# ccnmaastricht/ODE-Column

Hardware: NVIDIA B200
Metric: population_steps_per_sec_fwd_adjoint (higher is better)
Workload: dtype f32

## Files before the change

ode-column_b200/csrc/stage_tc.cu:

```cuda
#include <cstdlib>
#include "stage_tc.cuh"

namespace odecol {
namespace tc {

struct StoreEpi {
    float* C; int M, N, ldc;
    ODECOL_DEVINL void prepare() {}
    ODECOL_DEVINL void rows(int, int i, int n0, int, int g, int TNq, const float (&tot)[kMaxQ]) const {
        if (i >= M) return;
#pragma unroll
        for (int j = 0; j < kMaxQ; ++j) {
            const int b = n0 + g * TNq + j;
            if (j < TNq && b < N) C[(size_t)b * ldc + i] = tot[j];
        }
    }
    ODECOL_DEVINL void tile_done(int, int, int, int, int) const {}
};

struct ContractLayout { int Mp, Np, Kp, TN; size_t off_Ahi, off_Alo, off_Bhi, off_Blo, total; };
static ContractLayout contract_layout(int M, int N, int K) {
    ContractLayout L;
    L.Mp = round_up(M, BM); L.Kp = round_up(K, BK);
    L.TN = pick_tile_n(L.Mp / BM, N);
    L.Np = round_up(N, L.TN);
    size_t o = 0;
    auto take = [&](size_t floats) { const size_t r = o; o += (floats * 4 + 1023) / 1024 * 1024; return r; };
    L.off_Ahi = take((size_t)L.Mp * L.Kp); L.off_Alo = take((size_t)L.Mp * L.Kp);
    L.off_Bhi = take((size_t)L.Np * L.Kp); L.off_Blo = take((size_t)L.Np * L.Kp);
    L.total = o;
    return L;
}


__global__ void k_tc_init(DevProblem p, TileGeom tg, const float* __restrict__ y, const float* __restrict__ t_ptr,
                          float* __restrict__ hi0, float* __restrict__ lo0, float* __restrict__ hi1, float* __restrict__ lo1,
                          float* __restrict__ V0T, float* __restrict__ A0T, float* __restrict__ F0T, int KPa) {
    const int b = blockIdx.x, N = p.N, Kaug = N + p.n_in + 1;
    const size_t ro = (size_t)b * KPa;
    const int nt = b / tg.TN, g = (b % tg.TN) / tg.TNq, jq = (b % tg.TN) % tg.TNq;
    const int q = jq >> 2, e4 = jq & 3;
    if (b >= p.B) {
        for (int k = threadIdx.x; k < KPa; k += blockDim.x) { hi0[ro + k] = 0.f; lo0[ro + k] = 0.f; hi1[ro + k] = 0.f; lo1[ro + k] = 0.f; }
        for (int i = threadIdx.x; i < tg.Np; i += blockDim.x) {
            const size_t o = tg.off(nt, g, q, i) + e4;
            V0T[o] = 0.f; A0T[o] = 0.f; F0T[o] = 0.f;
        }
        return;
    }
    const float* yb = y + (size_t)b * 3 * N;
    int idx = 1;
    const float tcl = knot_locate(p.knot_t, p.K, __ldg(t_ptr), idx);
    const float* ku = p.knot_u + (size_t)b * p.knot_stride_b;
    for (int k = threadIdx.x; k < KPa; k += blockDim.x) {
        float v = 0.f, one = 0.f;
        if (k < N) v = phi_fast(yb[k] - yb[N + k]);
        else if (k < N + p.n_in) v = knot_value(p.knot_t, ku, p.n_in, idx, tcl, k - N);
        else if (k == Kaug - 1) { v = 1.f; one = 1.f; }
        const float h = tf32_rna(v);
        hi0[ro + k] = h; lo0[ro + k] = tf32_rna(v - h);
        hi1[ro + k] = one; lo1[ro + k] = 0.f;
    }
    for (int i = threadIdx.x; i < tg.Np; i += blockDim.x) {
        const size_t o = tg.off(nt, g, q, i) + e4;
        const bool in = i < N;
        const float V = in ? yb[i] : 0.f, A = in ? yb[N + i] : 0.f, F = in ? yb[2 * N + i] : 0.f;
        V0T[o] = V; A0T[o] = A; F0T[o] = F;
    }
}

struct TcFwdLayout {
    int Np, Bp, KPa, TN, KP16;
    size_t off_Whi, off_Wlo, off_Rhi[2], off_Rlo[2], off_K[3], off_Y[2], off_done, off_inv, total;
    size_t off_W16[2], off_R16[2], off_wscale;
};

static TcFwdLayout tc_fwd_layout(const DevProblem& p) {
    TcFwdLayout L;
    L.Np = round_up(p.N, BM);
    L.KPa = round_up(p.N + p.n_in + 1, BK);
    L.TN = pick_tile_n(L.Np / BM, p.B);
    L.Bp = round_up(p.B, L.TN);
    size_t o = 0;
    auto take = [&](size_t floats) { const size_t r = o; o += (floats * 4 + 1023) / 1024 * 1024; return r; };
    L.off_Whi = take((size_t)L.Np * L.KPa); L.off_Wlo = take((size_t)L.Np * L.KPa);
    for (int i = 0; i < 2; ++i) { L.off_Rhi[i] = take((size_t)L.Bp * L.KPa); L.off_Rlo[i] = take((size_t)L.Bp * L.KPa); }
    const size_t plane = (size_t)L.Np * L.Bp;
    for (int i = 0; i < 3; ++i) L.off_K[i] = take(plane);
    for (int i = 0; i < 2; ++i) L.off_Y[i] = take(3 * plane);
    L.off_done = take((size_t)(L.Bp / L.TN) + 64);
    L.off_inv = take(3ull * p.N + 4);
    L.KP16 = round_up(p.N + p.n_in + 1, BK16);
    for (int i = 0; i < 2; ++i) L.off_W16[i] = take(((size_t)L.Np * L.KP16 + 1) / 2);
    for (int i = 0; i < 2; ++i) L.off_R16[i] = take((size_t)L.Bp * L.KP16);
    L.off_wscale = take(4);
    L.total = o;
    return L;
}

}

void tc_launch_init(const DevProblem& p, const tc::TileGeom& tg, const float* y0, const float* t_dev, float* hi0, float* lo0,
                    float* hi1, float* lo1, float* V0T, float* A0T, float* F0T, int KPa, int Bp, cudaStream_t s) {
    tc::k_tc_init<<<Bp, 128, 0, s>>>(p, tg, y0, t_dev, hi0, lo0, hi1, lo1, V0T, A0T, F0T, KPa);
}

int tc_rk4_fwd_persistent(const DevProblem& p, const float* t_dev, int T, const float* y0, float* y_out, int out_every,
                          float* Whi, float* Wlo, float* const Rhi[2], float* const Rlo[2], float* const KT[3],
                          float* const YT[2], unsigned int* done, int Np, int Bp, int KPa, int TN, const tc::CkptView* ck,
                          const tc::Mixed16* mx, cudaStream_t s);

namespace tc {
static Mixed16 mixed16_view(const TcFwdLayout& L, char* w) {
    Mixed16 m;
    for (int i = 0; i < 2; ++i) { m.W16[i] = w + L.off_W16[i]; m.R16[i] = reinterpret_cast<uint16_t*>(w + L.off_R16[i]); }
    m.wscale = reinterpret_cast<float*>(w + L.off_wscale);
    m.KP16 = L.KP16;
    return m;
}
}

static bool persistent_enabled() {
    const char* v = getenv("ODECOL_PERSISTENT");
    return v ? atoi(v) != 0 : true;
}

size_t tc_rk4_fwd_workspace_bytes(const DevProblem& p, int) { return tc::tc_fwd_layout(p).total; }

int tc_rk4_fwd(const DevProblem& p, const float* t_dev, int T, const float* y0, float* y_out, int out_every, void* ws,
               size_t ws_bytes, cudaStream_t s) {
    using namespace tc;
    const TcFwdLayout L = tc_fwd_layout(p);
    if (!ws || ws_bytes < L.total) return ODECOL_E_WORKSPACE;
    if (p.N % 4 != 0) return ODECOL_E_UNSUPPORTED;
    char* w = static_cast<char*>(ws);
    auto F = [&](size_t off) { return reinterpret_cast<float*>(w + off); };
    float *Whi = F(L.off_Whi), *Wlo = F(L.off_Wlo);
    float* Rhi[2] = {F(L.off_Rhi[0]), F(L.off_Rhi[1])};
    float* Rlo[2] = {F(L.off_Rlo[0]), F(L.off_Rlo[1])};
    float* KT[3] = {F(L.off_K[0]), F(L.off_K[1]), F(L.off_K[2])};
    float* YT[2] = {F(L.off_Y[0]), F(L.off_Y[1])};
    const int Kaug = p.N + p.n_in + 1;
    const size_t st = (size_t)p.B * 3 * p.N;
    const TileGeom tg{L.Bp / L.TN, L.Np, L.TN, L.TN / 4};
    if (persistent_enabled() && L.KPa / BK <= kChunkMin) {
        const Mixed16 mx = mixed16_view(L, w);
        return tc_rk4_fwd_persistent(p, t_dev, T, y0, y_out, out_every, Whi, Wlo, Rhi, Rlo, KT, YT,
                                     reinterpret_cast<unsigned int*>(w + L.off_done), L.Np, L.Bp, L.KPa, L.TN, nullptr, &mx, s);
    }

    k_split_pad<<<296, 256, 0, s>>>(p.W_aug, p.N, Kaug, p.ld_w, Whi, Wlo, L.Np, L.KPa);
    k_tc_init<<<L.Bp, 128, 0, s>>>(p, tg, y0, t_dev, Rhi[0], Rlo[0], Rhi[1], Rlo[1], YT[0], YT[0] + tg.plane(),
                                   YT[0] + 2 * tg.plane(), L.KPa);
    count_launch(2);
    if (cudaMemcpyAsync(y_out, y0, sizeof(float) * st, cudaMemcpyDeviceToDevice, s) != cudaSuccess) return ODECOL_E_CUDA;
    CUtensorMap mWhi, mWlo, mRhi[2], mRlo[2];
    bool ok = make_map(&mWhi, Whi, L.Np, L.KPa, L.KPa, BM) && make_map(&mWlo, Wlo, L.Np, L.KPa, L.KPa, BM);
    for (int i = 0; i < 2; ++i)
        ok = ok && make_map(&mRhi[i], Rhi[i], L.Bp, L.KPa, L.KPa, L.TN) && make_map(&mRlo[i], Rlo[i], L.Bp, L.KPa, L.KPa, L.TN);
    if (!ok) return ODECOL_E_CUDA;
    const TileShape ts{L.Np / BM, L.Bp / L.TN, L.TN, L.KPa / BK, 0};
    int cur = 0;
    auto launch = [&](auto& e) { return launch_contract(mWhi, mWlo, mRhi[cur], mRlo[cur], ts, e, s); };
    for (int n = 0; n < T - 1; ++n) {
        const int j = n + 1;
        const bool emit = (j % out_every == 0) || (j == T - 1);
        const size_t r = (j % out_every == 0) ? (size_t)(j / out_every) : (size_t)((T - 2) / out_every + 1);
        auto fill = [&](auto& e) {
            e.p = p; e.tg = tg; e.t = t_dev; e.n = n; e.KPa = L.KPa;
            const size_t pl = tg.plane();
            e.V0T = YT[n & 1]; e.A0T = YT[n & 1] + pl; e.F0T = YT[n & 1] + 2 * pl;
            e.V1T = YT[(n + 1) & 1]; e.A1T = YT[(n + 1) & 1] + pl; e.F1T = YT[(n + 1) & 1] + 2 * pl;
            e.traj_row = emit ? y_out + r * st : nullptr; e.ysel_row = nullptr; e.inv = nullptr; e.G = 0;
            e.K1T = KT[0]; e.K2T = KT[1]; e.K3T = KT[2];
            e.Rhi_nxt = Rhi[cur ^ 1]; e.Rlo_nxt = Rlo[cur ^ 1]; e.DRT_nxt = nullptr;
            e.inv_tm = 1.0f / p.c.tau_m; e.inv_ta = 1.0f / p.c.tau_a; e.inv_ts = 1.0f / p.c.tau_s;
            e.t0 = e.t1 = e.dt = 0.f;
        };
        for (int S = 1; S <= 4; ++S) {
            int rc;
            if (S == 1) { FwdEpiT<1> e; fill(e); rc = launch(e); }
            else if (S == 2) { FwdEpiT<2> e; fill(e); rc = launch(e); }
            else if (S == 3) { FwdEpiT<3> e; fill(e); rc = launch(e); }
            else { FwdEpiT<4> e; fill(e); rc = launch(e); }
            if (rc != ODECOL_OK) return rc;
            cur ^= 1;
        }
    }
    return cudaGetLastError() == cudaSuccess ? ODECOL_OK : ODECOL_E_CUDA;
}


size_t tc_rk4_ckpt_bytes(const DevProblem& p, int T) {
    const tc::TcFwdLayout L = tc::tc_fwd_layout(p);
    if (L.KPa / tc::BK > tc::kChunkMin) return 0;
    const size_t plane = 4ull * L.Np * L.Bp;
    return plane * (2ull * T + 3ull * (T - 1));
}

int tc_rk4_fwd_ckpt(const DevProblem& p, const float* t_dev, int T, const float* y0, const int* sel, int G, float* y_sel,
                    void* ckpt, size_t ckpt_bytes, void* ws, size_t ws_bytes, cudaStream_t s) {
    using namespace tc;
    const TcFwdLayout L = tc_fwd_layout(p);
    if (!ws || ws_bytes < L.total) return ODECOL_E_WORKSPACE;
    if (L.KPa / BK > kChunkMin) return ODECOL_E_UNSUPPORTED;
    if (!ckpt || ckpt_bytes < tc_rk4_ckpt_bytes(p, T)) return ODECOL_E_WORKSPACE;
    if (p.N % 4 != 0) return ODECOL_E_UNSUPPORTED;
    char* w = static_cast<char*>(ws);
    auto F = [&](size_t off) { return reinterpret_cast<float*>(w + off); };
    float* Rhi[2] = {F(L.off_Rhi[0]), F(L.off_Rhi[1])};
    float* Rlo[2] = {F(L.off_Rlo[0]), F(L.off_Rlo[1])};
    float* KT[3] = {F(L.off_K[0]), F(L.off_K[1]), F(L.off_K[2])};
    float* YT[2] = {F(L.off_Y[0]), F(L.off_Y[1])};
    int* inv = reinterpret_cast<int*>(w + L.off_inv);
    const size_t plane = (size_t)L.Np * L.Bp;
    k_tc_build_inv<<<1, 256, 0, s>>>(sel, G, 3 * p.N, inv);
    k_tc_gather_sel<<<296, 256, 0, s>>>(y0, sel, G, p.B, 3 * p.N, y_sel);
    count_launch(2);
    CkptView ck;
    ck.VA = static_cast<float*>(ckpt); ck.K = ck.VA + 2 * plane * (size_t)T; ck.y_sel = y_sel; ck.inv = inv; ck.G = G;
    const Mixed16 mx = mixed16_view(L, w);
    return tc_rk4_fwd_persistent(p, t_dev, T, y0, nullptr, 1, F(L.off_Whi), F(L.off_Wlo), Rhi, Rlo, KT, YT,
                                 reinterpret_cast<unsigned int*>(w + L.off_done), L.Np, L.Bp, L.KPa, L.TN, &ck, &mx, s);
}

size_t tc_contract_workspace_bytes(int M, int N, int K) { return tc::contract_layout(M, N, K).total; }

int tc_contract(const float* A, const float* B, float* C, int M, int N, int K, void* ws, size_t ws_bytes, cudaStream_t s) {
    using namespace tc;
    const ContractLayout L = contract_layout(M, N, K);
    if (!ws || ws_bytes < L.total) return ODECOL_E_WORKSPACE;
    char* w = static_cast<char*>(ws);
    float* Ahi = reinterpret_cast<float*>(w + L.off_Ahi); float* Alo = reinterpret_cast<float*>(w + L.off_Alo);
    float* Bhi = reinterpret_cast<float*>(w + L.off_Bhi); float* Blo = reinterpret_cast<float*>(w + L.off_Blo);
    k_split_pad<<<296, 256, 0, s>>>(A, M, K, K, Ahi, Alo, L.Mp, L.Kp);
    k_split_pad<<<296, 256, 0, s>>>(B, N, K, K, Bhi, Blo, L.Np, L.Kp);
    count_launch(2);
    CUtensorMap ma_hi, ma_lo, mb_hi, mb_lo;
    if (!make_map(&ma_hi, Ahi, L.Mp, L.Kp, L.Kp, BM) || !make_map(&ma_lo, Alo, L.Mp, L.Kp, L.Kp, BM) ||
        !make_map(&mb_hi, Bhi, L.Np, L.Kp, L.Kp, L.TN) || !make_map(&mb_lo, Blo, L.Np, L.Kp, L.Kp, L.TN))
        return ODECOL_E_CUDA;
    const TileShape ts{L.Mp / BM, L.Np / L.TN, L.TN, L.Kp / BK, 0};
    StoreEpi epi{C, M, N, M};
    return launch_contract(ma_hi, ma_lo, mb_hi, mb_lo, ts, epi, s);
}

}
```

ode-column_b200/csrc/stage_tc.cuh:

```cuda
#pragma once
#include <cuda.h>
#include <cuda_fp16.h>
#include "odecol_common.cuh"

namespace odecol {

constexpr float kOneThirdL = 0.3333333333333333f;
constexpr float kTwoThirdsL = 0.6666666666666666f;

static inline int round_up(int x, int m) { return (x + m - 1) / m * m; }

ODECOL_DEVINL float4 ld4(const float* p) { return *reinterpret_cast<const float4*>(p); }
ODECOL_DEVINL void st4(float* p, float4 v) { *reinterpret_cast<float4*>(p) = v; }
ODECOL_DEVINL float4 ld4s(const float* p) { return __ldcg(reinterpret_cast<const float4*>(p)); }
ODECOL_DEVINL void st4s(float* p, float4 v) { __stcg(reinterpret_cast<float4*>(p), v); }

namespace tc {

constexpr int BM = 128;
constexpr int BK = 32;
#ifndef ODECOL_TC_STAGES
#define ODECOL_TC_STAGES 3
#endif
constexpr int STAGES = ODECOL_TC_STAGES;
constexpr int kEpiWarps = 16;
constexpr int kMainAcc = 3;
#ifndef ODECOL_EPI_REGS
#define ODECOL_EPI_REGS 0
#endif
constexpr int kEpiRegs = ODECOL_EPI_REGS;
constexpr int kThreads = 32 * ((kEpiRegs ? 4 : 2) + kEpiWarps);
#ifdef ODECOL_ROLES_HIGH
constexpr int kEpiWarp0 = 0, kTmaWarp = kEpiWarps, kMmaWarp = kEpiWarps + 1;
#else
constexpr int kTmaWarp = 0, kMmaWarp = 1, kEpiWarp0 = kEpiRegs ? 4 : 2;
#endif
template <int N> ODECOL_DEVINL void setmaxnreg_inc() { asm volatile("setmaxnreg.inc.sync.aligned.u32 %0;" ::"n"(N)); }
template <int N> ODECOL_DEVINL void setmaxnreg_dec() { asm volatile("setmaxnreg.dec.sync.aligned.u32 %0;" ::"n"(N)); }
constexpr uint32_t kSpinLimit = 1u << 24;
constexpr int kChunkKB = 16;
constexpr int kChunkMin = 24;

ODECOL_DEVINL uint32_t smem_u32(const void* p) { return (uint32_t)__cvta_generic_to_shared(p); }

ODECOL_DEVINL void mbar_init(uint32_t bar, uint32_t count) {
    asm volatile("mbarrier.init.shared::cta.b64 [%0], %1;" ::"r"(bar), "r"(count) : "memory");
}
ODECOL_DEVINL void mbar_expect_tx(uint32_t bar, uint32_t bytes) {
    asm volatile("mbarrier.arrive.expect_tx.shared::cta.b64 _, [%0], %1;" ::"r"(bar), "r"(bytes) : "memory");
}
ODECOL_DEVINL void mbar_arrive(uint32_t bar) {
    asm volatile("mbarrier.arrive.shared::cta.b64 _, [%0];" ::"r"(bar) : "memory");
}
ODECOL_DEVINL void mbar_wait(uint32_t bar, uint32_t parity) {
    uint32_t done = 0, spins = 0;
    while (true) {
        asm volatile("{\n\t.reg .pred p;\n\tmbarrier.try_wait.parity.shared::cta.b64 p, [%1], %2;\n\tselp.u32 %0, 1, 0, p;\n\t}"
                     : "=r"(done) : "r"(bar), "r"(parity) : "memory");
        if (done) break;
        if (++spins > kSpinLimit) __trap();
    }
}
ODECOL_DEVINL void tma_load_2d(uint32_t dst, const CUtensorMap* map, uint32_t bar, int c0, int c1) {
    asm volatile("cp.async.bulk.tensor.2d.shared::cluster.global.mbarrier::complete_tx::bytes [%0], [%1, {%3, %4}], [%2];"
                 ::"r"(dst), "l"(reinterpret_cast<uint64_t>(map)), "r"(bar), "r"(c0), "r"(c1) : "memory");
}
ODECOL_DEVINL void umma_tf32(uint32_t d_tmem, uint64_t adesc, uint64_t bdesc, uint32_t idesc, uint32_t accumulate) {
    asm volatile("{\n\t.reg .pred p;\n\tsetp.ne.b32 p, %4, 0;\n\ttcgen05.mma.cta_group::1.kind::tf32 [%0], %1, %2, %3, p;\n\t}"
                 ::"r"(d_tmem), "l"(adesc), "l"(bdesc), "r"(idesc), "r"(accumulate) : "memory");
}
ODECOL_DEVINL void umma_commit(uint32_t bar) {
    asm volatile("tcgen05.commit.cta_group::1.mbarrier::arrive::one.shared::cluster.b64 [%0];" ::"r"(bar) : "memory");
}
ODECOL_DEVINL void tc_fence_before() { asm volatile("tcgen05.fence::before_thread_sync;" ::: "memory"); }
ODECOL_DEVINL void tc_fence_after() { asm volatile("tcgen05.fence::after_thread_sync;" ::: "memory"); }
ODECOL_DEVINL void tmem_ld4_issue(uint32_t taddr, uint32_t (&u)[4]) {
    asm volatile("tcgen05.ld.sync.aligned.32x32b.x4.b32 {%0, %1, %2, %3}, [%4];"
                 : "=r"(u[0]), "=r"(u[1]), "=r"(u[2]), "=r"(u[3]) : "r"(taddr));
}
ODECOL_DEVINL void tmem_ld_wait() { asm volatile("tcgen05.wait::ld.sync.aligned;" ::: "memory"); }

ODECOL_DEVINL uint64_t make_smem_desc(uint32_t smem_addr) {
    uint64_t d = 0;
    d |= (uint64_t)((smem_addr & 0x3FFFFu) >> 4);
    d |= (uint64_t)1 << 16;
    d |= (uint64_t)(1024 >> 4) << 32;
    d |= (uint64_t)1 << 46;
    d |= (uint64_t)2 << 61;
    return d;
}
ODECOL_DEVINL uint32_t make_idesc(int tile_n) {
    return (1u << 4) | (2u << 7) | (2u << 10) | ((uint32_t)(tile_n >> 3) << 17) | ((uint32_t)(BM >> 4) << 24);
}

ODECOL_DEVINL float tf32_rna(float x) {
    return __uint_as_float((__float_as_uint(x) + 0x1000u) & 0xFFFFE000u);
}

ODECOL_DEVINL float ldg_if(const float* p, bool ok) {
    float v;
    asm volatile("{\n\t.reg .pred q;\n\tsetp.ne.b32 q, %2, 0;\n\tmov.f32 %0, 0f00000000;\n\t@q ld.global.nc.f32 %0, [%1];\n\t}"
                 : "=f"(v) : "l"(p), "r"((int)ok));
    return v;
}

constexpr int BK16 = 64;
constexpr float kF16Limit = 6.0e4f;
struct F16x2 { unsigned short h, l; };
ODECOL_DEVINL F16x2 f16_split2(float x) {
    const __half h = __float2half_rn(x);
    const __half l = __float2half_rn((x - __half2float(h)) * 2048.0f);
    return {__half_as_ushort(h), __half_as_ushort(l)};
}
ODECOL_DEVINL void st_global_u16_if(uint16_t* p, unsigned short v, bool ok) {
    asm volatile("{\n\t.reg .pred q;\n\tsetp.ne.b32 q, %2, 0;\n\t@q st.global.b16 [%0], %1;\n\t}" ::"l"(p), "h"(v), "r"((int)ok) : "memory");
}
ODECOL_DEVINL void umma_f16(uint32_t d_tmem, uint64_t adesc, uint64_t bdesc, uint32_t idesc, uint32_t accumulate) {
    asm volatile("{\n\t.reg .pred p;\n\tsetp.ne.b32 p, %4, 0;\n\ttcgen05.mma.cta_group::1.kind::f16 [%0], %1, %2, %3, p;\n\t}"
                 ::"r"(d_tmem), "l"(adesc), "l"(bdesc), "r"(idesc), "r"(accumulate) : "memory");
}
ODECOL_DEVINL uint32_t make_idesc16(int tile_n) {
    return (1u << 4) | ((uint32_t)(tile_n >> 3) << 17) | ((uint32_t)(BM >> 4) << 24);
}

struct Mixed16 {
    void* W16[2];
    uint16_t* R16[2];
    float* wscale;
    int KP16;
};

struct TileShape {
    int MT, NT, TN, KB;
    int b_row0;
};

ODECOL_DEVINL unsigned int ld_acquire_u32(const unsigned int* p) {
    unsigned int v;
    asm volatile("ld.acquire.gpu.global.u32 %0, [%1];" : "=r"(v) : "l"(p) : "memory");
    return v;
}

ODECOL_DEVINL void st_global(float* p, float v) { asm volatile("st.global.f32 [%0], %1;" ::"l"(p), "f"(v) : "memory"); }
ODECOL_DEVINL void st_global_if(float* p, float v, bool ok) {
    asm volatile("{\n\t.reg .pred q;\n\tsetp.ne.b32 q, %2, 0;\n\t@q st.global.f32 [%0], %1;\n\t}" ::"l"(p), "f"(v), "r"((int)ok) : "memory");
}
constexpr int kMaxQ = 32;

constexpr int kTileGroupM = 12;
ODECOL_DEVINL void tile_coords(int tile, int MT, int NT, int& m, int& nt) {
    const int per_group = kTileGroupM * NT;
    const int grp = tile / per_group, within = tile - grp * per_group;
    const int gm = min(kTileGroupM, MT - grp * kTileGroupM);
    nt = within / gm;
    m = grp * kTileGroupM + (within - nt * gm);
}

template <class Epi, bool CHUNKED, bool F16 = false>
__global__ void __launch_bounds__(kThreads, 1)
k_tc_contract(const __grid_constant__ CUtensorMap mA_hi, const __grid_constant__ CUtensorMap mA_lo,
              const __grid_constant__ CUtensorMap mB_hi, const __grid_constant__ CUtensorMap mB_lo, TileShape ts, Epi epi) {
    extern __shared__ uint8_t smem_raw[];
    __shared__ __align__(8) uint64_t bars[2 * STAGES + 4];
    __shared__ uint32_t tmem_base_slot;
    const int warp = threadIdx.x >> 5, lane = threadIdx.x & 31;
    const uint32_t ring = (smem_u32(smem_raw) + 1023u) & ~1023u;
    constexpr int KEL = F16 ? BK16 : BK;
    constexpr int CKB = F16 ? kChunkKB / 2 : kChunkKB;
    constexpr float XS = F16 ? 4.8828125e-4f : 1.0f;
    const uint32_t a_bytes = BM * 128, b_bytes = (uint32_t)ts.TN * 128;
    const uint32_t stage_bytes = 2 * a_bytes + 2 * b_bytes;
    const uint32_t full0 = smem_u32(&bars[0]), empty0 = smem_u32(&bars[STAGES]);
    const uint32_t tfull = smem_u32(&bars[2 * STAGES]), tempty = smem_u32(&bars[2 * STAGES + 1]);
    constexpr bool chunked = CHUNKED;
    const uint32_t cfull0 = tfull, cempty0 = smem_u32(&bars[2 * STAGES + 2]);

    const int tiles = ts.MT * ts.NT;
    const uint32_t acc_stride = (uint32_t)ts.TN;
    uint32_t ncols = 32;
    while (ncols < (kMainAcc + 1) * acc_stride) ncols <<= 1;

    if (threadIdx.x == 0) {
        for (int s = 0; s < STAGES; ++s) { mbar_init(full0 + 8 * s, 1); mbar_init(empty0 + 8 * s, 1); }
        mbar_init(tfull, 1);
        mbar_init(tempty, chunked ? 1 : kEpiWarps);
        mbar_init(cempty0, kEpiWarps);
        mbar_init(cempty0 + 8, kEpiWarps);
        asm volatile("fence.mbarrier_init.release.cluster;" ::: "memory");
    }
    if (warp == kMmaWarp) {
        asm volatile("tcgen05.alloc.cta_group::1.sync.aligned.shared::cta.b32 [%0], %1;" ::"r"(smem_u32(&tmem_base_slot)), "r"(ncols) : "memory");
        asm volatile("tcgen05.relinquish_alloc_permit.cta_group::1.sync.aligned;" ::: "memory");
    }
    tc_fence_before();
    __syncthreads();
    tc_fence_after();
    const uint32_t tmem_base = tmem_base_slot;

    if (warp == kTmaWarp) {
        if (lane == 0) {
            int stage = 0; uint32_t phase = 0;
            for (int tile = blockIdx.x; tile < tiles; tile += gridDim.x) {
                int mt_, nt_;
                tile_coords(tile, ts.MT, ts.NT, mt_, nt_);
                const int m0 = mt_ * BM, n0 = nt_ * ts.TN;
                for (int kb = 0; kb < ts.KB; ++kb) {
                    mbar_wait(empty0 + 8 * stage, phase ^ 1);
                    const uint32_t base = ring + stage * stage_bytes, fb = full0 + 8 * stage;
                    mbar_expect_tx(fb, stage_bytes);
                    tma_load_2d(base, &mA_hi, fb, kb * KEL, m0);
                    tma_load_2d(base + a_bytes, &mA_lo, fb, kb * KEL, m0);
                    tma_load_2d(base + 2 * a_bytes, &mB_hi, fb, kb * KEL, n0 + ts.b_row0);
                    tma_load_2d(base + 2 * a_bytes + b_bytes, &mB_lo, fb, kb * KEL, n0 + ts.b_row0);
                    if (++stage == STAGES) { stage = 0; phase ^= 1; }
                }
            }
        }
    } else if (warp == kMmaWarp) {
        if (lane == 0) {
            const uint32_t idesc = F16 ? make_idesc16(ts.TN) : make_idesc(ts.TN);
            const uint32_t d_small = tmem_base + kMainAcc * acc_stride;
            int stage = 0; uint32_t phase = 0, tphase = 0;
            int c = 0;
            for (int tile = blockIdx.x; chunked && tile < tiles; tile += gridDim.x) {
                int jj = 0;
                uint32_t d_main = tmem_base, d_cross = tmem_base + acc_stride;
                for (int kb = 0; kb < ts.KB; ++kb) {
                    if (kb % CKB == 0) {
                        const int set = c & 1;
                        mbar_wait(cempty0 + 8 * set, (uint32_t)((c >> 1) & 1) ^ 1u);
                        tc_fence_after();
                        d_main = tmem_base + (uint32_t)set * 2 * acc_stride;
                        d_cross = d_main + acc_stride;
                        jj = 0;
                    }
                    mbar_wait(full0 + 8 * stage, phase);
                    tc_fence_after();
                    const uint32_t base = ring + stage * stage_bytes;
                    const uint64_t a_hi = make_smem_desc(base), a_lo = make_smem_desc(base + a_bytes);
                    const uint64_t b_hi = make_smem_desc(base + 2 * a_bytes), b_lo = make_smem_desc(base + 2 * a_bytes + b_bytes);
#pragma unroll
                    for (int k = 0; k < 4; ++k, ++jj) {
                        const uint64_t adv = (uint64_t)(k * 32 >> 4);
                        if (F16) {
                            umma_f16(d_cross, a_lo + adv, b_hi + adv, idesc, jj != 0);
                            umma_f16(d_cross, a_hi + adv, b_lo + adv, idesc, 1);
                            umma_f16(d_main, a_hi + adv, b_hi + adv, idesc, jj != 0);
                        } else {
                            umma_tf32(d_cross, a_lo + adv, b_hi + adv, idesc, jj != 0);
                            umma_tf32(d_cross, a_hi + adv, b_lo + adv, idesc, 1);
                            umma_tf32(d_main, a_hi + adv, b_hi + adv, idesc, jj != 0);
                        }
                    }
                    umma_commit(empty0 + 8 * stage);
                    if (++stage == STAGES) { stage = 0; phase ^= 1; }
                    if (kb % CKB == CKB - 1 || kb == ts.KB - 1) { umma_commit(cfull0 + 8 * (c & 1)); ++c; }
                }
            }
            for (int tile = blockIdx.x; !chunked && tile < tiles; tile += gridDim.x) {
                mbar_wait(tempty, tphase ^ 1);
                tc_fence_after();
                int j = 0;
                for (int kb = 0; kb < ts.KB; ++kb) {
                    mbar_wait(full0 + 8 * stage, phase);
                    tc_fence_after();
                    const uint32_t base = ring + stage * stage_bytes;
                    const uint64_t a_hi = make_smem_desc(base), a_lo = make_smem_desc(base + a_bytes);
                    const uint64_t b_hi = make_smem_desc(base + 2 * a_bytes), b_lo = make_smem_desc(base + 2 * a_bytes + b_bytes);
#pragma unroll
                    for (int k = 0; k < 4; ++k, ++j) {
                        const uint64_t adv = (uint64_t)(k * 32 >> 4);
                        const uint32_t d_main = tmem_base + (uint32_t)(j % kMainAcc) * acc_stride;
                        if (F16) {
                            umma_f16(d_small, a_lo + adv, b_hi + adv, idesc, j != 0);
                            umma_f16(d_small, a_hi + adv, b_lo + adv, idesc, 1);
                            umma_f16(d_main, a_hi + adv, b_hi + adv, idesc, j >= kMainAcc);
                        } else {
                            umma_tf32(d_small, a_lo + adv, b_hi + adv, idesc, j != 0);
                            umma_tf32(d_small, a_hi + adv, b_lo + adv, idesc, 1);
                            umma_tf32(d_main, a_hi + adv, b_hi + adv, idesc, j >= kMainAcc);
                        }
                    }
                    umma_commit(empty0 + 8 * stage);
                    if (++stage == STAGES) { stage = 0; phase ^= 1; }
                }
                umma_commit(tfull);
                tphase ^= 1;
            }
        }
    } else if (warp >= kEpiWarp0) {
        const int ew = warp - kEpiWarp0;
        const int quarter = warp & 3;
        const int g = ew >> 2;
        const int etid = ew * 32 + lane;
        const int TNq = ts.TN >> 2;
        epi.prepare();
        uint32_t tphase = 0;
        int cchunk = 0;
        for (int tile = blockIdx.x; tile < tiles; tile += gridDim.x) {
            int m_tile, nt;
            tile_coords(tile, ts.MT, ts.NT, m_tile, nt);
            const int n0 = nt * ts.TN;
            const int row = m_tile * BM + quarter * 32 + lane;
            float tot[kMaxQ];
            if (chunked) {
                const uint32_t lb = tmem_base + ((uint32_t)(quarter * 32) << 16) + (uint32_t)(g * TNq);
#pragma unroll
                for (int q = 0; q < kMaxQ; ++q) tot[q] = 0.f;
                const int nchunks = (ts.KB + CKB - 1) / CKB;
                for (int cc = 0; cc < nchunks; ++cc, ++cchunk) {
                    const int set = cchunk & 1;
                    mbar_wait(cfull0 + 8 * set, (uint32_t)((cchunk >> 1) & 1));
                    tc_fence_after();
#pragma unroll
                    for (int q0 = 0; q0 < kMaxQ / 4; q0 += 4) {
                        uint32_t um[4][4], ux[4][4];
#pragma unroll
                        for (int d = 0; d < 4; ++d) {
                            if (4 * (q0 + d) < TNq) {
                                tmem_ld4_issue(lb + (uint32_t)set * 2 * acc_stride + 4 * (q0 + d), um[d]);
                                tmem_ld4_issue(lb + (uint32_t)set * 2 * acc_stride + acc_stride + 4 * (q0 + d), ux[d]);
                            }
                        }
                        tmem_ld_wait();
#pragma unroll
                        for (int d = 0; d < 4; ++d) {
                            if (4 * (q0 + d) < TNq) {
#pragma unroll
                                for (int e = 0; e < 4; ++e) tot[4 * (q0 + d) + e] += __uint_as_float(ux[d][e]) * XS + __uint_as_float(um[d][e]);
                            }
                        }
                    }
                    tc_fence_before();
                    __syncwarp();
                    if (lane == 0) mbar_arrive(cempty0 + 8 * set);
                }
                epi.rows(m_tile, row, n0, nt, g, TNq, tot);
                epi.tile_done(m_tile, n0, ts.TN, etid, kEpiWarps * 32);
                continue;
            }
            mbar_wait(tfull, tphase);
            tc_fence_after();
            const uint32_t lane_base = tmem_base + ((uint32_t)(quarter * 32) << 16) + (uint32_t)(g * TNq);
#pragma unroll
            for (int q = 0; q < kMaxQ / 4; ++q) {
                if (4 * q < TNq) {
                    uint32_t u[kMainAcc + 1][4];
#pragma unroll
                    for (int a = 0; a <= kMainAcc; ++a) tmem_ld4_issue(lane_base + a * acc_stride + 4 * q, u[a]);
                    tmem_ld_wait();
#pragma unroll
                    for (int e = 0; e < 4; ++e) {
                        float sum = __uint_as_float(u[kMainAcc][e]) * XS;
#pragma unroll
                        for (int a = 0; a < kMainAcc; ++a) sum += __uint_as_float(u[a][e]);
                        tot[4 * q + e] = sum;
                    }
                }
            }
            tc_fence_before();
            __syncwarp();
            if (lane == 0) mbar_arrive(tempty);
            tphase ^= 1;
            epi.rows(m_tile, row, n0, nt, g, TNq, tot);
            epi.tile_done(m_tile, n0, ts.TN, etid, kEpiWarps * 32);
        }
    }
    tc_fence_before();
    __syncthreads();
    if (warp == kMmaWarp) {
        asm volatile("tcgen05.dealloc.cta_group::1.sync.aligned.b32 %0, %1;" ::"r"(tmem_base), "r"(ncols) : "memory");
    }
}

typedef CUresult (*EncodeTiledFn)(CUtensorMap*, CUtensorMapDataType, cuuint32_t, void*, const cuuint64_t*, const cuuint64_t*,
                                  const cuuint32_t*, const cuuint32_t*, CUtensorMapInterleave, CUtensorMapSwizzle,
                                  CUtensorMapL2promotion, CUtensorMapFloatOOBfill);

inline EncodeTiledFn encode_fn() {
    static EncodeTiledFn fn = nullptr;
    if (!fn) {
        void* p = nullptr;
        cudaDriverEntryPointQueryResult q;
        if (cudaGetDriverEntryPoint("cuTensorMapEncodeTiled", &p, cudaEnableDefault, &q) == cudaSuccess && q == cudaDriverEntryPointSuccess)
            fn = reinterpret_cast<EncodeTiledFn>(p);
    }
    return fn;
}

inline bool make_map(CUtensorMap* map, const float* base, uint64_t rows, uint64_t cols, uint64_t ld, uint32_t box_rows,
                     CUtensorMapSwizzle swz = CU_TENSOR_MAP_SWIZZLE_128B) {
    EncodeTiledFn fn = encode_fn();
    if (!fn) return false;
    const cuuint64_t dims[2] = {cols, rows};
    const cuuint64_t strides[1] = {ld * sizeof(float)};
    const cuuint32_t box[2] = {BK, box_rows};
    const cuuint32_t estr[2] = {1, 1};
    return fn(map, CU_TENSOR_MAP_DATA_TYPE_FLOAT32, 2, const_cast<float*>(base), dims, strides, box, estr,
              CU_TENSOR_MAP_INTERLEAVE_NONE, swz, CU_TENSOR_MAP_L2_PROMOTION_L2_256B,
              CU_TENSOR_MAP_FLOAT_OOB_FILL_NONE) == CUDA_SUCCESS;
}

inline bool make_map16(CUtensorMap* map, const void* base, uint64_t rows, uint64_t cols, uint64_t ld, uint32_t box_rows, bool bf16) {
    EncodeTiledFn fn = encode_fn();
    if (!fn) return false;
    const cuuint64_t dims[2] = {cols, rows};
    const cuuint64_t strides[1] = {ld * 2};
    const cuuint32_t box[2] = {BK16, box_rows};
    const cuuint32_t estr[2] = {1, 1};
    return fn(map, bf16 ? CU_TENSOR_MAP_DATA_TYPE_BFLOAT16 : CU_TENSOR_MAP_DATA_TYPE_FLOAT16, 2, const_cast<void*>(base), dims,
              strides, box, estr, CU_TENSOR_MAP_INTERLEAVE_NONE, CU_TENSOR_MAP_SWIZZLE_128B, CU_TENSOR_MAP_L2_PROMOTION_L2_256B,
              CU_TENSOR_MAP_FLOAT_OOB_FILL_NONE) == CUDA_SUCCESS;
}

inline int num_sms() {
    static int n = 0;
    if (!n) {
        int dev = 0;
        cudaGetDevice(&dev);
        cudaDeviceGetAttribute(&n, cudaDevAttrMultiProcessorCount, dev);
        if (n <= 0) n = 148;
    }
    return n;
}

inline int pick_tile_n(int MT, int B) {
    const int sms = num_sms();
    int best = 16;
    double best_cost = 1e30;
    for (int tn = 16; tn <= 128; tn += 16) {
        const int nt = (B + tn - 1) / tn;
        const long tiles = (long)MT * nt;
        const long waves = (tiles + sms - 1) / sms;
        const double cost = (double)waves * (tn + 24.0);
        if (cost < best_cost - 1e-9) { best_cost = cost; best = tn; }
    }
    return best;
}

template <class Epi>
static int launch_contract(const CUtensorMap& a_hi, const CUtensorMap& a_lo, const CUtensorMap& b_hi, const CUtensorMap& b_lo,
                           const TileShape& ts, const Epi& epi, cudaStream_t s) {
    const size_t smem = (size_t)STAGES * (2 * BM * BK * 4 + 2 * (size_t)ts.TN * BK * 4) + 1024;
    static bool configured = false;
    if (!configured) {
        if (cudaFuncSetAttribute(k_tc_contract<Epi, false>, cudaFuncAttributeMaxDynamicSharedMemorySize, 200 * 1024) != cudaSuccess ||
            cudaFuncSetAttribute(k_tc_contract<Epi, true>, cudaFuncAttributeMaxDynamicSharedMemorySize, 200 * 1024) != cudaSuccess)
            return ODECOL_E_CUDA;
        configured = true;
    }
    const int tiles = ts.MT * ts.NT;
    const int grid = tiles < num_sms() ? tiles : num_sms();
    if (ts.KB > kChunkMin) k_tc_contract<Epi, true><<<grid, kThreads, smem, s>>>(a_hi, a_lo, b_hi, b_lo, ts, epi);
    else k_tc_contract<Epi, false><<<grid, kThreads, smem, s>>>(a_hi, a_lo, b_hi, b_lo, ts, epi);
    count_launch();
    return cudaGetLastError() == cudaSuccess ? ODECOL_OK : ODECOL_E_CUDA;
}

template <class Epi>
static int launch_contract16(const CUtensorMap& a_hi, const CUtensorMap& a_lo, const CUtensorMap& b_hi, const CUtensorMap& b_lo,
                             const TileShape& ts, const Epi& epi, cudaStream_t s) {
    const size_t smem = (size_t)STAGES * (2 * BM * 128 + 2 * (size_t)ts.TN * 128) + 1024;
    static bool configured = false;
    if (!configured) {
        if (cudaFuncSetAttribute(k_tc_contract<Epi, false, true>, cudaFuncAttributeMaxDynamicSharedMemorySize, 200 * 1024) != cudaSuccess ||
            cudaFuncSetAttribute(k_tc_contract<Epi, true, true>, cudaFuncAttributeMaxDynamicSharedMemorySize, 200 * 1024) != cudaSuccess)
            return ODECOL_E_CUDA;
        configured = true;
    }
    const int tiles = ts.MT * ts.NT;
    const int grid = tiles < num_sms() ? tiles : num_sms();
    if (ts.KB > kChunkMin / 2) k_tc_contract<Epi, true, true><<<grid, kThreads, smem, s>>>(a_hi, a_lo, b_hi, b_lo, ts, epi);
    else k_tc_contract<Epi, false, true><<<grid, kThreads, smem, s>>>(a_hi, a_lo, b_hi, b_lo, ts, epi);
    count_launch();
    return cudaGetLastError() == cudaSuccess ? ODECOL_OK : ODECOL_E_CUDA;
}

static __global__ void k_split_pad(const float* __restrict__ src, int rows, int cols, int ld, float* __restrict__ hi,
                            float* __restrict__ lo, int rows_p, int cols_p) {
    const size_t total = (size_t)rows_p * cols_p;
    for (size_t e = blockIdx.x * (size_t)blockDim.x + threadIdx.x; e < total; e += (size_t)gridDim.x * blockDim.x) {
        const int r = (int)(e / cols_p), c = (int)(e % cols_p);
        const float x = (r < rows && c < cols) ? src[(size_t)r * ld + c] : 0.0f;
        const float h = tf32_rna(x);
        hi[e] = h;
        lo[e] = tf32_rna(x - h);
    }
}

static __global__ void k_absmax(const float* __restrict__ src, int rows, int cols, int ld, unsigned int* __restrict__ out) {
    unsigned int m = 0;
    const size_t total = (size_t)rows * cols;
    for (size_t e = blockIdx.x * (size_t)blockDim.x + threadIdx.x; e < total; e += (size_t)gridDim.x * blockDim.x) {
        const float x = fabsf(src[(e / cols) * ld + (e % cols)]);
        if (x == x && x < 3.0e38f) m = max(m, __float_as_uint(x));
    }
#pragma unroll
    for (int o = 16; o > 0; o >>= 1) m = max(m, __shfl_xor_sync(0xffffffffu, m, o));
    if ((threadIdx.x & 31) == 0 && m) atomicMax(out, m);
}
static __global__ void k_split16_w(const float* __restrict__ src, int rows, int cols, int ld, __half* __restrict__ hi,
                                   __half* __restrict__ lo, int rows_p, int cols_p, const unsigned int* __restrict__ amax,
                                   float* __restrict__ wscale) {
    const float m = __uint_as_float(*amax);
    int ex = 0;
    if (m > 0.f) frexpf(m, &ex);
    const int sh = m > 0.f ? max(-100, min(100, 14 - ex)) : 0;
    const float sc = ldexpf(1.0f, sh);
    if (blockIdx.x == 0 && threadIdx.x == 0) wscale[0] = ldexpf(1.0f, -sh);
    unsigned int* ovf = reinterpret_cast<unsigned int*>(wscale + 2);
    const size_t total = (size_t)rows_p * cols_p;
    for (size_t e = blockIdx.x * (size_t)blockDim.x + threadIdx.x; e < total; e += (size_t)gridDim.x * blockDim.x) {
        const int r = (int)(e / cols_p), c = (int)(e % cols_p);
        const float x = (r < rows && c < cols) ? src[(size_t)r * ld + c] * sc : 0.0f;
        if (!(fabsf(x) <= kF16Limit)) *ovf = 1u;
        const F16x2 t = f16_split2(x);
        hi[e] = __ushort_as_half(t.h);
        lo[e] = __ushort_as_half(t.l);
    }
}
static __global__ void k_r16_from32(const float* __restrict__ hi, const float* __restrict__ lo, int Bp, int KPa,
                                    uint16_t* __restrict__ R16, int KP16, unsigned int* __restrict__ ovf) {
    const size_t total = (size_t)Bp * KP16, plane = total;
    for (size_t e = blockIdx.x * (size_t)blockDim.x + threadIdx.x; e < total; e += (size_t)gridDim.x * blockDim.x) {
        const int b = (int)(e / KP16), k = (int)(e % KP16);
        const float x = k < KPa ? hi[(size_t)b * KPa + k] + lo[(size_t)b * KPa + k] : 0.0f;
        if (!(fabsf(x) <= kF16Limit)) *ovf = 1u;
        const F16x2 t = f16_split2(x);
        R16[e] = t.h; R16[plane + e] = t.l;
    }
}

static __global__ void k_tc_build_inv(const int* __restrict__ sel, int G, int n3, int* __restrict__ inv) {
    for (int e = threadIdx.x; e < n3; e += blockDim.x) inv[e] = sel ? -1 : e;
    if (threadIdx.x == 0) inv[n3] = sel ? 0 : 1;
    __syncthreads();
    if (sel) for (int g = threadIdx.x; g < G; g += blockDim.x) {
        inv[sel[g]] = g;
        if (sel[g] >= 2 * (n3 / 3)) inv[n3] = 1;
    }
}

static __global__ void k_tc_gather_sel(const float* __restrict__ y, const int* __restrict__ sel, int G, int B, int n3,
                                       float* __restrict__ out) {
    const size_t total = (size_t)B * G;
    for (size_t e = blockIdx.x * (size_t)blockDim.x + threadIdx.x; e < total; e += (size_t)gridDim.x * blockDim.x) {
        const int b = (int)(e / G), g = (int)(e % G);
        out[e] = y[(size_t)b * n3 + (sel ? sel[g] : g)];
    }
}

struct CkptView {
    float* VA; float* K;
    float* y_sel;
    const int* inv;
    int G;
};


struct TileGeom {
    int NT, Np, TN, TNq;
    __host__ __device__ __forceinline__ size_t plane() const { return (size_t)NT * 4 * Np * TNq; }
    ODECOL_DEVINL size_t off(int nt, int g, int q, int i) const {
        return ((((size_t)nt * 4 + g) * (TNq >> 2) + q) * Np + i) * 4;
    }
};

ODECOL_DEVINL void stimulus_columns(const DevProblem& p, int KPa, int idx, float tcl, int n0, int tile_n, int part, int parts,
                                    int tid, int nthr, float* __restrict__ Rhi, float* __restrict__ Rlo) {
    const int n_in = p.n_in, N = p.N;
    const float x0 = __ldg(p.knot_t + idx - 1), x1 = __ldg(p.knot_t + idx);
    const float dx = __fsub_rn(x1, x0), dtc = __fsub_rn(tcl, x0);
    const bool vec = ((n_in | N | KPa | (int)p.knot_stride_b) & 3) == 0 &&
                     ((reinterpret_cast<uintptr_t>(p.knot_u) | reinterpret_cast<uintptr_t>(Rhi) | reinterpret_cast<uintptr_t>(Rlo)) & 15) == 0;
    if (vec) {
        const int nq = n_in >> 2, total = tile_n * nq, share = (total + parts - 1) / parts;
        const int e_end = min(total, (part + 1) * share);
        int e = part * share + tid;
        if (e >= e_end) return;
        int bl = e / nq, c = e - bl * nq;
        const int dbl = nthr / nq, dc = nthr - dbl * nq;
        for (; e < e_end; e += nthr) {
            const int b = n0 + bl;
            if (b < p.B) {
                const float* ku = p.knot_u + (size_t)b * p.knot_stride_b + 4 * c;
                const float4 y0 = __ldg(reinterpret_cast<const float4*>(ku + (size_t)(idx - 1) * n_in));
                const float4 y1 = __ldg(reinterpret_cast<const float4*>(ku + (size_t)idx * n_in));
                float4 h, l;
#pragma unroll
                for (int k = 0; k < 4; ++k) {
                    const float slope = __fdiv_rn(__fsub_rn((&y1.x)[k], (&y0.x)[k]), dx);
                    const float v = __fadd_rn((&y0.x)[k], __fmul_rn(slope, dtc));
                    (&h.x)[k] = tf32_rna(v);
                    (&l.x)[k] = tf32_rna(v - (&h.x)[k]);
                }
                const size_t at = (size_t)b * KPa + N + 4 * c;
                *reinterpret_cast<float4*>(Rhi + at) = h;
                *reinterpret_cast<float4*>(Rlo + at) = l;
            }
            bl += dbl; c += dc;
            if (c >= nq) { c -= nq; ++bl; }
        }
        return;
    }
    const int total = tile_n * n_in, share = (total + parts - 1) / parts;
    const int e_end = min(total, (part + 1) * share);
    for (int e = part * share + tid; e < e_end; e += nthr) {
        const int b = n0 + e / n_in, ch = e % n_in;
        if (b < p.B) {
            const float v = knot_value(p.knot_t, p.knot_u + (size_t)b * p.knot_stride_b, n_in, idx, tcl, ch);
            const float h = tf32_rna(v);
            Rhi[(size_t)b * KPa + N + ch] = h;
            Rlo[(size_t)b * KPa + N + ch] = tf32_rna(v - h);
        }
    }
}

ODECOL_DEVINL void stimulus_columns16(const DevProblem& p, int KP16, size_t plane, int idx, float tcl, int n0, int tile_n, int part,
                                      int parts, int tid, int nthr, uint16_t* __restrict__ R16, unsigned int* __restrict__ ovf) {
    const int n_in = p.n_in, N = p.N;
    const float x0 = __ldg(p.knot_t + idx - 1), x1 = __ldg(p.knot_t + idx);
    const float dx = __fsub_rn(x1, x0), dtc = __fsub_rn(tcl, x0);
    const bool vec = ((n_in | N | KP16 | (int)p.knot_stride_b) & 3) == 0 && (plane & 3) == 0 &&
                     (reinterpret_cast<uintptr_t>(p.knot_u) & 15) == 0 && (reinterpret_cast<uintptr_t>(R16) & 7) == 0;
    if (vec) {
        const int nq = n_in >> 2, total = tile_n * nq, share = (total + parts - 1) / parts;
        const int e_end = min(total, (part + 1) * share);
        int e = part * share + tid;
        if (e >= e_end) return;
        int bl = e / nq, c = e - bl * nq;
        const int dbl = nthr / nq, dc = nthr - dbl * nq;
        for (; e < e_end; e += nthr) {
            const int b = n0 + bl;
            if (b < p.B) {
                const float* ku = p.knot_u + (size_t)b * p.knot_stride_b + 4 * c;
                const float4 y0 = __ldg(reinterpret_cast<const float4*>(ku + (size_t)(idx - 1) * n_in));
                const float4 y1 = __ldg(reinterpret_cast<const float4*>(ku + (size_t)idx * n_in));
                F16x2 t[4];
                bool big = false;
#pragma unroll
                for (int k = 0; k < 4; ++k) {
                    const float slope = __fdiv_rn(__fsub_rn((&y1.x)[k], (&y0.x)[k]), dx);
                    const float v = __fadd_rn((&y0.x)[k], __fmul_rn(slope, dtc));
                    big |= !(fabsf(v) <= kF16Limit);
                    t[k] = f16_split2(v);
                }
                if (big) *ovf = 1u;
                uint16_t* at = R16 + (size_t)b * KP16 + N + 4 * c;
                *reinterpret_cast<uint2*>(at) = make_uint2((uint32_t)t[0].h | ((uint32_t)t[1].h << 16), (uint32_t)t[2].h | ((uint32_t)t[3].h << 16));
                *reinterpret_cast<uint2*>(at + plane) = make_uint2((uint32_t)t[0].l | ((uint32_t)t[1].l << 16), (uint32_t)t[2].l | ((uint32_t)t[3].l << 16));
            }
            bl += dbl; c += dc;
            if (c >= nq) { c -= nq; ++bl; }
        }
        return;
    }
    const int total = tile_n * n_in, share = (total + parts - 1) / parts;
    const int e_end = min(total, (part + 1) * share);
    for (int e = part * share + tid; e < e_end; e += nthr) {
        const int b = n0 + e / n_in, ch = e % n_in;
        if (b < p.B) {
            const float v = knot_value(p.knot_t, p.knot_u + (size_t)b * p.knot_stride_b, n_in, idx, tcl, ch);
            if (!(fabsf(v) <= kF16Limit)) *ovf = 1u;
            const F16x2 t = f16_split2(v);
            uint16_t* at = R16 + (size_t)b * KP16 + N + ch;
            at[0] = t.h; at[plane] = t.l;
        }
    }
}

template <int S, bool F16 = false>
struct FwdEpiT {
    DevProblem p;
    TileGeom tg;
    const float* t;
    int n, KPa;
    uint16_t* R16_nxt; size_t r16_plane; int KP16;
    const float* wscale;
    unsigned int* ovf;
    float ws;
    const float* V0T; const float* A0T; const float* F0T;
    float* V1T; float* A1T; float* F1T;
    float* traj_row;
    float* ysel_row;
    const int* inv;
    int G;
    float* K1T; float* K2T; float* K3T;
    float* Rhi_nxt; float* Rlo_nxt;
    float* DRT_nxt;
    float inv_tm, inv_ta, inv_ts;
    float t0, t1, dt;
    int needF;

    ODECOL_DEVINL void prepare() {
        t0 = __ldg(t + n); t1 = __ldg(t + n + 1);
        dt = __fsub_rn(t1, t0);
        needF = (S == 4 && ysel_row && inv && !traj_row) ? __ldg(inv + 3 * p.N) : 1;
        ws = F16 ? __ldg(wscale) : 1.0f;
    }

    struct Group { float4 V0, A0, k1V, k2V, k3V, F0; };
    ODECOL_DEVINL void load_group(Group& L, size_t oq) const {
        L.V0 = ld4s(V0T + oq); L.A0 = ld4s(A0T + oq);
        if (S >= 2) L.k1V = ld4s(K1T + oq);
        if (S >= 3) L.k2V = ld4s(K2T + oq);
        if (S >= 4) { L.k3V = ld4s(K3T + oq); if (needF) L.F0 = ld4s(F0T + oq); }
    }

    ODECOL_DEVINL void rows(int, int i, int n0, int nt, int g, int TNq, const float (&tot)[kMaxQ]) const {
        if (i >= p.N) return;
        const int N = p.N, B = p.B;
        const float kap = __ldg(p.kappa + i);
        const float third = kOneThirdL;
        const int nq = TNq >> 2;
        const size_t qstride = (size_t)tg.Np * 4;
        const size_t o0 = tg.off(nt, g, 0, i);
        int gV = -1, gA = -1, gF = -1;
        if (S == 4 && ysel_row) { gV = __ldg(inv + i); gA = __ldg(inv + N + i); gF = __ldg(inv + 2 * N + i); }
        Group nxt;
        load_group(nxt, o0);
#pragma unroll 1
        for (int q = 0; q < nq; ++q) {
            const size_t oq = o0 + q * qstride;
            const Group L = nxt;
            if (q + 1 < nq) load_group(nxt, oq + qstride);
            const float4 &V0 = L.V0, &A0 = L.A0, &F0 = L.F0;
            const float4 &k1V = L.k1V, &k2V = L.k2V, &k3V = L.k3V;
            const int q4 = 4 * q;
            float oKV[4], oNV[4], oNA[4], oNF[4], oR[4], oD[4];
#pragma unroll
            for (int e = 0; e < 4; ++e) {
                const float v0 = (&V0.x)[e], a0 = (&A0.x)[e];
                float k1A = 0.f, k2A = 0.f, k3A = 0.f, A = a0, V = v0;
                float r2 = 0.f, r3 = 0.f;
                const float r1 = phi_fast(v0 - a0);
                float r = r1;
                if (S >= 2) {
                    k1A = (kap * r1 - a0) * inv_ta;
                    const float v2 = v0 + dt * (&k1V.x)[e] * third, a2 = a0 + dt * k1A * third;
                    r2 = phi_fast(v2 - a2);
                    if (S == 2) { V = v2; A = a2; r = r2; }
                    if (S >= 3) {
                        k2A = (kap * r2 - a2) * inv_ta;
                        const float v3 = v0 + dt * ((&k2V.x)[e] - (&k1V.x)[e] * third), a3 = a0 + dt * (k2A - k1A * third);
                        r3 = phi_fast(v3 - a3);
                        if (S == 3) { V = v3; A = a3; r = r3; }
                        if (S >= 4) {
                            k3A = (kap * r3 - a3) * inv_ta;
                            V = v0 + dt * ((&k1V.x)[e] - (&k2V.x)[e] + (&k3V.x)[e]); A = a0 + dt * (k1A - k2A + k3A);
                            r = phi_fast(V - A);
                        }
                    }
                }
                const float total = (F16 ? tot[q4 + e] * ws : tot[q4 + e]) * p.c.tau_s;
                const float dV = (total * p.c.R - V) * inv_tm;
                const float dA = (kap * r - A) * inv_ta;
                oKV[e] = dV;
                float nV, nA, nF = 0.f;
                if (S == 1) { nV = v0 + dt * dV * third; nA = a0 + dt * dA * third; }
                if (S == 2) { nV = v0 + dt * (dV - (&k1V.x)[e] * third); nA = a0 + dt * (dA - k1A * third); }
                if (S == 3) { nV = v0 + dt * ((&k1V.x)[e] - (&k2V.x)[e] + dV); nA = a0 + dt * (k1A - k2A + dA); }
                if (S == 4) {
                    nV = v0 + ((&k1V.x)[e] + 3.f * ((&k2V.x)[e] + (&k3V.x)[e]) + dV) * dt * 0.125f;
                    nA = a0 + (k1A + 3.f * (k2A + k3A) + dA) * dt * 0.125f;
                    if (needF) {
                    const float f0 = (&F0.x)[e];
                    const float k1F = (r1 - f0) * inv_ts;
                    const float f2 = f0 + dt * k1F * third;
                    const float k2F = (r2 - f2) * inv_ts;
                    const float f3 = f0 + dt * (k2F - k1F * third);
                    const float k3F = (r3 - f3) * inv_ts;
                    const float f4 = f0 + dt * (k1F - k2F + k3F);
                    const float k4F = (r - f4) * inv_ts;
                    nF = f0 + (k1F + 3.f * (k2F + k3F) + k4F) * dt * 0.125f;
                    }
                }
                oNV[e] = nV; oNA[e] = nA; oNF[e] = nF;
                if (DRT_nxt) phi_dphi_fast(nV - nA, oR[e], oD[e]);
                else oR[e] = phi_fast(nV - nA);
            }
            if (DRT_nxt) st4s(DRT_nxt + oq, make_float4(oD[0], oD[1], oD[2], oD[3]));
            const float4 kV4 = make_float4(oKV[0], oKV[1], oKV[2], oKV[3]);
            if (S == 1) st4s(K1T + oq, kV4);
            if (S == 2) st4s(K2T + oq, kV4);
            if (S == 3) st4s(K3T + oq, kV4);
            if (S == 4) {
                st4s(V1T + oq, make_float4(oNV[0], oNV[1], oNV[2], oNV[3]));
                st4s(A1T + oq, make_float4(oNA[0], oNA[1], oNA[2], oNA[3]));
                if (needF) st4s(F1T + oq, make_float4(oNF[0], oNF[1], oNF[2], oNF[3]));
            }
            const int b0 = n0 + g * TNq + q4;
            float* rh = Rhi_nxt + (size_t)b0 * KPa + i;
            const ptrdiff_t lo_off = Rlo_nxt - Rhi_nxt;
            float* yr = (S == 4 && traj_row) ? traj_row + (size_t)b0 * 3 * N + i : nullptr;
            uint16_t* r16 = F16 ? R16_nxt + (size_t)b0 * KP16 + i : nullptr;
#pragma unroll
            for (int e = 0; e < 4; ++e) {
                const bool ok = b0 + e < B;
                if (F16) {
                    const F16x2 t2 = f16_split2(oR[e]);
                    uint16_t* ph = r16 + (size_t)e * KP16;
                    st_global_u16_if(ph, t2.h, ok);
                    st_global_u16_if(ph + r16_plane, t2.l, ok);
                    if (ok && !(fabsf(oR[e]) <= kF16Limit)) *ovf = 1u;
                } else {
                    const float h = tf32_rna(oR[e]);
                    float* ph = rh + (size_t)e * KPa;
                    st_global_if(ph, h, ok);
                    st_global_if(ph + lo_off, tf32_rna(oR[e] - h), ok);
                }
                if (S == 4 && yr && ok) {
                    float* y = yr + (size_t)e * 3 * N;
                    st_global(y, oNV[e]); st_global(y + N, oNA[e]); st_global(y + 2 * N, oNF[e]);
                }
                if (S == 4 && ysel_row) {
                    float* y = ysel_row + (size_t)(b0 + e) * G;
                    st_global_if(y + gV, oNV[e], ok && gV >= 0);
                    st_global_if(y + gA, oNA[e], ok && gA >= 0);
                    st_global_if(y + gF, oNF[e], ok && gF >= 0);
                }
            }
        }
    }

    ODECOL_DEVINL void tile_done(int m_tile, int n0, int tile_n, int etid, int nthr) const {
        if (p.n_in == 0) return;
        const float tn = S == 1 ? __fadd_rn(t0, __fmul_rn(dt, kOneThirdL)) : S == 2 ? __fadd_rn(t0, __fmul_rn(dt, kTwoThirdsL)) : t1;
        int idx = 1;
        const float tcl = knot_locate(p.knot_t, p.K, tn, idx);
        const int MT = tg.Np / BM;
        if (F16) stimulus_columns16(p, KP16, r16_plane, idx, tcl, n0, tile_n, m_tile, MT, etid, nthr, R16_nxt, ovf);
        else stimulus_columns(p, KPa, idx, tcl, n0, tile_n, m_tile, MT, etid, nthr, Rhi_nxt, Rlo_nxt);
    }
};


}
}
```

ode-column_b200/csrc/stage_tc_bwd.cu:

```cuda
#include "stage_tc.cuh"

namespace odecol {
namespace tc {

template <int S>
struct BwdEpiT {
    DevProblem p;
    TileGeom tg;
    const float* t;
    int n, NPk, G;
    float* acurT;
    float* lamT;
    float* b4T;
    float* b3T;
    const float* DRT;
    float* AVhi_nxt; float* AVlo_nxt;
    const float* grad_y;
    const int* inv;
    float gamma, inv_tm, inv_ta, inv_ts;
    float dt, h8p;
    const float* gy_step;
    int needF;

    ODECOL_DEVINL void prepare() {
        dt = __fsub_rn(__ldg(t + n + 1), __ldg(t + n));
        h8p = n > 0 ? __fsub_rn(__ldg(t + n), __ldg(t + n - 1)) * 0.125f : 0.f;
        needF = __ldg(inv + 3 * p.N);
        gy_step = grad_y + (size_t)n * p.B * G;
    }

    struct Group { float4 aV, aA, dr, lV, lA, lF, p4V, p4A, p3V, p3A, gv, ga, gf; };
    ODECOL_DEVINL void load_group(Group& L, size_t oq, size_t pl, int b0, int gV, int gA, int gF) const {
        L.dr = ld4s(DRT + oq);
        L.lV = ld4s(lamT + oq); L.lA = ld4s(lamT + pl + oq);
        L.lF = needF ? ld4s(lamT + 2 * pl + oq) : make_float4(0.f, 0.f, 0.f, 0.f);
        if (S == 1) { L.aV = ld4s(acurT + oq); L.aA = ld4s(acurT + pl + oq); }
        if (S <= 3) { L.p4V = ld4s(b4T + oq); L.p4A = ld4s(b4T + pl + oq); }
        if (S == 2) { L.p3V = ld4s(b3T + oq); L.p3A = ld4s(b3T + pl + oq); }
        if (S == 1) {
            const float* gy = gy_step + (size_t)b0 * G;
#pragma unroll
            for (int e = 0; e < 4; ++e) {
                const bool ok = b0 + e < p.B;
                (&L.gv.x)[e] = ldg_if(gy + gV, ok && gV >= 0);
                (&L.ga.x)[e] = ldg_if(gy + gA, ok && gA >= 0);
                (&L.gf.x)[e] = ldg_if(gy + gF, ok && gF >= 0);
                gy += G;
            }
        }
    }
    ODECOL_DEVINL void rows(int, int j, int n0, int nt, int g, int TNq, const float (&graw)[kMaxQ]) const {
        if (j >= p.N) return;
        const int N = p.N, B = p.B;
        const float kap = __ldg(p.kappa + j);
        const size_t pl = tg.plane();
        const float h8 = dt * 0.125f, h38 = 3.0f * h8, h3 = dt * kOneThirdL;
        int gV = -1, gA = -1, gF = -1;
        if (S == 1) { gV = inv[j]; gA = inv[N + j]; gF = inv[2 * N + j]; }
        const int nq = TNq >> 2;
        const size_t qstride = (size_t)tg.Np * 4;
        const size_t o0 = tg.off(nt, g, 0, j);
        const int bg = n0 + g * TNq;
        Group nxt;
        load_group(nxt, o0, pl, bg, gV, gA, gF);
#pragma unroll 1
        for (int q = 0; q < nq; ++q) {
            const size_t oq = o0 + q * qstride;
            const Group L = nxt;
            if (q + 1 < nq) load_group(nxt, oq + qstride, pl, bg + 4 * (q + 1), gV, gA, gF);
            float nV[4], nA[4], sV[4], sA[4], sF[4];
#pragma unroll
            for (int e = 0; e < 4; ++e) {
                const float d = (&L.dr.x)[e];
                const float lv = (&L.lV.x)[e], la = (&L.lA.x)[e], lf = (&L.lF.x)[e];
                float av, aa;
                if (S == 4) { av = h8 * lv; aa = h8 * la; }
                if (S == 3) { av = h38 * lv + dt * (&L.p4V.x)[e]; aa = h38 * la + dt * (&L.p4A.x)[e]; }
                if (S == 2) {
                    av = h38 * lv - dt * (&L.p4V.x)[e] + dt * (&L.p3V.x)[e];
                    aa = h38 * la - dt * (&L.p4A.x)[e] + dt * (&L.p3A.x)[e];
                }
                if (S == 1) { av = (&L.aV.x)[e]; aa = (&L.aA.x)[e]; }
                const float bF4 = -(h8 * lf) * inv_ts;
                float af = h8 * lf, bF3 = 0.f, bF2 = 0.f;
                if (S <= 3) { af = h38 * lf + dt * bF4; bF3 = -af * inv_ts; }
                if (S <= 2) { af = h38 * lf - dt * bF4 + dt * bF3; bF2 = -af * inv_ts; }
                if (S == 1) { af = h8 * lf + dt * bF4 - h3 * bF3 + h3 * bF2; }
                const float gg = graw[4 * q + e] + kap * aa * inv_ta + af * inv_ts;
                const float bV = -av * inv_tm + d * gg;
                const float bA = -aa * inv_ta - d * gg;
                if (S == 4) {
                    sV[e] = bV; sA[e] = bA;
                    nV[e] = h38 * lv + dt * bV; nA[e] = h38 * la + dt * bA;
                }
                if (S == 3) {
                    sV[e] = bV; sA[e] = bA;
                    nV[e] = h38 * lv - dt * (&L.p4V.x)[e] + dt * bV;
                    nA[e] = h38 * la - dt * (&L.p4A.x)[e] + dt * bA;
                }
                if (S == 2) {
                    nV[e] = h8 * lv + dt * (&L.p4V.x)[e] - h3 * (&L.p3V.x)[e] + h3 * bV;
                    nA[e] = h8 * la + dt * (&L.p4A.x)[e] - h3 * (&L.p3A.x)[e] + h3 * bA;
                    sV[e] = (&L.p4V.x)[e] + (&L.p3V.x)[e] + bV; sA[e] = (&L.p4A.x)[e] + (&L.p3A.x)[e] + bA;
                }
                if (S == 1) {
                    const float bF1 = -af * inv_ts;
                    const float LV = lv + (&L.p4V.x)[e] + bV + (&L.gv.x)[e];
                    const float LA = la + (&L.p4A.x)[e] + bA + (&L.ga.x)[e];
                    const float LF = lf + (bF4 + bF3 + bF2) + bF1 + (&L.gf.x)[e];
                    sV[e] = LV; sA[e] = LA; sF[e] = LF;
                    nV[e] = h8p * LV; nA[e] = h8p * LA;
                }
            }
            float* sdst = S == 4 ? b4T : S == 3 ? b3T : S == 2 ? b4T : lamT;
            st4s(sdst + oq, make_float4(sV[0], sV[1], sV[2], sV[3]));
            st4s(sdst + pl + oq, make_float4(sA[0], sA[1], sA[2], sA[3]));
            if (S == 1 && needF) st4s(lamT + 2 * pl + oq, make_float4(sF[0], sF[1], sF[2], sF[3]));
            if (S == 2) {
                st4s(acurT + oq, make_float4(nV[0], nV[1], nV[2], nV[3]));
                st4s(acurT + pl + oq, make_float4(nA[0], nA[1], nA[2], nA[3]));
            }
            const int b0 = bg + 4 * q;
            float* ah = AVhi_nxt + (size_t)b0 * NPk + j;
            const ptrdiff_t lo_off = AVlo_nxt - AVhi_nxt;
#pragma unroll
            for (int e = 0; e < 4; ++e) {
                const float v = gamma * nV[e];
                const float h = tf32_rna(v);
                float* ph = ah + (size_t)e * NPk;
                st_global_if(ph, h, b0 + e < B);
                st_global_if(ph + lo_off, tf32_rna(v - h), b0 + e < B);
            }
        }
    }
    ODECOL_DEVINL void tile_done(int, int, int, int, int) const {}
};

constexpr int DW_BK = 32;
constexpr int DW_T = 128;
struct DwShape { int MT, NT, Z, rows_per_split, total_rows, N, Kaug, ld_w; float* grad_W; uint32_t lbo, sbo, major_bits, kadv;
                 float* partial; };
ODECOL_DEVINL uint64_t make_smem_desc_mn(uint32_t smem_addr, uint32_t lbo, uint32_t sbo) {
    uint64_t d = 0;
    d |= (uint64_t)((smem_addr & 0x3FFFFu) >> 4);
    d |= (uint64_t)(lbo >> 4) << 16;
    d |= (uint64_t)(sbo >> 4) << 32;
    d |= (uint64_t)1 << 46;
    d |= (uint64_t)1 << 61;
    return d;
}

struct BwdChainArgs {
    DevProblem p;
    TileGeom tg;
    TileShape ts;
    const float* t;
    int n, NPk, G, Bp;
    float* acurT; float* lamT; float* b4T; float* b3T;
    const float* DRT[4];
    float* AVhi; float* AVlo;
    int set;
    const float* grad_y; const int* inv;
    float gamma, inv_tm, inv_ta, inv_ts;
    unsigned int* done; unsigned int done_base;
    DwShape ds;
};

template <int S>
ODECOL_DEVINL void chain_epilogue(const BwdChainArgs& a, int m_tile, int row, int n0, int nt, int g, int TNq,
                                  const float (&tot)[kMaxQ]) {
    BwdEpiT<S> e;
    e.p = a.p; e.tg = a.tg; e.t = a.t; e.n = a.n; e.NPk = a.NPk; e.G = a.G;
    e.acurT = a.acurT; e.lamT = a.lamT; e.b4T = a.b4T; e.b3T = a.b3T; e.DRT = a.DRT[S - 1];
    const size_t astride = (size_t)a.Bp * a.NPk;
    const size_t nxt = S == 1 ? (size_t)((a.set ^ 1) * 4 + 3) : (size_t)(a.set * 4 + S - 2);
    e.AVhi_nxt = a.AVhi + nxt * astride; e.AVlo_nxt = a.AVlo + nxt * astride;
    e.grad_y = a.grad_y; e.inv = a.inv; e.gamma = a.gamma;
    e.inv_tm = a.inv_tm; e.inv_ta = a.inv_ta; e.inv_ts = a.inv_ts;
    e.prepare();
    e.rows(m_tile, row, n0, nt, g, TNq, tot);
}

template <bool FUSE_DW>
__global__ void __launch_bounds__(kThreads, 1)
k_tc_bwd_chain(const __grid_constant__ CUtensorMap mW_hi, const __grid_constant__ CUtensorMap mW_lo,
               const __grid_constant__ CUtensorMap mA_hi, const __grid_constant__ CUtensorMap mA_lo,
               const __grid_constant__ CUtensorMap dA_hi, const __grid_constant__ CUtensorMap dA_lo,
               const __grid_constant__ CUtensorMap dB_hi, const __grid_constant__ CUtensorMap dB_lo, BwdChainArgs a) {
    extern __shared__ uint8_t smem_raw[];
    __shared__ __align__(8) uint64_t bars[2 * STAGES + 2];
    __shared__ uint32_t tmem_base_slot;
    const TileShape ts = a.ts;
    const int warp = threadIdx.x >> 5, lane = threadIdx.x & 31;
    const uint32_t ring = (smem_u32(smem_raw) + 1023u) & ~1023u;
    const uint32_t a_bytes = BM * BK * 4, b_bytes = (uint32_t)ts.TN * BK * 4;
    const uint32_t stage_bytes = 2 * a_bytes + 2 * b_bytes;
    const uint32_t full0 = smem_u32(&bars[0]), empty0 = smem_u32(&bars[STAGES]);
    const uint32_t tfull = smem_u32(&bars[2 * STAGES]), tempty = smem_u32(&bars[2 * STAGES + 1]);
    const int tiles = ts.MT * ts.NT;
    const uint32_t acc_stride = (uint32_t)ts.TN;
    uint32_t ncols = 32;
    while (ncols < (kMainAcc + 1) * acc_stride) ncols <<= 1;
    if (FUSE_DW) ncols = 512;
    const DwShape& ds = a.ds;
    const int dw_tiles = ds.MT * ds.NT, dw_items = FUSE_DW ? dw_tiles * ds.Z : 0;
    constexpr uint32_t dw_box = DW_BK * 128, dw_op = 4 * dw_box, dw_stage = 4 * dw_op;
    const uint32_t stride = FUSE_DW ? (stage_bytes > dw_stage ? stage_bytes : dw_stage) : stage_bytes;

    if (threadIdx.x == 0) {
        for (int s = 0; s < STAGES; ++s) { mbar_init(full0 + 8 * s, 1); mbar_init(empty0 + 8 * s, 1); }
        mbar_init(tfull, 1);
        mbar_init(tempty, kEpiWarps);
        asm volatile("fence.mbarrier_init.release.cluster;" ::: "memory");
    }
    if (warp == kMmaWarp) {
        asm volatile("tcgen05.alloc.cta_group::1.sync.aligned.shared::cta.b32 [%0], %1;" ::"r"(smem_u32(&tmem_base_slot)), "r"(ncols) : "memory");
        asm volatile("tcgen05.relinquish_alloc_permit.cta_group::1.sync.aligned;" ::: "memory");
    }
    tc_fence_before();
    __syncthreads();
    tc_fence_after();
    const uint32_t tmem_base = tmem_base_slot;
    if (kEpiRegs && warp < kEpiWarp0) setmaxnreg_dec<32>();

    if (warp == kTmaWarp) {
        if (lane == 0) {
            int stage = 0; uint32_t phase = 0;
            for (int q = 0; q < 4; ++q) {
                const int row0 = (a.set * 4 + 3 - q) * a.Bp;
                for (int tile = blockIdx.x; tile < tiles; tile += gridDim.x) {
                    const int nt = tile / ts.MT, m0 = (tile % ts.MT) * BM, n0 = nt * ts.TN;
                    const unsigned int need = a.done_base + (unsigned int)ts.MT * (unsigned int)q;
                    uint32_t spins = 0;
                    while ((int)(ld_acquire_u32(a.done + nt) - need) < 0) {
                        __nanosleep(64);
                        if (++spins > (1u << 26)) __trap();
                    }
                    asm volatile("fence.proxy.async;" ::: "memory");
                    for (int kb = 0; kb < ts.KB; ++kb) {
                        mbar_wait(empty0 + 8 * stage, phase ^ 1);
                        const uint32_t base = ring + stage * stride, fb = full0 + 8 * stage;
                        mbar_expect_tx(fb, stage_bytes);
                        tma_load_2d(base, &mW_hi, fb, kb * BK, m0);
                        tma_load_2d(base + a_bytes, &mW_lo, fb, kb * BK, m0);
                        tma_load_2d(base + 2 * a_bytes, &mA_hi, fb, kb * BK, n0 + row0);
                        tma_load_2d(base + 2 * a_bytes + b_bytes, &mA_lo, fb, kb * BK, n0 + row0);
                        if (++stage == STAGES) { stage = 0; phase ^= 1; }
                    }
                }
            }
            for (int item = blockIdx.x; item < dw_items; item += gridDim.x) {
                const int tile = item % dw_tiles, z = ds.Z - 1 - item / dw_tiles;
                const int i0 = (tile % ds.MT) * DW_T, k0 = (tile / ds.MT) * DW_T;
                const int r0 = z * ds.rows_per_split;
                int r1 = r0 + ds.rows_per_split;
                if (r1 > ds.total_rows) r1 = ds.total_rows;
                const int KBd = (r1 - r0) / DW_BK;
                for (int slot = r0 / a.Bp; slot <= (r1 - 1) / a.Bp && slot < 3 && KBd > 0; ++slot) {
                    const int lo = (r0 > slot * a.Bp ? r0 - slot * a.Bp : 0) / ts.TN;
                    const int hi = ((r1 < (slot + 1) * a.Bp ? r1 - slot * a.Bp : a.Bp) - 1) / ts.TN;
                    const unsigned int need = a.done_base + (unsigned int)ts.MT * (unsigned int)(3 - slot);
                    for (int nt = lo; nt <= hi; ++nt) {
                        uint32_t spins = 0;
                        while ((int)(ld_acquire_u32(a.done + nt) - need) < 0) {
                            __nanosleep(64);
                            if (++spins > (1u << 26)) __trap();
                        }
                    }
                }
                asm volatile("fence.proxy.async;" ::: "memory");
                for (int kb = 0; kb < KBd; ++kb) {
                    const int row = r0 + kb * DW_BK;
                    mbar_wait(empty0 + 8 * stage, phase ^ 1);
                    const uint32_t base = ring + stage * stride, fb = full0 + 8 * stage;
                    mbar_expect_tx(fb, dw_stage);
#pragma unroll
                    for (int m = 0; m < 4; ++m) {
                        tma_load_2d(base + m * dw_box, &dA_hi, fb, i0 + 32 * m, row);
                        tma_load_2d(base + dw_op + m * dw_box, &dA_lo, fb, i0 + 32 * m, row);
                        tma_load_2d(base + 2 * dw_op + m * dw_box, &dB_hi, fb, k0 + 32 * m, row);
                        tma_load_2d(base + 3 * dw_op + m * dw_box, &dB_lo, fb, k0 + 32 * m, row);
                    }
                    if (++stage == STAGES) { stage = 0; phase ^= 1; }
                }
            }
        }
    } else if (warp == kMmaWarp) {
        if (lane == 0) {
            const uint32_t idesc = make_idesc(ts.TN);
            const uint32_t d_small = tmem_base + kMainAcc * acc_stride;
            int stage = 0; uint32_t phase = 0, tphase = 0;
            for (int q = 0; q < 4; ++q) {
                for (int tile = blockIdx.x; tile < tiles; tile += gridDim.x) {
                    mbar_wait(tempty, tphase ^ 1);
                    tc_fence_after();
                    int j = 0;
                    for (int kb = 0; kb < ts.KB; ++kb) {
                        mbar_wait(full0 + 8 * stage, phase);
                        tc_fence_after();
                        const uint32_t base = ring + stage * stride;
                        const uint64_t a_hi = make_smem_desc(base), a_lo = make_smem_desc(base + a_bytes);
                        const uint64_t b_hi = make_smem_desc(base + 2 * a_bytes), b_lo = make_smem_desc(base + 2 * a_bytes + b_bytes);
#pragma unroll
                        for (int k = 0; k < BK / 8; ++k, ++j) {
                            const uint64_t adv = (uint64_t)(k * 32 >> 4);
                            umma_tf32(d_small, a_lo + adv, b_hi + adv, idesc, j != 0);
                            umma_tf32(d_small, a_hi + adv, b_lo + adv, idesc, 1);
                            umma_tf32(tmem_base + (uint32_t)(j % kMainAcc) * acc_stride, a_hi + adv, b_hi + adv, idesc, j >= kMainAcc);
                        }
                        umma_commit(empty0 + 8 * stage);
                        if (++stage == STAGES) { stage = 0; phase ^= 1; }
                    }
                    umma_commit(tfull);
                    tphase ^= 1;
                }
            }
            const uint32_t idesc_dw = (1u << 4) | (2u << 7) | (2u << 10) | ds.major_bits |
                                      ((uint32_t)(DW_T >> 3) << 17) | ((uint32_t)(BM >> 4) << 24);
            const uint32_t d_small_dw = tmem_base + kMainAcc * DW_T;
            for (int item = blockIdx.x; item < dw_items; item += gridDim.x) {
                const int z = ds.Z - 1 - item / dw_tiles;
                const int r0 = z * ds.rows_per_split;
                int r1 = r0 + ds.rows_per_split;
                if (r1 > ds.total_rows) r1 = ds.total_rows;
                const int KBd = (r1 - r0) / DW_BK;
                mbar_wait(tempty, tphase ^ 1);
                tc_fence_after();
                int j = 0;
                for (int kb = 0; kb < KBd; ++kb) {
                    mbar_wait(full0 + 8 * stage, phase);
                    tc_fence_after();
                    const uint32_t base = ring + stage * stride;
                    const uint64_t a_hi = make_smem_desc_mn(base, ds.lbo, ds.sbo), a_lo = make_smem_desc_mn(base + dw_op, ds.lbo, ds.sbo);
                    const uint64_t b_hi = make_smem_desc_mn(base + 2 * dw_op, ds.lbo, ds.sbo), b_lo = make_smem_desc_mn(base + 3 * dw_op, ds.lbo, ds.sbo);
#pragma unroll
                    for (int k = 0; k < DW_BK / 8; ++k, ++j) {
                        const uint64_t adv = (uint64_t)((k * ds.kadv) >> 4);
                        umma_tf32(d_small_dw, a_lo + adv, b_hi + adv, idesc_dw, j != 0);
                        umma_tf32(d_small_dw, a_hi + adv, b_lo + adv, idesc_dw, 1);
                        umma_tf32(tmem_base + (uint32_t)(j % kMainAcc) * DW_T, a_hi + adv, b_hi + adv, idesc_dw, j >= kMainAcc);
                    }
                    umma_commit(empty0 + 8 * stage);
                    if (++stage == STAGES) { stage = 0; phase ^= 1; }
                }
                umma_commit(tfull);
                tphase ^= 1;
            }
        }
    } else if (warp >= kEpiWarp0) {
        if (kEpiRegs) setmaxnreg_inc<(kEpiRegs ? kEpiRegs : 96)>();
        const int ew = warp - kEpiWarp0;
        const int quarter = warp & 3;
        const int g = ew >> 2;
        const int etid = ew * 32 + lane;
        const int TNq = ts.TN >> 2;
        uint32_t tphase = 0;
        for (int q = 0; q < 4; ++q) {
            for (int tile = blockIdx.x; tile < tiles; tile += gridDim.x) {
                const int m_tile = tile % ts.MT, nt = tile / ts.MT, n0 = nt * ts.TN;
                const int row = m_tile * BM + quarter * 32 + lane;
                float tot[kMaxQ];
                mbar_wait(tfull, tphase);
                tc_fence_after();
                const uint32_t lane_base = tmem_base + ((uint32_t)(quarter * 32) << 16) + (uint32_t)(g * TNq);
#pragma unroll
                for (int qq = 0; qq < kMaxQ / 4; ++qq) {
                    if (4 * qq < TNq) {
                        uint32_t u[kMainAcc + 1][4];
#pragma unroll
                        for (int c = 0; c <= kMainAcc; ++c) tmem_ld4_issue(lane_base + c * acc_stride + 4 * qq, u[c]);
                        tmem_ld_wait();
#pragma unroll
                        for (int e = 0; e < 4; ++e) {
                            float sum = __uint_as_float(u[kMainAcc][e]);
#pragma unroll
                            for (int c = 0; c < kMainAcc; ++c) sum += __uint_as_float(u[c][e]);
                            tot[4 * qq + e] = sum;
                        }
                    }
                }
                tc_fence_before();
                __syncwarp();
                if (lane == 0) mbar_arrive(tempty);
                tphase ^= 1;
                switch (q) {
                    case 0: chain_epilogue<4>(a, m_tile, row, n0, nt, g, TNq, tot); break;
                    case 1: chain_epilogue<3>(a, m_tile, row, n0, nt, g, TNq, tot); break;
                    case 2: chain_epilogue<2>(a, m_tile, row, n0, nt, g, TNq, tot); break;
                    default: chain_epilogue<1>(a, m_tile, row, n0, nt, g, TNq, tot); break;
                }
                __threadfence();
                asm volatile("bar.sync 1, %0;" ::"r"(kEpiWarps * 32) : "memory");
                if (etid == 0) atomicAdd(a.done + nt, 1u);
            }
        }
        for (int item = blockIdx.x; item < dw_items; item += gridDim.x) {
            const int tile = item % dw_tiles, z = ds.Z - 1 - item / dw_tiles;
            const int i0 = (tile % ds.MT) * DW_T, k0 = (tile / ds.MT) * DW_T;
            const int r0 = z * ds.rows_per_split;
            int r1 = r0 + ds.rows_per_split;
            if (r1 > ds.total_rows) r1 = ds.total_rows;
            const bool any = (r1 - r0) / DW_BK > 0;
            const int i = i0 + quarter * 32 + lane;
            mbar_wait(tfull, tphase);
            tc_fence_after();
            const uint32_t lane_base = tmem_base + ((uint32_t)(quarter * 32) << 16) + (uint32_t)(g * 32);
#pragma unroll
            for (int qq = 0; qq < 8; ++qq) {
                uint32_t u[kMainAcc + 1][4];
#pragma unroll
                for (int c = 0; c <= kMainAcc; ++c) tmem_ld4_issue(lane_base + c * DW_T + 4 * qq, u[c]);
                tmem_ld_wait();
#pragma unroll
                for (int e = 0; e < 4; ++e) {
                    float sum = __uint_as_float(u[kMainAcc][e]);
#pragma unroll
                    for (int c = 0; c < kMainAcc; ++c) sum += __uint_as_float(u[c][e]);
                    const int k = k0 + g * 32 + 4 * qq + e;
                    if (any && i < ds.N && k < ds.Kaug) atomicAdd(ds.grad_W + (size_t)i * ds.ld_w + k, sum);
                }
            }
            tc_fence_before();
            __syncwarp();
            if (lane == 0) mbar_arrive(tempty);
            tphase ^= 1;
        }
    }
    tc_fence_before();
    __syncthreads();
    if (warp == kMmaWarp) {
        asm volatile("tcgen05.dealloc.cta_group::1.sync.aligned.b32 %0, %1;" ::"r"(tmem_base), "r"(ncols) : "memory");
    }
}

__global__ void k_tc_step_begin(DevProblem p, TileGeom tg, const float* __restrict__ y, const float* __restrict__ t_ptr,
                                float* __restrict__ hi0, float* __restrict__ lo0, float* __restrict__ Y0T,
                                float* __restrict__ DRT, int KPa) {
    const int b4 = blockIdx.x * 4, N = p.N;
    const int nt = b4 / tg.TN, g = (b4 % tg.TN) / tg.TNq, q = ((b4 % tg.TN) % tg.TNq) >> 2;
    const size_t pl = tg.plane();
    for (int i = threadIdx.x; i < tg.Np; i += blockDim.x) {
        float V[4], A[4], F[4], R[4], D[4];
#pragma unroll
        for (int e = 0; e < 4; ++e) {
            const int b = b4 + e;
            const bool in = i < N && b < p.B;
            const float* yb = y + (size_t)b * 3 * N;
            V[e] = in ? yb[i] : 0.f; A[e] = in ? yb[N + i] : 0.f; F[e] = in ? yb[2 * N + i] : 0.f;
            R[e] = 0.f; D[e] = 0.f;
            if (in) {
                phi_dphi_fast(V[e] - A[e], R[e], D[e]);
                const float h = tf32_rna(R[e]);
                hi0[(size_t)b * KPa + i] = h;
                lo0[(size_t)b * KPa + i] = tf32_rna(R[e] - h);
            }
        }
        const size_t o = tg.off(nt, g, q, i);
        st4(Y0T + o, make_float4(V[0], V[1], V[2], V[3]));
        st4(Y0T + pl + o, make_float4(A[0], A[1], A[2], A[3]));
        st4(Y0T + 2 * pl + o, make_float4(F[0], F[1], F[2], F[3]));
        if (DRT) st4(DRT + o, make_float4(D[0], D[1], D[2], D[3]));
    }
    int idx = 1;
    const float tcl = knot_locate(p.knot_t, p.K, __ldg(t_ptr), idx);
    for (int e = threadIdx.x; e < 4 * (p.n_in + 1); e += blockDim.x) {
        const int b = b4 + e / (p.n_in + 1), ch = e % (p.n_in + 1);
        if (b >= p.B) continue;
        float v = 1.0f;
        if (ch < p.n_in) v = knot_value(p.knot_t, p.knot_u + (size_t)b * p.knot_stride_b, p.n_in, idx, tcl, ch);
        const float h = tf32_rna(v);
        hi0[(size_t)b * KPa + N + ch] = h;
        lo0[(size_t)b * KPa + N + ch] = tf32_rna(v - h);
    }
}

struct ReplayJob {
    DevProblem p; TileGeom tg;
    const float* VA; const float* KV; const float* t;
    int n, KPa, slices;
    float* Rhi; float* Rlo; size_t rstride;
    float* D[4];
};

ODECOL_DEVINL void replay_unit(const ReplayJob& j, int blk, int slice, int tid) {
    const DevProblem& p = j.p;
    const TileGeom& tg = j.tg;
    const int b4 = blk * 4, N = p.N;
    const float t0 = __ldg(j.t + j.n), t1 = __ldg(j.t + j.n + 1), dt = __fsub_rn(t1, t0);
    const float third = kOneThirdL, inv_ta = 1.0f / p.c.tau_a;
    const int i = slice * 128 + tid;
    if (i < N) {
        const size_t o = tg.off(b4 / tg.TN, (b4 % tg.TN) / tg.TNq, ((b4 % tg.TN) % tg.TNq) >> 2, i), pl = tg.plane();
        const float4 V0 = ld4s(j.VA + o), A0 = ld4s(j.VA + pl + o);
        const float4 k1V = ld4s(j.KV + o), k2V = ld4s(j.KV + pl + o), k3V = ld4s(j.KV + 2 * pl + o);
        const float kap = __ldg(p.kappa + i);
        float R[4][4], D[4][4];
#pragma unroll
        for (int e = 0; e < 4; ++e) {
            const float v0 = (&V0.x)[e], a0 = (&A0.x)[e];
            phi_dphi_fast(v0 - a0, R[0][e], D[0][e]);
            const float k1A = (kap * R[0][e] - a0) * inv_ta;
            float nV = v0 + dt * (&k1V.x)[e] * third, nA = a0 + dt * k1A * third;
            phi_dphi_fast(nV - nA, R[1][e], D[1][e]);
            const float k2A = (kap * R[1][e] - nA) * inv_ta;
            nV = v0 + dt * ((&k2V.x)[e] - (&k1V.x)[e] * third); nA = a0 + dt * (k2A - k1A * third);
            phi_dphi_fast(nV - nA, R[2][e], D[2][e]);
            const float k3A = (kap * R[2][e] - nA) * inv_ta;
            nV = v0 + dt * ((&k1V.x)[e] - (&k2V.x)[e] + (&k3V.x)[e]); nA = a0 + dt * (k1A - k2A + k3A);
            phi_dphi_fast(nV - nA, R[3][e], D[3][e]);
        }
#pragma unroll
        for (int s = 0; s < 4; ++s) st4s(j.D[s] + o, make_float4(D[s][0], D[s][1], D[s][2], D[s][3]));
        float* rh = j.Rhi + (size_t)b4 * j.KPa + i;
        const ptrdiff_t lo_off = j.Rlo - j.Rhi;
#pragma unroll
        for (int s = 0; s < 4; ++s)
#pragma unroll
            for (int e = 0; e < 4; ++e) {
                const float h = tf32_rna(R[s][e]);
                float* ph = rh + s * j.rstride + (size_t)e * j.KPa;
                st_global_if(ph, h, b4 + e < p.B);
                st_global_if(ph + lo_off, tf32_rna(R[s][e] - h), b4 + e < p.B);
            }
    }
    if (slice != 0) return;
    if (p.n_in == 0) return;
    const int s = tid >> 5;
    const float ts = s == 0 ? t0 : s == 1 ? __fadd_rn(t0, __fmul_rn(dt, kOneThirdL)) : s == 2 ? __fadd_rn(t0, __fmul_rn(dt, kTwoThirdsL)) : t1;
    int idx = 1;
    const float tcl = knot_locate(p.knot_t, p.K, ts, idx);
    stimulus_columns(p, j.KPa, idx, tcl, b4, 4, 0, 1, tid & 31, 32, j.Rhi + s * j.rstride, j.Rlo + s * j.rstride);
}

__global__ void __launch_bounds__(128, 8) k_tc_replay(ReplayJob j) {
    for (int slice = 0; slice < j.slices; ++slice) replay_unit(j, blockIdx.x, slice, threadIdx.x);
}

__global__ void k_tc_bwd_begin(DevProblem p, TileGeom tg, const float* __restrict__ grad_y, const int* __restrict__ inv,
                               int G, const float* __restrict__ t, int T, float gamma, float* __restrict__ lamT,
                               float* __restrict__ acurT, float* __restrict__ AVhi, float* __restrict__ AVlo, int NPk) {
    const int b4 = blockIdx.x * 4, N = p.N;
    const int nt = b4 / tg.TN, g = (b4 % tg.TN) / tg.TNq, q = ((b4 % tg.TN) % tg.TNq) >> 2;
    const size_t pl = tg.plane();
    const float h8 = __fsub_rn(__ldg(t + T - 1), __ldg(t + T - 2)) * 0.125f;
    for (int i = threadIdx.x; i < tg.Np; i += blockDim.x) {
        float L[3][4];
#pragma unroll
        for (int c = 0; c < 3; ++c)
#pragma unroll
            for (int e = 0; e < 4; ++e) {
                const int b = b4 + e;
                float v = 0.f;
                if (i < N && b < p.B) {
                    const int gi = inv[c * N + i];
                    if (gi >= 0) v = grad_y[((size_t)(T - 1) * p.B + b) * G + gi];
                }
                L[c][e] = v;
            }
        const size_t o = tg.off(nt, g, q, i);
#pragma unroll
        for (int c = 0; c < 3; ++c) {
            st4(lamT + c * pl + o, make_float4(L[c][0], L[c][1], L[c][2], L[c][3]));
        }
#pragma unroll
        for (int e = 0; e < 4; ++e) {
            const int b = b4 + e;
            if (i < N && b < p.B) {
                const float v = gamma * h8 * L[0][e];
                const float h = tf32_rna(v);
                AVhi[(size_t)b * NPk + i] = h;
                AVlo[(size_t)b * NPk + i] = tf32_rna(v - h);
            }
        }
    }
}

__global__ void k_tc_untile(DevProblem p, TileGeom tg, const float* __restrict__ srcT, float* __restrict__ dst) {
    const int b4 = blockIdx.x * 4, N = p.N;
    const int nt = b4 / tg.TN, g = (b4 % tg.TN) / tg.TNq, q = ((b4 % tg.TN) % tg.TNq) >> 2;
    const size_t pl = tg.plane();
    for (int i = threadIdx.x; i < N; i += blockDim.x) {
        const size_t o = tg.off(nt, g, q, i);
        for (int c = 0; c < 3; ++c) {
            const float4 v = ld4(srcT + c * pl + o);
#pragma unroll
            for (int e = 0; e < 4; ++e)
                if (b4 + e < p.B) dst[(size_t)(b4 + e) * 3 * N + c * N + i] = (&v.x)[e];
        }
    }
}

__global__ void k_tc_set_one(float* __restrict__ Rhi, int Bp, int B, int KPa, int col, int nslots) {
    const int e = blockIdx.x * blockDim.x + threadIdx.x;
    if (e >= nslots * B) return;
    const int s = e / B, b = e % B;
    Rhi[((size_t)s * Bp + b) * KPa + col] = 1.0f;
}



#ifndef ODECOL_DW_CHUNK
#define ODECOL_DW_CHUNK 8
#endif
constexpr int DW_CHUNK = ODECOL_DW_CHUNK;

__global__ void __launch_bounds__(kThreads, 1)
k_tc_dw(const __grid_constant__ CUtensorMap mA_hi, const __grid_constant__ CUtensorMap mA_lo,
        const __grid_constant__ CUtensorMap mB_hi, const __grid_constant__ CUtensorMap mB_lo, DwShape ds) {
    extern __shared__ uint8_t smem_raw[];
    __shared__ __align__(8) uint64_t bars[2 * STAGES + 4];
    __shared__ uint32_t tmem_base_slot;
    const int warp = threadIdx.x >> 5, lane = threadIdx.x & 31;
    const uint32_t ring = (smem_u32(smem_raw) + 1023u) & ~1023u;
    constexpr uint32_t box_bytes = DW_BK * 128;
    constexpr uint32_t op_bytes = 4 * box_bytes;
    constexpr uint32_t stage_bytes = 4 * op_bytes;
    const uint32_t full0 = smem_u32(&bars[0]), empty0 = smem_u32(&bars[STAGES]);
    const uint32_t tfull0 = smem_u32(&bars[2 * STAGES]), tempty0 = smem_u32(&bars[2 * STAGES + 2]);
    constexpr uint32_t ncols = 512;
    const int tile = blockIdx.x % (ds.MT * ds.NT), z = blockIdx.x / (ds.MT * ds.NT);
    const int i0 = (tile % ds.MT) * DW_T, k0 = (tile / ds.MT) * DW_T;
    const int r0 = z * ds.rows_per_split;
    int r1 = r0 + ds.rows_per_split;
    if (r1 > ds.total_rows) r1 = ds.total_rows;
    const int KB = (r1 - r0) / DW_BK;
    const int nchunks = (KB + DW_CHUNK - 1) / DW_CHUNK;

    if (threadIdx.x == 0) {
        for (int s = 0; s < STAGES; ++s) { mbar_init(full0 + 8 * s, 1); mbar_init(empty0 + 8 * s, 1); }
        for (int s = 0; s < 2; ++s) { mbar_init(tfull0 + 8 * s, 1); mbar_init(tempty0 + 8 * s, kEpiWarps); }
        asm volatile("fence.mbarrier_init.release.cluster;" ::: "memory");
    }
    if (warp == kMmaWarp) {
        asm volatile("tcgen05.alloc.cta_group::1.sync.aligned.shared::cta.b32 [%0], %1;" ::"r"(smem_u32(&tmem_base_slot)), "r"(ncols) : "memory");
        asm volatile("tcgen05.relinquish_alloc_permit.cta_group::1.sync.aligned;" ::: "memory");
    }
    tc_fence_before();
    __syncthreads();
    tc_fence_after();
    const uint32_t tmem_base = tmem_base_slot;

    if (warp == kTmaWarp) {
        if (lane == 0) {
            int stage = 0; uint32_t phase = 0;
            for (int kb = 0; kb < KB; ++kb) {
                mbar_wait(empty0 + 8 * stage, phase ^ 1);
                const uint32_t base = ring + stage * stage_bytes, fb = full0 + 8 * stage;
                mbar_expect_tx(fb, stage_bytes);
                const int row = r0 + kb * DW_BK;
#pragma unroll
                for (int m = 0; m < 4; ++m) {
                    tma_load_2d(base + m * box_bytes, &mA_hi, fb, i0 + 32 * m, row);
                    tma_load_2d(base + op_bytes + m * box_bytes, &mA_lo, fb, i0 + 32 * m, row);
                    tma_load_2d(base + 2 * op_bytes + m * box_bytes, &mB_hi, fb, k0 + 32 * m, row);
                    tma_load_2d(base + 3 * op_bytes + m * box_bytes, &mB_lo, fb, k0 + 32 * m, row);
                }
                if (++stage == STAGES) { stage = 0; phase ^= 1; }
            }
        }
    } else if (warp == kMmaWarp) {
        if (lane == 0) {
            const uint32_t idesc = (1u << 4) | (2u << 7) | (2u << 10) | ds.major_bits |
                                   ((uint32_t)(DW_T >> 3) << 17) | ((uint32_t)(BM >> 4) << 24);
            int stage = 0; uint32_t phase = 0;
            int c = 0, jj = 0;
            uint32_t d_main = tmem_base, d_cross = tmem_base + DW_T;
            for (int kb = 0; kb < KB; ++kb) {
                if (kb % DW_CHUNK == 0) {
                    const int set = c & 1;
                    mbar_wait(tempty0 + 8 * set, (uint32_t)((c >> 1) & 1) ^ 1u);
                    tc_fence_after();
                    d_main = tmem_base + (uint32_t)set * 2 * DW_T;
                    d_cross = d_main + DW_T;
                    jj = 0;
                }
                mbar_wait(full0 + 8 * stage, phase);
                tc_fence_after();
                const uint32_t base = ring + stage * stage_bytes;
                const uint64_t a_hi = make_smem_desc_mn(base, ds.lbo, ds.sbo), a_lo = make_smem_desc_mn(base + op_bytes, ds.lbo, ds.sbo);
                const uint64_t b_hi = make_smem_desc_mn(base + 2 * op_bytes, ds.lbo, ds.sbo), b_lo = make_smem_desc_mn(base + 3 * op_bytes, ds.lbo, ds.sbo);
#pragma unroll
                for (int k = 0; k < DW_BK / 8; ++k, ++jj) {
                    const uint64_t adv = (uint64_t)((k * ds.kadv) >> 4);
                    umma_tf32(d_cross, a_lo + adv, b_hi + adv, idesc, jj != 0);
                    umma_tf32(d_cross, a_hi + adv, b_lo + adv, idesc, 1);
                    umma_tf32(d_main, a_hi + adv, b_hi + adv, idesc, jj != 0);
                }
                umma_commit(empty0 + 8 * stage);
                if (++stage == STAGES) { stage = 0; phase ^= 1; }
                if (kb % DW_CHUNK == DW_CHUNK - 1 || kb == KB - 1) { umma_commit(tfull0 + 8 * (c & 1)); ++c; }
            }
        }
    } else if (warp >= kEpiWarp0) {
        const int ew = warp - kEpiWarp0, quarter = warp & 3, g = ew >> 2;
        const int i = i0 + quarter * 32 + lane;
        float acc[32];
        float* dst = ds.partial ? ds.partial + (size_t)z * ds.N * ds.ld_w : nullptr;
#pragma unroll
        for (int q = 0; q < 32; ++q) {
            const int k = k0 + g * 32 + q;
            acc[q] = (dst && i < ds.N && k < ds.Kaug) ? __ldcg(dst + (size_t)i * ds.ld_w + k) : 0.f;
        }
        for (int c = 0; c < nchunks; ++c) {
            const int set = c & 1;
            mbar_wait(tfull0 + 8 * set, (uint32_t)((c >> 1) & 1));
            tc_fence_after();
            const uint32_t lane_base = tmem_base + ((uint32_t)(quarter * 32) << 16) + (uint32_t)(set * 2 * DW_T + g * 32);
#pragma unroll
            for (int q = 0; q < 8; ++q) {
                uint32_t um[4], ux[4];
                tmem_ld4_issue(lane_base + 4 * q, um);
                tmem_ld4_issue(lane_base + DW_T + 4 * q, ux);
                tmem_ld_wait();
#pragma unroll
                for (int e = 0; e < 4; ++e) acc[4 * q + e] += __uint_as_float(ux[e]) + __uint_as_float(um[e]);
            }
            tc_fence_before();
            __syncwarp();
            if (lane == 0) mbar_arrive(tempty0 + 8 * set);
        }
        if (dst) {
#pragma unroll
            for (int q = 0; q < 32; ++q) {
                const int k = k0 + g * 32 + q;
                if (i < ds.N && k < ds.Kaug) dst[(size_t)i * ds.ld_w + k] = acc[q];
            }
        } else {
#pragma unroll
            for (int q = 0; q < 32; ++q) {
                const int k = k0 + g * 32 + q;
                if (i < ds.N && k < ds.Kaug) atomicAdd(ds.grad_W + (size_t)i * ds.ld_w + k, acc[q]);
            }
        }
    }
    tc_fence_before();
    __syncthreads();
    if (warp == kMmaWarp) {
        asm volatile("tcgen05.dealloc.cta_group::1.sync.aligned.b32 %0, %1;" ::"r"(tmem_base), "r"(ncols) : "memory");
    }
}

__global__ void k_dw_reduce_partials(const float* __restrict__ partial, int Z, size_t n, float* __restrict__ grad_W) {
    for (size_t e = blockIdx.x * (size_t)blockDim.x + threadIdx.x; e < n; e += (size_t)gridDim.x * blockDim.x) {
        float s = 0.f;
        for (int z = 0; z < Z; ++z) s += partial[(size_t)z * n + e];
        grad_W[e] = s;
    }
}

static int launch_dw(const CUtensorMap& a_hi, const CUtensorMap& a_lo, const CUtensorMap& b_hi, const CUtensorMap& b_lo,
                     const DwShape& ds, cudaStream_t s) {
    static bool configured = false;
    if (!configured) {
        if (cudaFuncSetAttribute(k_tc_dw, cudaFuncAttributeMaxDynamicSharedMemorySize, 200 * 1024) != cudaSuccess)
            return ODECOL_E_CUDA;
        configured = true;
    }
    k_tc_dw<<<ds.MT * ds.NT * ds.Z, kThreads, (size_t)STAGES * 4 * 4 * DW_BK * 128 + 1024, s>>>(a_hi, a_lo, b_hi, b_lo, ds);
    count_launch();
    return cudaGetLastError() == cudaSuccess ? ODECOL_OK : ODECOL_E_CUDA;
}


__global__ void k_split_pad_T(const float* __restrict__ src, int n, int ld, float* __restrict__ hi, float* __restrict__ lo,
                              int rows_p, int cols_p) {
    const size_t total = (size_t)rows_p * cols_p;
    for (size_t e = blockIdx.x * (size_t)blockDim.x + threadIdx.x; e < total; e += (size_t)gridDim.x * blockDim.x) {
        const int r = (int)(e / cols_p), c = (int)(e % cols_p);
        const float x = (r < n && c < n) ? src[(size_t)c * ld + r] : 0.0f;
        const float h = tf32_rna(x);
        hi[e] = h;
        lo[e] = tf32_rna(x - h);
    }
}

struct TcBwdLayout {
    int Np, Bp, KPa, NPk, TN;
    size_t off_Whi, off_Wlo, off_WThi, off_WTlo, off_Rhi, off_Rlo, off_AVhi, off_AVlo;
    size_t off_K[3], off_Y, off_DRT[4], off_lam, off_b4, off_b3, off_acur, off_inv, off_done, off_dwpart, total;
    int dwZ;
};

static TcBwdLayout tc_bwd_layout(const DevProblem& p) {
    TcBwdLayout L;
    L.Np = round_up(p.N, BM);
    L.NPk = L.Np;
    L.KPa = round_up(p.N + p.n_in + 1, BK);
    L.TN = pick_tile_n(L.Np / BM, p.B);
    L.Bp = round_up(p.B, L.TN);
    size_t o = 0;
    auto take = [&](size_t bytes) { const size_t r = o; o += (bytes + 1023) / 1024 * 1024; return r; };
    L.off_Whi = take(4ull * L.Np * L.KPa); L.off_Wlo = take(4ull * L.Np * L.KPa);
    L.off_WThi = take(4ull * L.Np * L.NPk); L.off_WTlo = take(4ull * L.Np * L.NPk);
    L.off_Rhi = take(16ull * L.Bp * L.KPa); L.off_Rlo = take(16ull * L.Bp * L.KPa);
    L.off_AVhi = take(32ull * L.Bp * L.NPk); L.off_AVlo = take(32ull * L.Bp * L.NPk);
    const size_t plane = 4ull * L.Np * L.Bp;
    for (int i = 0; i < 3; ++i) L.off_K[i] = take(plane);
    L.off_Y = take(3 * plane);
    for (int i = 0; i < 4; ++i) L.off_DRT[i] = take(plane);
    L.off_lam = take(3 * plane); L.off_b4 = take(2 * plane); L.off_b3 = take(2 * plane); L.off_acur = take(2 * plane);
    L.off_inv = take(sizeof(int) * (3ull * p.N + 4));
    L.off_done = take(sizeof(unsigned int) * (size_t)(L.Bp / L.TN) + 256);
    {
        const int tiles = (L.Np / DW_T) * ((L.KPa + DW_T - 1) / DW_T);
        int z = num_sms() / tiles;
        if (z < 1) z = 1;
        L.dwZ = z;
        L.off_dwpart = take(4ull * (size_t)z * p.N * p.ld_w);
    }
    L.total = o;
    return L;
}

}

size_t tc_contract_tn_workspace_bytes(int M, int N, int K) {
    const size_t Mp = round_up(M, 128), Np = round_up(N, 32), Kp = round_up(K, 64);
    return 4 * (2 * Kp * Mp + 2 * Kp * Np) + 4096;
}

int tc_contract_tn(const float* A, const float* B, float* C, int M, int N, int K, void* ws, size_t ws_bytes, cudaStream_t s) {
    using namespace tc;
    const int Mp = round_up(M, 128), Np = round_up(N, 32), Kp = round_up(K, 64);
    if (!ws || ws_bytes < tc_contract_tn_workspace_bytes(M, N, K)) return ODECOL_E_WORKSPACE;
    float* Ahi = static_cast<float*>(ws);
    float* Alo = Ahi + (size_t)Kp * Mp;
    float* Bhi = Alo + (size_t)Kp * Mp;
    float* Blo = Bhi + (size_t)Kp * Np;
    k_split_pad<<<296, 256, 0, s>>>(A, K, M, M, Ahi, Alo, Kp, Mp);
    k_split_pad<<<296, 256, 0, s>>>(B, K, N, N, Bhi, Blo, Kp, Np);
    CUtensorMap a_hi, a_lo, b_hi, b_lo;
    const CUtensorMapSwizzle sw = CU_TENSOR_MAP_SWIZZLE_128B_ATOM_32B;
    if (!make_map(&a_hi, Ahi, Kp, Mp, Mp, DW_BK, sw) || !make_map(&a_lo, Alo, Kp, Mp, Mp, DW_BK, sw) ||
        !make_map(&b_hi, Bhi, Kp, Np, Np, DW_BK, sw) || !make_map(&b_lo, Blo, Kp, Np, Np, DW_BK, sw))
        return ODECOL_E_CUDA;
    DwShape ds;
    ds.MT = Mp / DW_T; ds.NT = (Np + DW_T - 1) / DW_T; ds.total_rows = Kp;
    int z = 2;
    int rows = (Kp / DW_BK + z - 1) / z * DW_BK;
    ds.rows_per_split = rows; ds.Z = (Kp + rows - 1) / rows;
    ds.N = M; ds.Kaug = N; ds.ld_w = N; ds.grad_W = C; ds.partial = nullptr;
    ds.lbo = DW_BK * 128; ds.sbo = 512; ds.major_bits = (1u << 15) | (1u << 16); ds.kadv = 1024;
    if (cudaMemsetAsync(C, 0, sizeof(float) * (size_t)M * N, s) != cudaSuccess) return ODECOL_E_CUDA;
    count_launch(2);
    return launch_dw(a_hi, a_lo, b_hi, b_lo, ds, s);
}

int tc_dw_accumulate(const float* Ahi, const float* Alo, const float* Bhi, const float* Blo, int rows, int Np, int KPa, int N,
                     int Kaug, int ld_w, float* grad_W, cudaStream_t s) {
    using namespace tc;
    if (rows % DW_BK) return ODECOL_E_SHAPE;
    CUtensorMap a_hi, a_lo, b_hi, b_lo;
    const CUtensorMapSwizzle sw = CU_TENSOR_MAP_SWIZZLE_128B_ATOM_32B;
    if (!make_map(&a_hi, Ahi, rows, Np, Np, DW_BK, sw) || !make_map(&a_lo, Alo, rows, Np, Np, DW_BK, sw) ||
        !make_map(&b_hi, Bhi, rows, KPa, KPa, DW_BK, sw) || !make_map(&b_lo, Blo, rows, KPa, KPa, DW_BK, sw))
        return ODECOL_E_CUDA;
    DwShape ds;
    ds.MT = Np / DW_T; ds.NT = (KPa + DW_T - 1) / DW_T; ds.total_rows = rows;
    int z = num_sms() / (ds.MT * ds.NT);
    if (z < 1) z = 1;
    int rps = (rows / DW_BK + z - 1) / z * DW_BK;
    if (rps < DW_BK) rps = DW_BK;
    ds.rows_per_split = rps; ds.Z = (rows + rps - 1) / rps;
    ds.N = N; ds.Kaug = Kaug; ds.ld_w = ld_w; ds.grad_W = grad_W; ds.partial = nullptr;
    ds.lbo = DW_BK * 128; ds.sbo = 512; ds.major_bits = (1u << 15) | (1u << 16); ds.kadv = 1024;
    return launch_dw(a_hi, a_lo, b_hi, b_lo, ds, s);
}

size_t tc_rk4_bwd_workspace_bytes(const DevProblem& p, int) { return tc::tc_bwd_layout(p).total; }

static int tc_rk4_bwd_impl(const DevProblem& p, const float* t_dev, int T, const float* y_traj, const float* ckVA,
                           const float* ckK, const float* grad_y, const int* sel, int G, float* grad_y0, float* grad_W,
                           void* ws, size_t ws_bytes, cudaStream_t s) {
    using namespace tc;
    const TcBwdLayout L = tc_bwd_layout(p);
    if (!ws || ws_bytes < L.total) return ODECOL_E_WORKSPACE;
    if (p.N % 4 != 0) return ODECOL_E_UNSUPPORTED;
    char* w = static_cast<char*>(ws);
    auto F = [&](size_t off) { return reinterpret_cast<float*>(w + off); };
    float *Whi = F(L.off_Whi), *Wlo = F(L.off_Wlo), *WThi = F(L.off_WThi), *WTlo = F(L.off_WTlo);
    float *Rhi = F(L.off_Rhi), *Rlo = F(L.off_Rlo), *AVhi = F(L.off_AVhi), *AVlo = F(L.off_AVlo);
    float* KT[3] = {F(L.off_K[0]), F(L.off_K[1]), F(L.off_K[2])};
    float* YT = F(L.off_Y);
    float* DRT[4];
    for (int k = 0; k < 4; ++k) DRT[k] = F(L.off_DRT[k]);
    float *lamT = F(L.off_lam), *b4T = F(L.off_b4), *b3T = F(L.off_b3), *acurT = F(L.off_acur);
    int* inv = reinterpret_cast<int*>(w + L.off_inv);
    const int Kaug = p.N + p.n_in + 1;
    const size_t st = (size_t)p.B * 3 * p.N;
    const float gamma = p.c.tau_s * p.c.R / p.c.tau_m;
    const TileGeom tg{L.Bp / L.TN, L.Np, L.TN, L.TN / 4};
    const size_t rstride = (size_t)L.Bp * L.KPa, astride = (size_t)L.Bp * L.NPk;

    if (cudaMemsetAsync(w + L.off_Rhi, 0, L.off_K[0] - L.off_Rhi, s) != cudaSuccess) return ODECOL_E_CUDA;
    k_split_pad<<<296, 256, 0, s>>>(p.W_aug, p.N, Kaug, p.ld_w, Whi, Wlo, L.Np, L.KPa);
    k_split_pad_T<<<296, 256, 0, s>>>(p.W_aug, p.N, p.ld_w, WThi, WTlo, L.Np, L.NPk);
    k_tc_set_one<<<(4 * p.B + 255) / 256, 256, 0, s>>>(Rhi, L.Bp, p.B, L.KPa, Kaug - 1, 4);
    k_tc_build_inv<<<1, 256, 0, s>>>(sel, G, 3 * p.N, inv);
    const size_t first = (size_t)(((T - 2) & 1) * 4 + 3);
    k_tc_bwd_begin<<<L.Bp / 4, 128, 0, s>>>(p, tg, grad_y, inv, G, t_dev, T, gamma, lamT, acurT, AVhi + first * astride,
                                           AVlo + first * astride, L.NPk);
    unsigned int* done = reinterpret_cast<unsigned int*>(w + L.off_done);
    if (cudaMemsetAsync(done, 0, sizeof(unsigned int) * (size_t)(L.Bp / L.TN), s) != cudaSuccess) return ODECOL_E_CUDA;
    count_launch(5);

    CUtensorMap mWhi, mWlo, mWThi, mWTlo, mRhi, mRlo, mAVhi, mAVlo, dAhi[2], dAlo[2], dBhi, dBlo;
    bool ok = make_map(&mWhi, Whi, L.Np, L.KPa, L.KPa, BM) && make_map(&mWlo, Wlo, L.Np, L.KPa, L.KPa, BM) &&
              make_map(&mWThi, WThi, L.Np, L.NPk, L.NPk, BM) && make_map(&mWTlo, WTlo, L.Np, L.NPk, L.NPk, BM) &&
              make_map(&mRhi, Rhi, 4ull * L.Bp, L.KPa, L.KPa, L.TN) && make_map(&mRlo, Rlo, 4ull * L.Bp, L.KPa, L.KPa, L.TN) &&
              make_map(&mAVhi, AVhi, 8ull * L.Bp, L.NPk, L.NPk, L.TN) && make_map(&mAVlo, AVlo, 8ull * L.Bp, L.NPk, L.NPk, L.TN) &&
              make_map(&dAhi[0], AVhi, 4ull * L.Bp, L.NPk, L.NPk, DW_BK, CU_TENSOR_MAP_SWIZZLE_128B_ATOM_32B) &&
              make_map(&dAlo[0], AVlo, 4ull * L.Bp, L.NPk, L.NPk, DW_BK, CU_TENSOR_MAP_SWIZZLE_128B_ATOM_32B) &&
              make_map(&dAhi[1], AVhi + 4 * astride, 4ull * L.Bp, L.NPk, L.NPk, DW_BK, CU_TENSOR_MAP_SWIZZLE_128B_ATOM_32B) &&
              make_map(&dAlo[1], AVlo + 4 * astride, 4ull * L.Bp, L.NPk, L.NPk, DW_BK, CU_TENSOR_MAP_SWIZZLE_128B_ATOM_32B) &&
              make_map(&dBhi, Rhi, 4ull * L.Bp, L.KPa, L.KPa, DW_BK, CU_TENSOR_MAP_SWIZZLE_128B_ATOM_32B) &&
              make_map(&dBlo, Rlo, 4ull * L.Bp, L.KPa, L.KPa, DW_BK, CU_TENSOR_MAP_SWIZZLE_128B_ATOM_32B);
    if (!ok) return ODECOL_E_CUDA;

    DwShape ds;
    ds.MT = L.Np / DW_T; ds.NT = (L.KPa + DW_T - 1) / DW_T;
    ds.total_rows = 4 * L.Bp;
    int z = num_sms() / (ds.MT * ds.NT);
    if (z < 1) z = 1;
    int rows = (ds.total_rows / DW_BK + z - 1) / z * DW_BK;
    if (rows < DW_BK) rows = DW_BK;
    ds.rows_per_split = rows; ds.Z = (ds.total_rows + rows - 1) / rows;
    ds.N = p.N; ds.Kaug = Kaug; ds.ld_w = p.ld_w; ds.grad_W = grad_W;
    ds.lbo = DW_BK * 128; ds.sbo = 512; ds.major_bits = (1u << 15) | (1u << 16); ds.kadv = 1024;
    ds.partial = nullptr;

    const int MT = L.Np / BM, NT = L.Bp / L.TN;
    const char* pe = getenv("ODECOL_PERSISTENT");
    bool use_chain = (pe ? atoi(pe) != 0 : true) && L.NPk / BK <= kChunkMin && L.KPa / BK <= kChunkMin;
    const char* fe = getenv("ODECOL_FUSE_DW");
    const bool dw_fixed_order = (p.flags & ODECOL_FLAG_DETERMINISTIC) != 0;
    const bool fuse_dw = use_chain && !dw_fixed_order && (fe ? atoi(fe) != 0 : true);
    float* dw_partial = nullptr;
    if (dw_fixed_order && ds.Z <= L.dwZ) {
        dw_partial = reinterpret_cast<float*>(w + L.off_dwpart);
        if (cudaMemsetAsync(dw_partial, 0, sizeof(float) * (size_t)ds.Z * p.N * p.ld_w, s) != cudaSuccess) return ODECOL_E_CUDA;
        ds.partial = dw_partial;
    }
    const size_t chain_stage = 2 * BM * BK * 4 + 2 * (size_t)L.TN * BK * 4, dw_stage_b = 4 * 4 * DW_BK * 128;
    const size_t chain_smem = (size_t)STAGES * (fuse_dw && dw_stage_b > chain_stage ? dw_stage_b : chain_stage) + 1024;
    int chain_grid = MT * NT < num_sms() ? MT * NT : num_sms();
    if (use_chain) {
        int max_blocks = 0;
        if (cudaFuncSetAttribute(k_tc_bwd_chain<false>, cudaFuncAttributeMaxDynamicSharedMemorySize, 200 * 1024) != cudaSuccess ||
            cudaFuncSetAttribute(k_tc_bwd_chain<true>, cudaFuncAttributeMaxDynamicSharedMemorySize, 200 * 1024) != cudaSuccess ||
            cudaOccupancyMaxActiveBlocksPerMultiprocessor(&max_blocks, k_tc_bwd_chain<true>, kThreads, chain_smem) != cudaSuccess || max_blocks < 1)
            use_chain = false;
    }
    const size_t ckpl = (size_t)L.Np * L.Bp;
    auto replay = [&](int n) {
        ReplayJob j;
        j.p = p; j.tg = tg;
        j.VA = ckVA + 2 * ckpl * (size_t)n; j.KV = ckK + 3 * ckpl * (size_t)n; j.t = t_dev;
        j.n = n; j.KPa = L.KPa; j.slices = L.Np / 128;
        j.Rhi = Rhi; j.Rlo = Rlo; j.rstride = rstride;
        for (int k = 0; k < 4; ++k) j.D[k] = DRT[k];
        k_tc_replay<<<L.Bp / 4, 128, 0, s>>>(j);
        count_launch();
    };
    for (int n = T - 2; n >= 0; --n) {
        int rc = ODECOL_OK;
        if (ckVA) {
            replay(n);
        } else {
        const float* yn = y_traj + (size_t)n * st;
        k_tc_step_begin<<<L.Bp / 4, 128, 0, s>>>(p, tg, yn, t_dev + n, Rhi, Rlo, YT, DRT[0], L.KPa);
        count_launch();
        auto fill_f = [&](auto& e, int S) {
            e.p = p; e.tg = tg; e.t = t_dev; e.n = n; e.KPa = L.KPa;
            e.V0T = YT; e.A0T = YT + tg.plane(); e.F0T = nullptr;
            e.V1T = e.A1T = e.F1T = nullptr; e.traj_row = nullptr; e.ysel_row = nullptr; e.inv = nullptr; e.G = 0;
            e.K1T = KT[0]; e.K2T = KT[1]; e.K3T = KT[2];
            e.Rhi_nxt = Rhi + S * rstride; e.Rlo_nxt = Rlo + S * rstride; e.DRT_nxt = DRT[S];
            e.inv_tm = 1.0f / p.c.tau_m; e.inv_ta = 1.0f / p.c.tau_a; e.inv_ts = 1.0f / p.c.tau_s;
            e.t0 = e.t1 = e.dt = 0.f;
        };
        { FwdEpiT<1> e; fill_f(e, 1); rc = launch_contract(mWhi, mWlo, mRhi, mRlo, TileShape{MT, NT, L.TN, L.KPa / BK, 0 * L.Bp}, e, s); if (rc) return rc; }
        { FwdEpiT<2> e; fill_f(e, 2); rc = launch_contract(mWhi, mWlo, mRhi, mRlo, TileShape{MT, NT, L.TN, L.KPa / BK, 1 * L.Bp}, e, s); if (rc) return rc; }
        { FwdEpiT<3> e; fill_f(e, 3); rc = launch_contract(mWhi, mWlo, mRhi, mRlo, TileShape{MT, NT, L.TN, L.KPa / BK, 2 * L.Bp}, e, s); if (rc) return rc; }
        }
        const int set = n & 1;
        if (use_chain) {
            BwdChainArgs a;
            a.p = p; a.tg = tg; a.ts = TileShape{MT, NT, L.TN, L.NPk / BK, 0}; a.t = t_dev; a.n = n; a.NPk = L.NPk; a.G = G;
            a.Bp = L.Bp; a.acurT = acurT; a.lamT = lamT; a.b4T = b4T; a.b3T = b3T;
            for (int k = 0; k < 4; ++k) a.DRT[k] = DRT[k];
            a.AVhi = AVhi; a.AVlo = AVlo; a.set = set; a.grad_y = grad_y; a.inv = inv; a.gamma = gamma;
            a.inv_tm = 1.0f / p.c.tau_m; a.inv_ta = 1.0f / p.c.tau_a; a.inv_ts = 1.0f / p.c.tau_s;
            a.done = done; a.done_base = (unsigned int)MT * 4u * (unsigned int)(T - 2 - n);
            a.ds = ds;
            void* args[] = {&mWThi, &mWTlo, &mAVhi, &mAVlo, &dAhi[set], &dAlo[set], &dBhi, &dBlo, &a};
            const void* chain_fn = fuse_dw ? (const void*)k_tc_bwd_chain<true> : (const void*)k_tc_bwd_chain<false>;
            if (cudaLaunchCooperativeKernel(chain_fn, dim3(chain_grid), dim3(kThreads), args, chain_smem, s) != cudaSuccess)
                return ODECOL_E_CUDA;
            count_launch();
        } else {
            auto fill_b = [&](auto& e, int S) {
                e.p = p; e.tg = tg; e.t = t_dev; e.n = n; e.NPk = L.NPk; e.G = G;
                e.acurT = acurT; e.lamT = lamT; e.b4T = b4T; e.b3T = b3T; e.DRT = DRT[S - 1];
                const size_t nxt = S == 1 ? (size_t)((set ^ 1) * 4 + 3) : (size_t)(set * 4 + S - 2);
                e.AVhi_nxt = AVhi + nxt * astride; e.AVlo_nxt = AVlo + nxt * astride;
                e.grad_y = grad_y; e.inv = inv; e.gamma = gamma;
                e.inv_tm = 1.0f / p.c.tau_m; e.inv_ta = 1.0f / p.c.tau_a; e.inv_ts = 1.0f / p.c.tau_s;
                e.dt = e.h8p = 0.f;
            };
            const int r0 = set * 4 * L.Bp;
            { BwdEpiT<4> e; fill_b(e, 4); rc = launch_contract(mWThi, mWTlo, mAVhi, mAVlo, TileShape{MT, NT, L.TN, L.NPk / BK, r0 + 3 * L.Bp}, e, s); if (rc) return rc; }
            { BwdEpiT<3> e; fill_b(e, 3); rc = launch_contract(mWThi, mWTlo, mAVhi, mAVlo, TileShape{MT, NT, L.TN, L.NPk / BK, r0 + 2 * L.Bp}, e, s); if (rc) return rc; }
            { BwdEpiT<2> e; fill_b(e, 2); rc = launch_contract(mWThi, mWTlo, mAVhi, mAVlo, TileShape{MT, NT, L.TN, L.NPk / BK, r0 + 1 * L.Bp}, e, s); if (rc) return rc; }
            { BwdEpiT<1> e; fill_b(e, 1); rc = launch_contract(mWThi, mWTlo, mAVhi, mAVlo, TileShape{MT, NT, L.TN, L.NPk / BK, r0 + 0 * L.Bp}, e, s); if (rc) return rc; }
        }
        if (!(use_chain && fuse_dw)) {
            const int rcd = launch_dw(dAhi[set], dAlo[set], dBhi, dBlo, ds, s);
            if (rcd) return rcd;
        }
    }
    if (dw_partial) {
        k_dw_reduce_partials<<<296, 256, 0, s>>>(dw_partial, ds.Z, (size_t)p.N * p.ld_w, grad_W);
        count_launch();
    }
    if (grad_y0) {
        k_tc_untile<<<L.Bp / 4, 128, 0, s>>>(p, tg, lamT, grad_y0);
        count_launch();
    }
    return cudaGetLastError() == cudaSuccess ? ODECOL_OK : ODECOL_E_CUDA;
}

int tc_rk4_bwd(const DevProblem& p, const float* t_dev, int T, const float* y_traj, const float* grad_y, const int* sel,
               int G, float* grad_y0, float* grad_W, void* ws, size_t ws_bytes, cudaStream_t s) {
    return tc_rk4_bwd_impl(p, t_dev, T, y_traj, nullptr, nullptr, grad_y, sel, G, grad_y0, grad_W, ws, ws_bytes, s);
}

int tc_rk4_bwd_ckpt(const DevProblem& p, const float* t_dev, int T, const void* ckpt, size_t ckpt_bytes, const float* grad_y,
                    const int* sel, int G, float* grad_y0, float* grad_W, void* ws, size_t ws_bytes, cudaStream_t s) {
    const tc::TcBwdLayout L = tc::tc_bwd_layout(p);
    const size_t plane = (size_t)L.Np * L.Bp;
    if (!ckpt || ckpt_bytes < 4 * plane * (2ull * T + 3ull * (T - 1))) return ODECOL_E_WORKSPACE;
    const float* VA = static_cast<const float*>(ckpt);
    return tc_rk4_bwd_impl(p, t_dev, T, nullptr, VA, VA + 2 * plane * (size_t)T, grad_y, sel, G, grad_y0, grad_W, ws, ws_bytes, s);
}

}
```

ode-column_b200/csrc/stage_tc_persist.cu:

```cuda
#include "stage_tc.cuh"

namespace odecol {
namespace tc {

struct PersistArgs {
    DevProblem p;
    TileGeom tg;
    TileShape ts;
    const float* t;
    int T, out_every, KPa;
    float* y_out;
    float* YT[2];
    float* KT[3];
    float* Rhi[2]; float* Rlo[2];
    uint16_t* R16[2]; size_t r16_plane; int KP16; const float* wscale;
    unsigned int* ovf;
    const unsigned int* run_if;
    unsigned int* done;
    CkptView ck;
    float inv_tm, inv_ta, inv_ts;
};

template <int S, bool F16>
ODECOL_DEVINL FwdEpiT<S, F16> persist_epi(const PersistArgs& a, int n, int q) {
    FwdEpiT<S, F16> e;
    e.p = a.p; e.tg = a.tg; e.t = a.t; e.n = n; e.KPa = a.KPa;
    const size_t pl = a.tg.plane();
    const int j = n + 1;
    e.F0T = a.YT[n & 1] + 2 * pl; e.F1T = a.YT[j & 1] + 2 * pl;
    if (a.ck.VA) {
        e.V0T = a.ck.VA + 2 * pl * (size_t)n; e.A0T = e.V0T + pl;
        e.V1T = a.ck.VA + 2 * pl * (size_t)j; e.A1T = e.V1T + pl;
        e.K1T = a.ck.K + 3 * pl * (size_t)n; e.K2T = e.K1T + pl; e.K3T = e.K2T + pl;
        e.traj_row = nullptr;
        e.ysel_row = a.ck.y_sel + (size_t)j * a.p.B * a.ck.G; e.inv = a.ck.inv; e.G = a.ck.G;
    } else {
        e.V0T = a.YT[n & 1]; e.A0T = e.V0T + pl; e.V1T = a.YT[j & 1]; e.A1T = e.V1T + pl;
        e.K1T = a.KT[0]; e.K2T = a.KT[1]; e.K3T = a.KT[2];
        const bool emit = (j % a.out_every == 0) || (j == a.T - 1);
        const size_t r = (j % a.out_every == 0) ? (size_t)(j / a.out_every) : (size_t)((a.T - 2) / a.out_every + 1);
        e.traj_row = emit ? a.y_out + r * ((size_t)a.p.B * 3 * a.p.N) : nullptr;
        e.ysel_row = nullptr; e.inv = nullptr; e.G = 0;
    }
    e.Rhi_nxt = a.Rhi[(q + 1) & 1]; e.Rlo_nxt = a.Rlo[(q + 1) & 1];
    e.R16_nxt = a.R16[(q + 1) & 1]; e.r16_plane = a.r16_plane; e.KP16 = a.KP16; e.wscale = a.wscale; e.ovf = a.ovf;
    e.DRT_nxt = nullptr;
    e.inv_tm = a.inv_tm; e.inv_ta = a.inv_ta; e.inv_ts = a.inv_ts;
    return e;
}

template <int S, bool F16>
ODECOL_DEVINL void persist_epilogue(const PersistArgs& a, int n, int q, int m_tile, int row, int n0, int nt, int g, int TNq,
                                    const float (&tot)[kMaxQ], int etid) {
    FwdEpiT<S, F16> e = persist_epi<S, F16>(a, n, q);
    e.prepare();
    e.rows(m_tile, row, n0, nt, g, TNq, tot);
    e.tile_done(m_tile, n0, a.ts.TN, etid, kEpiWarps * 32);
}

template <bool F16>
__global__ void __launch_bounds__(kThreads, 1)
k_tc_rk4_fwd_persistent(const __grid_constant__ CUtensorMap mW_hi, const __grid_constant__ CUtensorMap mW_lo,
                        const __grid_constant__ CUtensorMap mR_hi0, const __grid_constant__ CUtensorMap mR_lo0,
                        const __grid_constant__ CUtensorMap mR_hi1, const __grid_constant__ CUtensorMap mR_lo1,
                        PersistArgs a) {
    extern __shared__ uint8_t smem_raw[];
    __shared__ __align__(8) uint64_t bars[2 * STAGES + 2];
    __shared__ uint32_t tmem_base_slot;
    if (!F16 && a.run_if && *a.run_if == 0u) return;
    const TileShape ts = a.ts;
    const int warp = threadIdx.x >> 5, lane = threadIdx.x & 31;
    const uint32_t ring = (smem_u32(smem_raw) + 1023u) & ~1023u;
    constexpr int RSTAGES = STAGES;
    constexpr int KEL = F16 ? BK16 : BK;
    const uint32_t a_bytes = BM * 128, b_bytes = (uint32_t)ts.TN * 128;
    const uint32_t stage_bytes = 2 * a_bytes + 2 * b_bytes;
    const uint32_t full0 = smem_u32(&bars[0]), empty0 = smem_u32(&bars[STAGES]);
    const uint32_t tfull = smem_u32(&bars[2 * STAGES]), tempty = smem_u32(&bars[2 * STAGES + 1]);
    const int tiles = ts.MT * ts.NT;
    const uint32_t acc_stride = (uint32_t)ts.TN;
    uint32_t ncols = 32;
    while (ncols < (kMainAcc + 1) * acc_stride) ncols <<= 1;
    const int n_seq = 4 * (a.T - 1);

    if (threadIdx.x == 0) {
        for (int s = 0; s < RSTAGES; ++s) { mbar_init(full0 + 8 * s, 1); mbar_init(empty0 + 8 * s, 1); }
        mbar_init(tfull, 1);
        mbar_init(tempty, kEpiWarps);
        asm volatile("fence.mbarrier_init.release.cluster;" ::: "memory");
    }
    if (warp == kMmaWarp) {
        asm volatile("tcgen05.alloc.cta_group::1.sync.aligned.shared::cta.b32 [%0], %1;" ::"r"(smem_u32(&tmem_base_slot)), "r"(ncols) : "memory");
        asm volatile("tcgen05.relinquish_alloc_permit.cta_group::1.sync.aligned;" ::: "memory");
    }
    tc_fence_before();
    __syncthreads();
    tc_fence_after();
    const uint32_t tmem_base = tmem_base_slot;
    if (kEpiRegs && warp < kEpiWarp0) setmaxnreg_dec<32>();

    if (warp == kTmaWarp) {
        if (lane == 0) {
            int stage = 0; uint32_t phase = 0;
            for (int q = 0; q < n_seq; ++q) {
                const CUtensorMap* mb_hi = (q & 1) ? &mR_hi1 : &mR_hi0;
                const CUtensorMap* mb_lo = (q & 1) ? &mR_lo1 : &mR_lo0;
                for (int tile = blockIdx.x; tile < tiles; tile += gridDim.x) {
                    const int nt = tile / ts.MT, m0 = (tile % ts.MT) * BM, n0 = nt * ts.TN;
                    const unsigned int need = (unsigned int)ts.MT * (unsigned int)q;
                    uint32_t spins = 0;
                    while (ld_acquire_u32(a.done + nt) < need) {
                        __nanosleep(64);
                        if (++spins > (1u << 26)) __trap();
                    }
                    asm volatile("fence.proxy.async;" ::: "memory");
                    for (int kb = 0; kb < ts.KB; ++kb) {
                        mbar_wait(empty0 + 8 * stage, phase ^ 1);
                        const uint32_t base = ring + stage * stage_bytes, fb = full0 + 8 * stage;
                        mbar_expect_tx(fb, stage_bytes);
                        tma_load_2d(base, &mW_hi, fb, kb * KEL, m0);
                        tma_load_2d(base + a_bytes, &mW_lo, fb, kb * KEL, m0);
                        tma_load_2d(base + 2 * a_bytes, mb_hi, fb, kb * KEL, n0);
                        tma_load_2d(base + 2 * a_bytes + b_bytes, mb_lo, fb, kb * KEL, n0);
                        if (++stage == RSTAGES) { stage = 0; phase ^= 1; }
                    }
                }
            }
        }
    } else if (warp == kMmaWarp) {
        if (lane == 0) {
            const uint32_t idesc = F16 ? make_idesc16(ts.TN) : make_idesc(ts.TN);
            const uint32_t d_small = tmem_base + kMainAcc * acc_stride;
            int stage = 0; uint32_t phase = 0, tphase = 0;
            for (int q = 0; q < n_seq; ++q) {
                for (int tile = blockIdx.x; tile < tiles; tile += gridDim.x) {
                    mbar_wait(tempty, tphase ^ 1);
                    tc_fence_after();
                    int j = 0;
                    for (int kb = 0; kb < ts.KB; ++kb) {
                        mbar_wait(full0 + 8 * stage, phase);
                        tc_fence_after();
                        const uint32_t base = ring + stage * stage_bytes;
                        const uint64_t a_hi = make_smem_desc(base), a_lo = make_smem_desc(base + a_bytes);
                        const uint64_t b_hi = make_smem_desc(base + 2 * a_bytes), b_lo = make_smem_desc(base + 2 * a_bytes + b_bytes);
#pragma unroll
                        for (int k = 0; k < 4; ++k, ++j) {
                            const uint64_t adv = (uint64_t)(k * 32 >> 4);
                            const uint32_t d_main = tmem_base + (uint32_t)(j % kMainAcc) * acc_stride;
                            if (F16) {
                                umma_f16(d_small, a_lo + adv, b_hi + adv, idesc, j != 0);
                                umma_f16(d_small, a_hi + adv, b_lo + adv, idesc, 1);
                                umma_f16(d_main, a_hi + adv, b_hi + adv, idesc, j >= kMainAcc);
                            } else {
                                umma_tf32(d_small, a_lo + adv, b_hi + adv, idesc, j != 0);
                                umma_tf32(d_small, a_hi + adv, b_lo + adv, idesc, 1);
                                umma_tf32(d_main, a_hi + adv, b_hi + adv, idesc, j >= kMainAcc);
                            }
                        }
                        umma_commit(empty0 + 8 * stage);
                        if (++stage == RSTAGES) { stage = 0; phase ^= 1; }
                    }
                    umma_commit(tfull);
                    tphase ^= 1;
                }
            }
        }
    } else if (warp >= kEpiWarp0) {
        if (kEpiRegs) setmaxnreg_inc<(kEpiRegs ? kEpiRegs : 96)>();
        const int ew = warp - kEpiWarp0;
        const int quarter = warp & 3;
        const int g = ew >> 2;
        const int etid = ew * 32 + lane;
        const int TNq = ts.TN >> 2;
        uint32_t tphase = 0;
        for (int q = 0; q < n_seq; ++q) {
            const int n = q >> 2, s = (q & 3) + 1;
            for (int tile = blockIdx.x; tile < tiles; tile += gridDim.x) {
                const int m_tile = tile % ts.MT, nt = tile / ts.MT, n0 = nt * ts.TN;
                const int row = m_tile * BM + quarter * 32 + lane;
                float tot[kMaxQ];
                mbar_wait(tfull, tphase);
                tc_fence_after();
                const uint32_t lane_base = tmem_base + ((uint32_t)(quarter * 32) << 16) + (uint32_t)(g * TNq);
#pragma unroll
                for (int qq = 0; qq < kMaxQ / 4; ++qq) {
                    if (4 * qq < TNq) {
                        uint32_t u[kMainAcc + 1][4];
#pragma unroll
                        for (int c = 0; c <= kMainAcc; ++c) tmem_ld4_issue(lane_base + c * acc_stride + 4 * qq, u[c]);
                        tmem_ld_wait();
#pragma unroll
                        for (int e = 0; e < 4; ++e) {
                            float sum = __uint_as_float(u[kMainAcc][e]);
                            if (F16) sum *= 4.8828125e-4f;
#pragma unroll
                            for (int c = 0; c < kMainAcc; ++c) sum += __uint_as_float(u[c][e]);
                            tot[4 * qq + e] = sum;
                        }
                    }
                }
                tc_fence_before();
                __syncwarp();
                if (lane == 0) mbar_arrive(tempty);
                tphase ^= 1;
                switch (s) {
                    case 1: persist_epilogue<1, F16>(a, n, q, m_tile, row, n0, nt, g, TNq, tot, etid); break;
                    case 2: persist_epilogue<2, F16>(a, n, q, m_tile, row, n0, nt, g, TNq, tot, etid); break;
                    case 3: persist_epilogue<3, F16>(a, n, q, m_tile, row, n0, nt, g, TNq, tot, etid); break;
                    default: persist_epilogue<4, F16>(a, n, q, m_tile, row, n0, nt, g, TNq, tot, etid); break;
                }
                __threadfence();
                asm volatile("bar.sync 1, %0;" ::"r"(kEpiWarps * 32) : "memory");
                if (etid == 0) atomicAdd(a.done + nt, 1u);
            }
        }
    }
    tc_fence_before();
    __syncthreads();
    if (warp == kMmaWarp) {
        asm volatile("tcgen05.dealloc.cta_group::1.sync.aligned.b32 %0, %1;" ::"r"(tmem_base), "r"(ncols) : "memory");
    }
}

}

int tc_rk4_fwd_persistent(const DevProblem& p, const float* t_dev, int T, const float* y0, float* y_out, int out_every,
                          float* Whi, float* Wlo, float* const Rhi[2], float* const Rlo[2], float* const KT[3],
                          float* const YT[2], unsigned int* done, int Np, int Bp, int KPa, int TN, const tc::CkptView* ck,
                          const tc::Mixed16* mx, cudaStream_t s) {
    using namespace tc;
    const int Kaug = p.N + p.n_in + 1;
    const size_t st = (size_t)p.B * 3 * p.N;
    const TileGeom tg{Bp / TN, Np, TN, TN / 4};
    static const bool fwd16_env = [] { const char* e = getenv("ODECOL_FWD16"); return e ? atoi(e) != 0 : true; }();
    const bool f16 = mx && fwd16_env;
    const TileShape tsh{Np / BM, Bp / TN, TN, f16 ? mx->KP16 / BK16 : KPa / BK, 0};
    const int tiles = tsh.MT * tsh.NT;
    int grid = tiles < num_sms() ? tiles : num_sms();

    k_split_pad<<<296, 256, 0, s>>>(p.W_aug, p.N, Kaug, p.ld_w, Whi, Wlo, Np, KPa);
    extern void tc_launch_init(const DevProblem&, const TileGeom&, const float*, const float*, float*, float*, float*, float*,
                               float*, float*, float*, int, int, cudaStream_t);
    const size_t pl = tg.plane();
    float* V0 = ck ? ck->VA : YT[0];
    tc_launch_init(p, tg, y0, t_dev, Rhi[0], Rlo[0], Rhi[1], Rlo[1], V0, V0 + pl, YT[0] + 2 * pl, KPa, Bp, s);
    count_launch(2);
    unsigned int* ovf = f16 ? reinterpret_cast<unsigned int*>(mx->wscale + 2) : nullptr;
    if (f16) {
        unsigned int* amax = reinterpret_cast<unsigned int*>(mx->wscale + 1);
        if (cudaMemsetAsync(amax, 0, 2 * sizeof(unsigned int), s) != cudaSuccess) return ODECOL_E_CUDA;
        k_absmax<<<148, 256, 0, s>>>(p.W_aug, p.N, Kaug, p.ld_w, amax);
        k_split16_w<<<296, 256, 0, s>>>(p.W_aug, p.N, Kaug, p.ld_w, static_cast<__half*>(mx->W16[0]), static_cast<__half*>(mx->W16[1]),
                                        Np, mx->KP16, amax, mx->wscale);
        for (int i = 0; i < 2; ++i) k_r16_from32<<<592, 256, 0, s>>>(Rhi[i], Rlo[i], Bp, KPa, mx->R16[i], mx->KP16, ovf);
        count_launch(4);
    }
    if (cudaMemsetAsync(done, 0, sizeof(unsigned int) * tsh.NT, s) != cudaSuccess) return ODECOL_E_CUDA;
    if (!ck && cudaMemcpyAsync(y_out, y0, sizeof(float) * st, cudaMemcpyDeviceToDevice, s) != cudaSuccess) return ODECOL_E_CUDA;
    CUtensorMap mWhi, mWlo, mR[2][2], m32[6];
    bool ok = make_map(&m32[0], Whi, Np, KPa, KPa, BM) && make_map(&m32[1], Wlo, Np, KPa, KPa, BM);
    for (int i = 0; i < 2; ++i)
        ok = ok && make_map(&m32[2 + 2 * i], Rhi[i], Bp, KPa, KPa, TN) && make_map(&m32[3 + 2 * i], Rlo[i], Bp, KPa, KPa, TN);
    if (f16) {
        const size_t plane = (size_t)Bp * mx->KP16;
        ok = ok && make_map16(&mWhi, mx->W16[0], Np, mx->KP16, mx->KP16, BM, false) && make_map16(&mWlo, mx->W16[1], Np, mx->KP16, mx->KP16, BM, false);
        for (int i = 0; i < 2; ++i)
            for (int c = 0; c < 2; ++c)
                ok = ok && make_map16(&mR[i][c], mx->R16[i] + c * plane, Bp, mx->KP16, mx->KP16, TN, false);
    }
    if (!ok) return ODECOL_E_CUDA;

    PersistArgs a;
    a.p = p; a.tg = tg; a.ts = tsh; a.t = t_dev; a.T = T; a.out_every = out_every; a.KPa = KPa; a.y_out = y_out;
    for (int i = 0; i < 2; ++i) { a.YT[i] = YT[i]; a.Rhi[i] = Rhi[i]; a.Rlo[i] = Rlo[i]; a.R16[i] = f16 ? mx->R16[i] : nullptr; }
    a.r16_plane = f16 ? (size_t)Bp * mx->KP16 : 0; a.KP16 = f16 ? mx->KP16 : 0; a.wscale = f16 ? mx->wscale : nullptr;
    a.ovf = ovf; a.run_if = nullptr;
    for (int i = 0; i < 3; ++i) a.KT[i] = KT[i];
    a.done = done;
    if (ck) a.ck = *ck; else a.ck = CkptView{nullptr, nullptr, nullptr, nullptr, 0};
    a.inv_tm = 1.0f / p.c.tau_m; a.inv_ta = 1.0f / p.c.tau_a; a.inv_ts = 1.0f / p.c.tau_s;
    const size_t smem = (size_t)STAGES * (2 * BM * BK * 4 + 2 * (size_t)TN * BK * 4) + 1024;
    for (int v = 0; v < 2; ++v) {
        const void* kern = v ? (const void*)k_tc_rk4_fwd_persistent<true> : (const void*)k_tc_rk4_fwd_persistent<false>;
        if (cudaFuncSetAttribute(kern, cudaFuncAttributeMaxDynamicSharedMemorySize, 200 * 1024) != cudaSuccess) return ODECOL_E_CUDA;
        int max_blocks = 0;
        if (cudaOccupancyMaxActiveBlocksPerMultiprocessor(&max_blocks, kern, kThreads, smem) != cudaSuccess || max_blocks < 1)
            return ODECOL_E_CUDA;
        if (grid > max_blocks * num_sms()) grid = max_blocks * num_sms();
    }
    if (f16) {
        void* args16[] = {&mWhi, &mWlo, &mR[0][0], &mR[0][1], &mR[1][0], &mR[1][1], &a};
        if (cudaLaunchCooperativeKernel((const void*)k_tc_rk4_fwd_persistent<true>, dim3(grid), dim3(kThreads), args16, smem, s) != cudaSuccess)
            return ODECOL_E_CUDA;
        count_launch();
        tc_launch_init(p, tg, y0, t_dev, Rhi[0], Rlo[0], Rhi[1], Rlo[1], V0, V0 + pl, YT[0] + 2 * pl, KPa, Bp, s);
        if (cudaMemsetAsync(done, 0, sizeof(unsigned int) * tsh.NT, s) != cudaSuccess) return ODECOL_E_CUDA;
        a.ts.KB = KPa / BK; a.run_if = ovf;
        count_launch();
    }
    void* args[] = {&m32[0], &m32[1], &m32[2], &m32[3], &m32[4], &m32[5], &a};
    if (cudaLaunchCooperativeKernel((const void*)k_tc_rk4_fwd_persistent<false>, dim3(grid), dim3(kThreads), args, smem, s) != cudaSuccess)
        return ODECOL_E_CUDA;
    count_launch();
    return cudaGetLastError() == cudaSuccess ? ODECOL_OK : ODECOL_E_CUDA;
}

}
```

Before: 7.732 billion.

## Use split-FP16 UMMA for the backward weight-gradient contraction with dynamic scaling

```diff
diff --git a/ode-column_b200/csrc/stage_tc.cu b/ode-column_b200/csrc/stage_tc.cu
--- a/ode-column_b200/csrc/stage_tc.cu
+++ b/ode-column_b200/csrc/stage_tc.cu
@@ -195,7 +195,7 @@
     const tc::TcFwdLayout L = tc::tc_fwd_layout(p);
     if (L.KPa / tc::BK > tc::kChunkMin) return 0;
     const size_t plane = 4ull * L.Np * L.Bp;
-    return plane * (2ull * T + 3ull * (T - 1));
+    return plane * (2ull * T + 3ull * (T - 1)) + 256;
 }
 
 int tc_rk4_fwd_ckpt(const DevProblem& p, const float* t_dev, int T, const float* y0, const int* sel, int G, float* y_sel,
@@ -219,6 +219,7 @@
     count_launch(2);
     CkptView ck;
     ck.VA = static_cast<float*>(ckpt); ck.K = ck.VA + 2 * plane * (size_t)T; ck.y_sel = y_sel; ck.inv = inv; ck.G = G;
+    ck.fmt = reinterpret_cast<unsigned int*>(ck.K + 3 * plane * (size_t)(T - 1));
     const Mixed16 mx = mixed16_view(L, w);
     return tc_rk4_fwd_persistent(p, t_dev, T, y0, nullptr, 1, F(L.off_Whi), F(L.off_Wlo), Rhi, Rlo, KT, YT,
                                  reinterpret_cast<unsigned int*>(w + L.off_done), L.Np, L.Bp, L.KPa, L.TN, &ck, &mx, s);
diff --git a/ode-column_b200/csrc/stage_tc.cuh b/ode-column_b200/csrc/stage_tc.cuh
--- a/ode-column_b200/csrc/stage_tc.cuh
+++ b/ode-column_b200/csrc/stage_tc.cuh
@@ -555,6 +555,7 @@
     float* y_sel;
     const int* inv;
     int G;
+    unsigned int* fmt;
 };
 
 
diff --git a/ode-column_b200/csrc/stage_tc_bwd.cu b/ode-column_b200/csrc/stage_tc_bwd.cu
--- a/ode-column_b200/csrc/stage_tc_bwd.cu
+++ b/ode-column_b200/csrc/stage_tc_bwd.cu
@@ -2,6 +2,35 @@
 
 namespace odecol {
 namespace tc {
+
+constexpr int DW_BK16 = 64;
+struct Dw16 {
+    const unsigned int* fmt;
+    unsigned int* amx;
+    float* scl;
+    unsigned int* rs_done;
+    uint16_t* A16; size_t a16_plane;
+};
+ODECOL_DEVINL int dw16_shift(unsigned int mbits) {
+    if (mbits == 0u || mbits >= 0x7f800000u) return 0;
+    int e = 0;
+    frexpf(__uint_as_float(mbits), &e);
+    return max(-126, min(126, 10 - e));
+}
+ODECOL_DEVINL bool dw16_window(unsigned int mbits, int sh) {
+    if (mbits == 0u) return true;
+    if (mbits >= 0x7f800000u) return false;
+    int e = 0;
+    frexpf(__uint_as_float(mbits), &e);
+    return e + sh >= 5 && e + sh <= 15;
+}
+ODECOL_DEVINL void dw16_resplit(const float* __restrict__ hi, const float* __restrict__ lo, uint16_t* __restrict__ h16,
+                                size_t plane16, size_t count, float sc, size_t e0, size_t step) {
+    for (size_t e = e0; e < count; e += step) {
+        const F16x2 t = f16_split2((__ldcg(hi + e) + __ldcg(lo + e)) * sc);
+        h16[e] = t.h; h16[plane16 + e] = t.l;
+    }
+}
 
 template <int S>
 struct BwdEpiT {
@@ -15,10 +44,14 @@
     float* b3T;
     const float* DRT;
     float* AVhi_nxt; float* AVlo_nxt;
+    uint16_t* A16_nxt;
+    size_t a16_plane;
+    const unsigned int* amx_pred; unsigned int* amx_rec;
     const float* grad_y;
     const int* inv;
     float gamma, inv_tm, inv_ta, inv_ts;
     float dt, h8p;
+    float a16s;
     const float* gy_step;
     int needF;
 
@@ -27,6 +60,7 @@
         h8p = n > 0 ? __fsub_rn(__ldg(t + n), __ldg(t + n - 1)) * 0.125f : 0.f;
         needF = __ldg(inv + 3 * p.N);
         gy_step = grad_y + (size_t)n * p.B * G;
+        a16s = A16_nxt ? ldexpf(1.0f, dw16_shift(__ldcg(amx_pred))) : 0.f;
     }
 
     struct Group { float4 aV, aA, dr, lV, lA, lF, p4V, p4A, p3V, p3A, gv, ga, gf; };
@@ -63,6 +97,7 @@
         const int bg = n0 + g * TNq;
         Group nxt;
         load_group(nxt, o0, pl, bg, gV, gA, gF);
+        unsigned int mx = 0u;
 #pragma unroll 1
         for (int q = 0; q < nq; ++q) {
             const size_t oq = o0 + q * qstride;
@@ -127,10 +162,23 @@
             for (int e = 0; e < 4; ++e) {
                 const float v = gamma * nV[e];
                 const float h = tf32_rna(v);
+                const bool ok = b0 + e < B;
                 float* ph = ah + (size_t)e * NPk;
-                st_global_if(ph, h, b0 + e < B);
-                st_global_if(ph + lo_off, tf32_rna(v - h), b0 + e < B);
-            }
+                st_global_if(ph, h, ok);
+                st_global_if(ph + lo_off, tf32_rna(v - h), ok);
+                if (A16_nxt) {
+                    const F16x2 t2 = f16_split2(v * a16s);
+                    uint16_t* p16 = A16_nxt + (size_t)(b0 + e) * NPk + j;
+                    st_global_u16_if(p16, t2.h, ok);
+                    st_global_u16_if(p16 + a16_plane, t2.l, ok);
+                    if (ok) mx = max(mx, __float_as_uint(fabsf(v)));
+                }
+            }
+        }
+        if (A16_nxt) {
+            const unsigned int act = __activemask();
+            const unsigned int m = __reduce_max_sync(act, mx);
+            if (m && (threadIdx.x & 31) == (unsigned)(__ffs(act) - 1)) atomicMax(amx_rec, m);
         }
     }
     ODECOL_DEVINL void tile_done(int, int, int, int, int) const {}
@@ -139,14 +187,17 @@
 constexpr int DW_BK = 32;
 constexpr int DW_T = 128;
 struct DwShape { int MT, NT, Z, rows_per_split, total_rows, N, Kaug, ld_w; float* grad_W; uint32_t lbo, sbo, major_bits, kadv;
-                 float* partial; };
-ODECOL_DEVINL uint64_t make_smem_desc_mn(uint32_t smem_addr, uint32_t lbo, uint32_t sbo) {
+                 float* partial;
+                 const unsigned int* fmt;
+                 const float* scl; };
+constexpr uint32_t DW16_BOX = DW_BK16 * 128, DW16_SBO = 1024, DW16_KADV = 2048;
+ODECOL_DEVINL uint64_t make_smem_desc_mn(uint32_t smem_addr, uint32_t lbo, uint32_t sbo, uint32_t swz = 1) {
     uint64_t d = 0;
     d |= (uint64_t)((smem_addr & 0x3FFFFu) >> 4);
     d |= (uint64_t)(lbo >> 4) << 16;
     d |= (uint64_t)(sbo >> 4) << 32;
     d |= (uint64_t)1 << 46;
-    d |= (uint64_t)1 << 61;
+    d |= (uint64_t)swz << 61;
     return d;
 }
 
@@ -164,7 +215,16 @@
     float gamma, inv_tm, inv_ta, inv_ts;
     unsigned int* done; unsigned int done_base;
     DwShape ds;
+    Dw16 d16;
 };
+
+template <class E>
+__host__ __device__ __forceinline__ void set_a16(E& e, const Dw16& d, int n, int S, size_t nxt, size_t astride) {
+    const int m = S == 1 ? n - 1 : n;
+    e.A16_nxt = d.A16 ? d.A16 + nxt * astride : nullptr;
+    e.a16_plane = d.a16_plane;
+    e.amx_pred = d.amx + m + 2; e.amx_rec = d.amx + m;
+}
 
 template <int S>
 ODECOL_DEVINL void chain_epilogue(const BwdChainArgs& a, int m_tile, int row, int n0, int nt, int g, int TNq,
@@ -175,10 +235,19 @@
     const size_t astride = (size_t)a.Bp * a.NPk;
     const size_t nxt = S == 1 ? (size_t)((a.set ^ 1) * 4 + 3) : (size_t)(a.set * 4 + S - 2);
     e.AVhi_nxt = a.AVhi + nxt * astride; e.AVlo_nxt = a.AVlo + nxt * astride;
+    set_a16(e, a.d16, a.n, S, nxt, astride);
     e.grad_y = a.grad_y; e.inv = a.inv; e.gamma = a.gamma;
     e.inv_tm = a.inv_tm; e.inv_ta = a.inv_ta; e.inv_ts = a.inv_ts;
     e.prepare();
     e.rows(m_tile, row, n0, nt, g, TNq, tot);
+}
+
+ODECOL_DEVINL void wait_count(const unsigned int* c, unsigned int need) {
+    uint32_t spins = 0;
+    while ((int)(ld_acquire_u32(c) - need) < 0) {
+        __nanosleep(64);
+        if (++spins > (1u << 26)) __trap();
+    }
 }
 
 template <bool FUSE_DW>
@@ -186,7 +255,9 @@
 k_tc_bwd_chain(const __grid_constant__ CUtensorMap mW_hi, const __grid_constant__ CUtensorMap mW_lo,
                const __grid_constant__ CUtensorMap mA_hi, const __grid_constant__ CUtensorMap mA_lo,
                const __grid_constant__ CUtensorMap dA_hi, const __grid_constant__ CUtensorMap dA_lo,
-               const __grid_constant__ CUtensorMap dB_hi, const __grid_constant__ CUtensorMap dB_lo, BwdChainArgs a) {
+               const __grid_constant__ CUtensorMap dB_hi, const __grid_constant__ CUtensorMap dB_lo,
+               const __grid_constant__ CUtensorMap dA16_hi, const __grid_constant__ CUtensorMap dA16_lo,
+               const __grid_constant__ CUtensorMap dB16_hi, const __grid_constant__ CUtensorMap dB16_lo, BwdChainArgs a) {
     extern __shared__ uint8_t smem_raw[];
     __shared__ __align__(8) uint64_t bars[2 * STAGES + 2];
     __shared__ uint32_t tmem_base_slot;
@@ -205,6 +276,8 @@
     const DwShape& ds = a.ds;
     const int dw_tiles = ds.MT * ds.NT, dw_items = FUSE_DW ? dw_tiles * ds.Z : 0;
     constexpr uint32_t dw_box = DW_BK * 128, dw_op = 4 * dw_box, dw_stage = 4 * dw_op;
+    const bool dw16 = FUSE_DW && ds.fmt && *ds.fmt == 0u;
+    const int dw_rows_kb = dw16 ? DW_BK16 : DW_BK;
     const uint32_t stride = FUSE_DW ? (stage_bytes > dw_stage ? stage_bytes : dw_stage) : stage_bytes;
 
     if (threadIdx.x == 0) {
@@ -249,13 +322,18 @@
                     }
                 }
             }
+            if (dw16 && dw_items) {
+                for (int nt = 0; nt < ts.NT; ++nt) wait_count(a.done + nt, a.done_base + (unsigned int)ts.MT * 3u);
+                const unsigned int m = ld_acquire_u32(a.d16.amx + a.n);
+                if (!dw16_window(m, dw16_shift(__ldcg(a.d16.amx + a.n + 2)))) wait_count(a.d16.rs_done + a.n, gridDim.x);
+            }
             for (int item = blockIdx.x; item < dw_items; item += gridDim.x) {
                 const int tile = item % dw_tiles, z = ds.Z - 1 - item / dw_tiles;
                 const int i0 = (tile % ds.MT) * DW_T, k0 = (tile / ds.MT) * DW_T;
                 const int r0 = z * ds.rows_per_split;
                 int r1 = r0 + ds.rows_per_split;
                 if (r1 > ds.total_rows) r1 = ds.total_rows;
-                const int KBd = (r1 - r0) / DW_BK;
+                const int KBd = (r1 - r0) / dw_rows_kb;
                 for (int slot = r0 / a.Bp; slot <= (r1 - 1) / a.Bp && slot < 3 && KBd > 0; ++slot) {
                     const int lo = (r0 > slot * a.Bp ? r0 - slot * a.Bp : 0) / ts.TN;
                     const int hi = ((r1 < (slot + 1) * a.Bp ? r1 - slot * a.Bp : a.Bp) - 1) / ts.TN;
@@ -270,16 +348,26 @@
                 }
                 asm volatile("fence.proxy.async;" ::: "memory");
                 for (int kb = 0; kb < KBd; ++kb) {
-                    const int row = r0 + kb * DW_BK;
+                    const int row = r0 + kb * dw_rows_kb;
                     mbar_wait(empty0 + 8 * stage, phase ^ 1);
                     const uint32_t base = ring + stage * stride, fb = full0 + 8 * stage;
                     mbar_expect_tx(fb, dw_stage);
-#pragma unroll
-                    for (int m = 0; m < 4; ++m) {
-                        tma_load_2d(base + m * dw_box, &dA_hi, fb, i0 + 32 * m, row);
-                        tma_load_2d(base + dw_op + m * dw_box, &dA_lo, fb, i0 + 32 * m, row);
-                        tma_load_2d(base + 2 * dw_op + m * dw_box, &dB_hi, fb, k0 + 32 * m, row);
-                        tma_load_2d(base + 3 * dw_op + m * dw_box, &dB_lo, fb, k0 + 32 * m, row);
+                    if (dw16) {
+#pragma unroll
+                        for (int m = 0; m < 2; ++m) {
+                            tma_load_2d(base + m * DW16_BOX, &dA16_hi, fb, i0 + 64 * m, row);
+                            tma_load_2d(base + dw_op + m * DW16_BOX, &dA16_lo, fb, i0 + 64 * m, row);
+                            tma_load_2d(base + 2 * dw_op + m * DW16_BOX, &dB16_hi, fb, k0 + 64 * m, row);
+                            tma_load_2d(base + 3 * dw_op + m * DW16_BOX, &dB16_lo, fb, k0 + 64 * m, row);
+                        }
+                    } else {
+#pragma unroll
+                        for (int m = 0; m < 4; ++m) {
+                            tma_load_2d(base + m * dw_box, &dA_hi, fb, i0 + 32 * m, row);
+                            tma_load_2d(base + dw_op + m * dw_box, &dA_lo, fb, i0 + 32 * m, row);
+                            tma_load_2d(base + 2 * dw_op + m * dw_box, &dB_hi, fb, k0 + 32 * m, row);
+                            tma_load_2d(base + 3 * dw_op + m * dw_box, &dB_lo, fb, k0 + 32 * m, row);
+                        }
                     }
                     if (++stage == STAGES) { stage = 0; phase ^= 1; }
                 }
@@ -315,15 +403,17 @@
                     tphase ^= 1;
                 }
             }
-            const uint32_t idesc_dw = (1u << 4) | (2u << 7) | (2u << 10) | ds.major_bits |
+            const uint32_t idesc_dw = (1u << 4) | (dw16 ? 0u : (2u << 7) | (2u << 10)) | ds.major_bits |
                                       ((uint32_t)(DW_T >> 3) << 17) | ((uint32_t)(BM >> 4) << 24);
             const uint32_t d_small_dw = tmem_base + kMainAcc * DW_T;
+            const uint32_t lbo = dw16 ? DW16_BOX : ds.lbo, sbo = dw16 ? DW16_SBO : ds.sbo, kadv = dw16 ? DW16_KADV : ds.kadv;
+            const uint32_t swz = dw16 ? 2u : 1u;
             for (int item = blockIdx.x; item < dw_items; item += gridDim.x) {
                 const int z = ds.Z - 1 - item / dw_tiles;
                 const int r0 = z * ds.rows_per_split;
                 int r1 = r0 + ds.rows_per_split;
                 if (r1 > ds.total_rows) r1 = ds.total_rows;
-                const int KBd = (r1 - r0) / DW_BK;
+                const int KBd = (r1 - r0) / dw_rows_kb;
                 mbar_wait(tempty, tphase ^ 1);
                 tc_fence_after();
                 int j = 0;
@@ -331,14 +421,21 @@
                     mbar_wait(full0 + 8 * stage, phase);
                     tc_fence_after();
                     const uint32_t base = ring + stage * stride;
-                    const uint64_t a_hi = make_smem_desc_mn(base, ds.lbo, ds.sbo), a_lo = make_smem_desc_mn(base + dw_op, ds.lbo, ds.sbo);
-                    const uint64_t b_hi = make_smem_desc_mn(base + 2 * dw_op, ds.lbo, ds.sbo), b_lo = make_smem_desc_mn(base + 3 * dw_op, ds.lbo, ds.sbo);
-#pragma unroll
-                    for (int k = 0; k < DW_BK / 8; ++k, ++j) {
-                        const uint64_t adv = (uint64_t)((k * ds.kadv) >> 4);
-                        umma_tf32(d_small_dw, a_lo + adv, b_hi + adv, idesc_dw, j != 0);
-                        umma_tf32(d_small_dw, a_hi + adv, b_lo + adv, idesc_dw, 1);
-                        umma_tf32(tmem_base + (uint32_t)(j % kMainAcc) * DW_T, a_hi + adv, b_hi + adv, idesc_dw, j >= kMainAcc);
+                    const uint64_t a_hi = make_smem_desc_mn(base, lbo, sbo, swz), a_lo = make_smem_desc_mn(base + dw_op, lbo, sbo, swz);
+                    const uint64_t b_hi = make_smem_desc_mn(base + 2 * dw_op, lbo, sbo, swz), b_lo = make_smem_desc_mn(base + 3 * dw_op, lbo, sbo, swz);
+#pragma unroll
+                    for (int k = 0; k < 4; ++k, ++j) {
+                        const uint64_t adv = (uint64_t)((k * kadv) >> 4);
+                        const uint32_t d_main = tmem_base + (uint32_t)(j % kMainAcc) * DW_T;
+                        if (dw16) {
+                            umma_f16(d_small_dw, a_lo + adv, b_hi + adv, idesc_dw, j != 0);
+                            umma_f16(d_small_dw, a_hi + adv, b_lo + adv, idesc_dw, 1);
+                            umma_f16(d_main, a_hi + adv, b_hi + adv, idesc_dw, j >= kMainAcc);
+                        } else {
+                            umma_tf32(d_small_dw, a_lo + adv, b_hi + adv, idesc_dw, j != 0);
+                            umma_tf32(d_small_dw, a_hi + adv, b_lo + adv, idesc_dw, 1);
+                            umma_tf32(d_main, a_hi + adv, b_hi + adv, idesc_dw, j >= kMainAcc);
+                        }
                     }
                     umma_commit(empty0 + 8 * stage);
                     if (++stage == STAGES) { stage = 0; phase ^= 1; }
@@ -394,13 +491,34 @@
                 if (etid == 0) atomicAdd(a.done + nt, 1u);
             }
         }
+        float dw_xs = 1.0f, dw_inv = 1.0f;
+        if (dw16 && dw_items) {
+            if (etid == 0)
+                for (int nt = 0; nt < ts.NT; ++nt) wait_count(a.done + nt, a.done_base + (unsigned int)ts.MT * 3u);
+            asm volatile("bar.sync 1, %0;" ::"r"(kEpiWarps * 32) : "memory");
+            const unsigned int m = ld_acquire_u32(a.d16.amx + a.n);
+            const int shp = dw16_shift(__ldcg(a.d16.amx + a.n + 2));
+            const bool ok = dw16_window(m, shp);
+            const int sh = ok ? shp : dw16_shift(m);
+            dw_xs = 4.8828125e-4f;
+            dw_inv = ldexpf(1.0f, -sh);
+            if (!ok) {
+                const size_t astride = (size_t)a.Bp * a.NPk, o = (size_t)a.set * 4 * astride;
+                const int nthr = kEpiWarps * 32;
+                dw16_resplit(a.AVhi + o, a.AVlo + o, a.d16.A16 + o, a.d16.a16_plane, 4 * astride, ldexpf(1.0f, sh),
+                             (size_t)blockIdx.x * nthr + etid, (size_t)gridDim.x * nthr);
+                __threadfence();
+                asm volatile("bar.sync 1, %0;" ::"r"(kEpiWarps * 32) : "memory");
+                if (etid == 0) atomicAdd(a.d16.rs_done + a.n, 1u);
+            }
+        }
         for (int item = blockIdx.x; item < dw_items; item += gridDim.x) {
             const int tile = item % dw_tiles, z = ds.Z - 1 - item / dw_tiles;
             const int i0 = (tile % ds.MT) * DW_T, k0 = (tile / ds.MT) * DW_T;
             const int r0 = z * ds.rows_per_split;
             int r1 = r0 + ds.rows_per_split;
             if (r1 > ds.total_rows) r1 = ds.total_rows;
-            const bool any = (r1 - r0) / DW_BK > 0;
+            const bool any = (r1 - r0) / dw_rows_kb > 0;
             const int i = i0 + quarter * 32 + lane;
             mbar_wait(tfull, tphase);
             tc_fence_after();
@@ -413,11 +531,11 @@
                 tmem_ld_wait();
 #pragma unroll
                 for (int e = 0; e < 4; ++e) {
-                    float sum = __uint_as_float(u[kMainAcc][e]);
+                    float sum = __uint_as_float(u[kMainAcc][e]) * dw_xs;
 #pragma unroll
                     for (int c = 0; c < kMainAcc; ++c) sum += __uint_as_float(u[c][e]);
                     const int k = k0 + g * 32 + 4 * qq + e;
-                    if (any && i < ds.N && k < ds.Kaug) atomicAdd(ds.grad_W + (size_t)i * ds.ld_w + k, sum);
+                    if (any && i < ds.N && k < ds.Kaug) atomicAdd(ds.grad_W + (size_t)i * ds.ld_w + k, sum * dw_inv);
                 }
             }
             tc_fence_before();
@@ -479,10 +597,13 @@
     const float* VA; const float* KV; const float* t;
     int n, KPa, slices;
     float* Rhi; float* Rlo; size_t rstride;
+    uint16_t* R16; size_t r16_plane;
+    const unsigned int* fmt;
+    unsigned int* ovf;
     float* D[4];
 };
 
-ODECOL_DEVINL void replay_unit(const ReplayJob& j, int blk, int slice, int tid) {
+ODECOL_DEVINL void replay_unit(const ReplayJob& j, bool f16, int blk, int slice, int tid) {
     const DevProblem& p = j.p;
     const TileGeom& tg = j.tg;
     const int b4 = blk * 4, N = p.N;
@@ -511,17 +632,30 @@
         }
 #pragma unroll
         for (int s = 0; s < 4; ++s) st4s(j.D[s] + o, make_float4(D[s][0], D[s][1], D[s][2], D[s][3]));
-        float* rh = j.Rhi + (size_t)b4 * j.KPa + i;
-        const ptrdiff_t lo_off = j.Rlo - j.Rhi;
-#pragma unroll
-        for (int s = 0; s < 4; ++s)
-#pragma unroll
-            for (int e = 0; e < 4; ++e) {
-                const float h = tf32_rna(R[s][e]);
-                float* ph = rh + s * j.rstride + (size_t)e * j.KPa;
-                st_global_if(ph, h, b4 + e < p.B);
-                st_global_if(ph + lo_off, tf32_rna(R[s][e] - h), b4 + e < p.B);
-            }
+        if (f16) {
+            uint16_t* r16 = j.R16 + (size_t)b4 * j.KPa + i;
+#pragma unroll
+            for (int s = 0; s < 4; ++s)
+#pragma unroll
+                for (int e = 0; e < 4; ++e) {
+                    const F16x2 t2 = f16_split2(R[s][e]);
+                    uint16_t* ph = r16 + s * j.rstride + (size_t)e * j.KPa;
+                    st_global_u16_if(ph, t2.h, b4 + e < p.B);
+                    st_global_u16_if(ph + j.r16_plane, t2.l, b4 + e < p.B);
+                }
+        } else {
+            float* rh = j.Rhi + (size_t)b4 * j.KPa + i;
+            const ptrdiff_t lo_off = j.Rlo - j.Rhi;
+#pragma unroll
+            for (int s = 0; s < 4; ++s)
+#pragma unroll
+                for (int e = 0; e < 4; ++e) {
+                    const float h = tf32_rna(R[s][e]);
+                    float* ph = rh + s * j.rstride + (size_t)e * j.KPa;
+                    st_global_if(ph, h, b4 + e < p.B);
+                    st_global_if(ph + lo_off, tf32_rna(R[s][e] - h), b4 + e < p.B);
+                }
+        }
     }
     if (slice != 0) return;
     if (p.n_in == 0) return;
@@ -529,20 +663,25 @@
     const float ts = s == 0 ? t0 : s == 1 ? __fadd_rn(t0, __fmul_rn(dt, kOneThirdL)) : s == 2 ? __fadd_rn(t0, __fmul_rn(dt, kTwoThirdsL)) : t1;
     int idx = 1;
     const float tcl = knot_locate(p.knot_t, p.K, ts, idx);
-    stimulus_columns(p, j.KPa, idx, tcl, b4, 4, 0, 1, tid & 31, 32, j.Rhi + s * j.rstride, j.Rlo + s * j.rstride);
+    if (f16) stimulus_columns16(p, j.KPa, j.r16_plane, idx, tcl, b4, 4, 0, 1, tid & 31, 32, j.R16 + s * j.rstride, j.ovf);
+    else stimulus_columns(p, j.KPa, idx, tcl, b4, 4, 0, 1, tid & 31, 32, j.Rhi + s * j.rstride, j.Rlo + s * j.rstride);
 }
 
 __global__ void __launch_bounds__(128, 8) k_tc_replay(ReplayJob j) {
-    for (int slice = 0; slice < j.slices; ++slice) replay_unit(j, blockIdx.x, slice, threadIdx.x);
+    const bool f16 = j.fmt && *j.fmt == 0u;
+    for (int slice = 0; slice < j.slices; ++slice) replay_unit(j, f16, blockIdx.x, slice, threadIdx.x);
 }
 
 __global__ void k_tc_bwd_begin(DevProblem p, TileGeom tg, const float* __restrict__ grad_y, const int* __restrict__ inv,
                                int G, const float* __restrict__ t, int T, float gamma, float* __restrict__ lamT,
-                               float* __restrict__ acurT, float* __restrict__ AVhi, float* __restrict__ AVlo, int NPk) {
+                               float* __restrict__ acurT, float* __restrict__ AVhi, float* __restrict__ AVlo, int NPk,
+                               uint16_t* __restrict__ A16, size_t a16_plane, unsigned int* __restrict__ amx) {
     const int b4 = blockIdx.x * 4, N = p.N;
     const int nt = b4 / tg.TN, g = (b4 % tg.TN) / tg.TNq, q = ((b4 % tg.TN) % tg.TNq) >> 2;
     const size_t pl = tg.plane();
     const float h8 = __fsub_rn(__ldg(t + T - 1), __ldg(t + T - 2)) * 0.125f;
+    const float a16s = A16 ? ldexpf(1.0f, dw16_shift(amx[T])) : 0.f;
+    unsigned int mx = 0u;
     for (int i = threadIdx.x; i < tg.Np; i += blockDim.x) {
         float L[3][4];
 #pragma unroll
@@ -570,8 +709,19 @@
                 const float h = tf32_rna(v);
                 AVhi[(size_t)b * NPk + i] = h;
                 AVlo[(size_t)b * NPk + i] = tf32_rna(v - h);
-            }
-        }
+                if (A16) {
+                    const F16x2 t2 = f16_split2(v * a16s);
+                    A16[(size_t)b * NPk + i] = t2.h;
+                    A16[a16_plane + (size_t)b * NPk + i] = t2.l;
+                    mx = max(mx, __float_as_uint(fabsf(v)));
+                }
+            }
+        }
+    }
+    if (A16) {
+#pragma unroll
+        for (int o = 16; o > 0; o >>= 1) mx = max(mx, __shfl_xor_sync(0xffffffffu, mx, o));
+        if ((threadIdx.x & 31) == 0 && mx) { atomicMax(amx + T - 2, mx); atomicMax(amx + T - 1, mx); }
     }
 }
 
@@ -590,11 +740,13 @@
     }
 }
 
-__global__ void k_tc_set_one(float* __restrict__ Rhi, int Bp, int B, int KPa, int col, int nslots) {
+__global__ void k_tc_set_one(float* __restrict__ Rhi, uint16_t* __restrict__ R16, const unsigned int* __restrict__ fmt,
+                             int Bp, int B, int KPa, int col, int nslots) {
     const int e = blockIdx.x * blockDim.x + threadIdx.x;
     if (e >= nslots * B) return;
     const int s = e / B, b = e % B;
-    Rhi[((size_t)s * Bp + b) * KPa + col] = 1.0f;
+    if (fmt && *fmt == 0u) R16[((size_t)s * Bp + b) * KPa + col] = 0x3C00u;
+    else Rhi[((size_t)s * Bp + b) * KPa + col] = 1.0f;
 }
 
 
@@ -606,7 +758,9 @@
 
 __global__ void __launch_bounds__(kThreads, 1)
 k_tc_dw(const __grid_constant__ CUtensorMap mA_hi, const __grid_constant__ CUtensorMap mA_lo,
-        const __grid_constant__ CUtensorMap mB_hi, const __grid_constant__ CUtensorMap mB_lo, DwShape ds) {
+        const __grid_constant__ CUtensorMap mB_hi, const __grid_constant__ CUtensorMap mB_lo,
+        const __grid_constant__ CUtensorMap mA16_hi, const __grid_constant__ CUtensorMap mA16_lo,
+        const __grid_constant__ CUtensorMap mB16_hi, const __grid_constant__ CUtensorMap mB16_lo, DwShape ds) {
     extern __shared__ uint8_t smem_raw[];
     __shared__ __align__(8) uint64_t bars[2 * STAGES + 4];
     __shared__ uint32_t tmem_base_slot;
@@ -618,12 +772,14 @@
     const uint32_t full0 = smem_u32(&bars[0]), empty0 = smem_u32(&bars[STAGES]);
     const uint32_t tfull0 = smem_u32(&bars[2 * STAGES]), tempty0 = smem_u32(&bars[2 * STAGES + 2]);
     constexpr uint32_t ncols = 512;
+    const bool f16 = ds.fmt && *ds.fmt == 0u;
     const int tile = blockIdx.x % (ds.MT * ds.NT), z = blockIdx.x / (ds.MT * ds.NT);
     const int i0 = (tile % ds.MT) * DW_T, k0 = (tile / ds.MT) * DW_T;
     const int r0 = z * ds.rows_per_split;
     int r1 = r0 + ds.rows_per_split;
     if (r1 > ds.total_rows) r1 = ds.total_rows;
-    const int KB = (r1 - r0) / DW_BK;
+    const int rows_kb = f16 ? DW_BK16 : DW_BK;
+    const int KB = (r1 - r0) / rows_kb;
     const int nchunks = (KB + DW_CHUNK - 1) / DW_CHUNK;
 
     if (threadIdx.x == 0) {
@@ -647,21 +803,33 @@
                 mbar_wait(empty0 + 8 * stage, phase ^ 1);
                 const uint32_t base = ring + stage * stage_bytes, fb = full0 + 8 * stage;
                 mbar_expect_tx(fb, stage_bytes);
-                const int row = r0 + kb * DW_BK;
-#pragma unroll
-                for (int m = 0; m < 4; ++m) {
-                    tma_load_2d(base + m * box_bytes, &mA_hi, fb, i0 + 32 * m, row);
-                    tma_load_2d(base + op_bytes + m * box_bytes, &mA_lo, fb, i0 + 32 * m, row);
-                    tma_load_2d(base + 2 * op_bytes + m * box_bytes, &mB_hi, fb, k0 + 32 * m, row);
-                    tma_load_2d(base + 3 * op_bytes + m * box_bytes, &mB_lo, fb, k0 + 32 * m, row);
+                const int row = r0 + kb * rows_kb;
+                if (f16) {
+#pragma unroll
+                    for (int m = 0; m < 2; ++m) {
+                        tma_load_2d(base + m * DW16_BOX, &mA16_hi, fb, i0 + 64 * m, row);
+                        tma_load_2d(base + op_bytes + m * DW16_BOX, &mA16_lo, fb, i0 + 64 * m, row);
+                        tma_load_2d(base + 2 * op_bytes + m * DW16_BOX, &mB16_hi, fb, k0 + 64 * m, row);
+                        tma_load_2d(base + 3 * op_bytes + m * DW16_BOX, &mB16_lo, fb, k0 + 64 * m, row);
+                    }
+                } else {
+#pragma unroll
+                    for (int m = 0; m < 4; ++m) {
+                        tma_load_2d(base + m * box_bytes, &mA_hi, fb, i0 + 32 * m, row);
+                        tma_load_2d(base + op_bytes + m * box_bytes, &mA_lo, fb, i0 + 32 * m, row);
+                        tma_load_2d(base + 2 * op_bytes + m * box_bytes, &mB_hi, fb, k0 + 32 * m, row);
+                        tma_load_2d(base + 3 * op_bytes + m * box_bytes, &mB_lo, fb, k0 + 32 * m, row);
+                    }
                 }
                 if (++stage == STAGES) { stage = 0; phase ^= 1; }
             }
         }
     } else if (warp == kMmaWarp) {
         if (lane == 0) {
-            const uint32_t idesc = (1u << 4) | (2u << 7) | (2u << 10) | ds.major_bits |
+            const uint32_t idesc = (1u << 4) | (f16 ? 0u : (2u << 7) | (2u << 10)) | ds.major_bits |
                                    ((uint32_t)(DW_T >> 3) << 17) | ((uint32_t)(BM >> 4) << 24);
+            const uint32_t lbo = f16 ? DW16_BOX : ds.lbo, sbo = f16 ? DW16_SBO : ds.sbo, kadv = f16 ? DW16_KADV : ds.kadv;
+            const uint32_t swz = f16 ? 2u : 1u;
             int stage = 0; uint32_t phase = 0;
             int c = 0, jj = 0;
             uint32_t d_main = tmem_base, d_cross = tmem_base + DW_T;
@@ -677,14 +845,20 @@
                 mbar_wait(full0 + 8 * stage, phase);
                 tc_fence_after();
                 const uint32_t base = ring + stage * stage_bytes;
-                const uint64_t a_hi = make_smem_desc_mn(base, ds.lbo, ds.sbo), a_lo = make_smem_desc_mn(base + op_bytes, ds.lbo, ds.sbo);
-                const uint64_t b_hi = make_smem_desc_mn(base + 2 * op_bytes, ds.lbo, ds.sbo), b_lo = make_smem_desc_mn(base + 3 * op_bytes, ds.lbo, ds.sbo);
-#pragma unroll
-                for (int k = 0; k < DW_BK / 8; ++k, ++jj) {
-                    const uint64_t adv = (uint64_t)((k * ds.kadv) >> 4);
-                    umma_tf32(d_cross, a_lo + adv, b_hi + adv, idesc, jj != 0);
-                    umma_tf32(d_cross, a_hi + adv, b_lo + adv, idesc, 1);
-                    umma_tf32(d_main, a_hi + adv, b_hi + adv, idesc, jj != 0);
+                const uint64_t a_hi = make_smem_desc_mn(base, lbo, sbo, swz), a_lo = make_smem_desc_mn(base + op_bytes, lbo, sbo, swz);
+                const uint64_t b_hi = make_smem_desc_mn(base + 2 * op_bytes, lbo, sbo, swz), b_lo = make_smem_desc_mn(base + 3 * op_bytes, lbo, sbo, swz);
+#pragma unroll
+                for (int k = 0; k < 4; ++k, ++jj) {
+                    const uint64_t adv = (uint64_t)((k * kadv) >> 4);
+                    if (f16) {
+                        umma_f16(d_cross, a_lo + adv, b_hi + adv, idesc, jj != 0);
+                        umma_f16(d_cross, a_hi + adv, b_lo + adv, idesc, 1);
+                        umma_f16(d_main, a_hi + adv, b_hi + adv, idesc, jj != 0);
+                    } else {
+                        umma_tf32(d_cross, a_lo + adv, b_hi + adv, idesc, jj != 0);
+                        umma_tf32(d_cross, a_hi + adv, b_lo + adv, idesc, 1);
+                        umma_tf32(d_main, a_hi + adv, b_hi + adv, idesc, jj != 0);
+                    }
                 }
                 umma_commit(empty0 + 8 * stage);
                 if (++stage == STAGES) { stage = 0; phase ^= 1; }
@@ -696,6 +870,7 @@
         const int i = i0 + quarter * 32 + lane;
         float acc[32];
         float* dst = ds.partial ? ds.partial + (size_t)z * ds.N * ds.ld_w : nullptr;
+        const float xs = f16 ? 4.8828125e-4f : 1.0f, inv = f16 ? *ds.scl : 1.0f;
 #pragma unroll
         for (int q = 0; q < 32; ++q) {
             const int k = k0 + g * 32 + q;
@@ -713,7 +888,7 @@
                 tmem_ld4_issue(lane_base + DW_T + 4 * q, ux);
                 tmem_ld_wait();
 #pragma unroll
-                for (int e = 0; e < 4; ++e) acc[4 * q + e] += __uint_as_float(ux[e]) + __uint_as_float(um[e]);
+                for (int e = 0; e < 4; ++e) acc[4 * q + e] += (__uint_as_float(ux[e]) * xs + __uint_as_float(um[e])) * inv;
             }
             tc_fence_before();
             __syncwarp();
@@ -749,6 +924,7 @@
 }
 
 static int launch_dw(const CUtensorMap& a_hi, const CUtensorMap& a_lo, const CUtensorMap& b_hi, const CUtensorMap& b_lo,
+                     const CUtensorMap& a16_hi, const CUtensorMap& a16_lo, const CUtensorMap& b16_hi, const CUtensorMap& b16_lo,
                      const DwShape& ds, cudaStream_t s) {
     static bool configured = false;
     if (!configured) {
@@ -756,9 +932,22 @@
             return ODECOL_E_CUDA;
         configured = true;
     }
-    k_tc_dw<<<ds.MT * ds.NT * ds.Z, kThreads, (size_t)STAGES * 4 * 4 * DW_BK * 128 + 1024, s>>>(a_hi, a_lo, b_hi, b_lo, ds);
+    k_tc_dw<<<ds.MT * ds.NT * ds.Z, kThreads, (size_t)STAGES * 4 * 4 * DW_BK * 128 + 1024, s>>>(a_hi, a_lo, b_hi, b_lo, a16_hi, a16_lo,
+                                                                                                b16_hi, b16_lo, ds);
     count_launch();
     return cudaGetLastError() == cudaSuccess ? ODECOL_OK : ODECOL_E_CUDA;
+}
+
+__global__ void k_dw16_check(Dw16 d, int n, const float* __restrict__ AVhi, const float* __restrict__ AVlo, size_t o, size_t count) {
+    if (*d.fmt != 0u) return;
+    const unsigned int m = d.amx[n];
+    const int shp = dw16_shift(d.amx[n + 2]);
+    const bool ok = dw16_window(m, shp);
+    const int sh = ok ? shp : dw16_shift(m);
+    if (blockIdx.x == 0 && threadIdx.x == 0) d.scl[n] = ldexpf(1.0f, -sh);
+    if (ok) return;
+    dw16_resplit(AVhi + o, AVlo + o, d.A16 + o, d.a16_plane, count, ldexpf(1.0f, sh), blockIdx.x * (size_t)blockDim.x + threadIdx.x,
+                 (size_t)gridDim.x * blockDim.x);
 }
 
 
@@ -778,10 +967,11 @@
     int Np, Bp, KPa, NPk, TN;
     size_t off_Whi, off_Wlo, off_WThi, off_WTlo, off_Rhi, off_Rlo, off_AVhi, off_AVlo;
     size_t off_K[3], off_Y, off_DRT[4], off_lam, off_b4, off_b3, off_acur, off_inv, off_done, off_dwpart, total;
+    size_t off_A16, off_R16, off_d16;
     int dwZ;
 };
 
-static TcBwdLayout tc_bwd_layout(const DevProblem& p) {
+static TcBwdLayout tc_bwd_layout(const DevProblem& p, int T) {
     TcBwdLayout L;
     L.Np = round_up(p.N, BM);
     L.NPk = L.Np;
@@ -808,6 +998,9 @@
         L.dwZ = z;
         L.off_dwpart = take(4ull * (size_t)z * p.N * p.ld_w);
     }
+    L.off_A16 = take(2 * 2 * 8ull * L.Bp * L.NPk);
+    L.off_R16 = take(2 * 2 * 4ull * L.Bp * L.KPa);
+    L.off_d16 = take(4 * (3ull * (T > 0 ? T : 0) + 2) + 4);
     L.total = o;
     return L;
 }
@@ -841,9 +1034,10 @@
     ds.rows_per_split = rows; ds.Z = (Kp + rows - 1) / rows;
     ds.N = M; ds.Kaug = N; ds.ld_w = N; ds.grad_W = C; ds.partial = nullptr;
     ds.lbo = DW_BK * 128; ds.sbo = 512; ds.major_bits = (1u << 15) | (1u << 16); ds.kadv = 1024;
+    ds.fmt = nullptr; ds.scl = nullptr;
     if (cudaMemsetAsync(C, 0, sizeof(float) * (size_t)M * N, s) != cudaSuccess) return ODECOL_E_CUDA;
     count_launch(2);
-    return launch_dw(a_hi, a_lo, b_hi, b_lo, ds, s);
+    return launch_dw(a_hi, a_lo, b_hi, b_lo, a_hi, a_lo, b_hi, b_lo, ds, s);
 }
 
 int tc_dw_accumulate(const float* Ahi, const float* Alo, const float* Bhi, const float* Blo, int rows, int Np, int KPa, int N,
@@ -864,16 +1058,17 @@
     ds.rows_per_split = rps; ds.Z = (rows + rps - 1) / rps;
     ds.N = N; ds.Kaug = Kaug; ds.ld_w = ld_w; ds.grad_W = grad_W; ds.partial = nullptr;
     ds.lbo = DW_BK * 128; ds.sbo = 512; ds.major_bits = (1u << 15) | (1u << 16); ds.kadv = 1024;
-    return launch_dw(a_hi, a_lo, b_hi, b_lo, ds, s);
-}
-
-size_t tc_rk4_bwd_workspace_bytes(const DevProblem& p, int) { return tc::tc_bwd_layout(p).total; }
+    ds.fmt = nullptr; ds.scl = nullptr;
+    return launch_dw(a_hi, a_lo, b_hi, b_lo, a_hi, a_lo, b_hi, b_lo, ds, s);
+}
+
+size_t tc_rk4_bwd_workspace_bytes(const DevProblem& p, int T) { return tc::tc_bwd_layout(p, T).total; }
 
 static int tc_rk4_bwd_impl(const DevProblem& p, const float* t_dev, int T, const float* y_traj, const float* ckVA,
-                           const float* ckK, const float* grad_y, const int* sel, int G, float* grad_y0, float* grad_W,
-                           void* ws, size_t ws_bytes, cudaStream_t s) {
+                           const float* ckK, const unsigned int* fmt, const float* grad_y, const int* sel, int G,
+                           float* grad_y0, float* grad_W, void* ws, size_t ws_bytes, cudaStream_t s) {
     using namespace tc;
-    const TcBwdLayout L = tc_bwd_layout(p);
+    const TcBwdLayout L = tc_bwd_layout(p, T);
     if (!ws || ws_bytes < L.total) return ODECOL_E_WORKSPACE;
     if (p.N % 4 != 0) return ODECOL_E_UNSUPPORTED;
     char* w = static_cast<char*>(ws);
@@ -892,14 +1087,27 @@
     const TileGeom tg{L.Bp / L.TN, L.Np, L.TN, L.TN / 4};
     const size_t rstride = (size_t)L.Bp * L.KPa, astride = (size_t)L.Bp * L.NPk;
 
+    Dw16 d16;
+    uint16_t* R16 = reinterpret_cast<uint16_t*>(w + L.off_R16);
+    const size_t r16_plane = 4 * rstride;
+    unsigned int* d16w = reinterpret_cast<unsigned int*>(w + L.off_d16);
+    d16.fmt = ckVA ? fmt : nullptr;
+    d16.amx = d16w + 1;
+    d16.scl = reinterpret_cast<float*>(d16w + T + 2);
+    d16.rs_done = d16w + 2 * T + 2;
+    d16.A16 = d16.fmt ? reinterpret_cast<uint16_t*>(w + L.off_A16) : nullptr;
+    d16.a16_plane = 8 * astride;
+
     if (cudaMemsetAsync(w + L.off_Rhi, 0, L.off_K[0] - L.off_Rhi, s) != cudaSuccess) return ODECOL_E_CUDA;
+    if (d16.fmt && cudaMemsetAsync(w + L.off_A16, 0, L.total - L.off_A16, s) != cudaSuccess) return ODECOL_E_CUDA;
     k_split_pad<<<296, 256, 0, s>>>(p.W_aug, p.N, Kaug, p.ld_w, Whi, Wlo, L.Np, L.KPa);
     k_split_pad_T<<<296, 256, 0, s>>>(p.W_aug, p.N, p.ld_w, WThi, WTlo, L.Np, L.NPk);
-    k_tc_set_one<<<(4 * p.B + 255) / 256, 256, 0, s>>>(Rhi, L.Bp, p.B, L.KPa, Kaug - 1, 4);
+    k_tc_set_one<<<(4 * p.B + 255) / 256, 256, 0, s>>>(Rhi, R16, d16.fmt, L.Bp, p.B, L.KPa, Kaug - 1, 4);
     k_tc_build_inv<<<1, 256, 0, s>>>(sel, G, 3 * p.N, inv);
     const size_t first = (size_t)(((T - 2) & 1) * 4 + 3);
     k_tc_bwd_begin<<<L.Bp / 4, 128, 0, s>>>(p, tg, grad_y, inv, G, t_dev, T, gamma, lamT, acurT, AVhi + first * astride,
-                                           AVlo + first * astride, L.NPk);
+                                           AVlo + first * astride, L.NPk, d16.A16 ? d16.A16 + first * astride : nullptr,
+                                           d16.a16_plane, d16.amx);
     unsigned int* done = reinterpret_cast<unsigned int*>(w + L.off_done);
     if (cudaMemsetAsync(done, 0, sizeof(unsigned int) * (size_t)(L.Bp / L.TN), s) != cudaSuccess) return ODECOL_E_CUDA;
     count_launch(5);
@@ -915,6 +1123,13 @@
               make_map(&dAlo[1], AVlo + 4 * astride, 4ull * L.Bp, L.NPk, L.NPk, DW_BK, CU_TENSOR_MAP_SWIZZLE_128B_ATOM_32B) &&
               make_map(&dBhi, Rhi, 4ull * L.Bp, L.KPa, L.KPa, DW_BK, CU_TENSOR_MAP_SWIZZLE_128B_ATOM_32B) &&
               make_map(&dBlo, Rlo, 4ull * L.Bp, L.KPa, L.KPa, DW_BK, CU_TENSOR_MAP_SWIZZLE_128B_ATOM_32B);
+    CUtensorMap dA16hi[2], dA16lo[2], dB16hi, dB16lo;
+    const uint16_t* A16 = reinterpret_cast<const uint16_t*>(w + L.off_A16);
+    for (int k = 0; k < 2; ++k)
+        ok = ok && make_map16(&dA16hi[k], A16 + 4 * k * astride, 4ull * L.Bp, L.NPk, L.NPk, DW_BK16, false) &&
+             make_map16(&dA16lo[k], A16 + d16.a16_plane + 4 * k * astride, 4ull * L.Bp, L.NPk, L.NPk, DW_BK16, false);
+    ok = ok && make_map16(&dB16hi, R16, 4ull * L.Bp, L.KPa, L.KPa, DW_BK16, false) &&
+         make_map16(&dB16lo, R16 + r16_plane, 4ull * L.Bp, L.KPa, L.KPa, DW_BK16, false);
     if (!ok) return ODECOL_E_CUDA;
 
     DwShape ds;
@@ -922,12 +1137,13 @@
     ds.total_rows = 4 * L.Bp;
     int z = num_sms() / (ds.MT * ds.NT);
     if (z < 1) z = 1;
-    int rows = (ds.total_rows / DW_BK + z - 1) / z * DW_BK;
-    if (rows < DW_BK) rows = DW_BK;
+    int rows = (ds.total_rows / DW_BK16 + z - 1) / z * DW_BK16;
+    if (rows < DW_BK16) rows = DW_BK16;
     ds.rows_per_split = rows; ds.Z = (ds.total_rows + rows - 1) / rows;
     ds.N = p.N; ds.Kaug = Kaug; ds.ld_w = p.ld_w; ds.grad_W = grad_W;
     ds.lbo = DW_BK * 128; ds.sbo = 512; ds.major_bits = (1u << 15) | (1u << 16); ds.kadv = 1024;
     ds.partial = nullptr;
+    ds.fmt = d16.fmt; ds.scl = nullptr;
 
     const int MT = L.Np / BM, NT = L.Bp / L.TN;
     const char* pe = getenv("ODECOL_PERSISTENT");
@@ -958,6 +1174,7 @@
         j.VA = ckVA + 2 * ckpl * (size_t)n; j.KV = ckK + 3 * ckpl * (size_t)n; j.t = t_dev;
         j.n = n; j.KPa = L.KPa; j.slices = L.Np / 128;
         j.Rhi = Rhi; j.Rlo = Rlo; j.rstride = rstride;
+        j.R16 = R16; j.r16_plane = r16_plane; j.fmt = d16.fmt; j.ovf = d16w + 3 * T + 2;
         for (int k = 0; k < 4; ++k) j.D[k] = DRT[k];
         k_tc_replay<<<L.Bp / 4, 128, 0, s>>>(j);
         count_launch();
@@ -992,8 +1209,9 @@
             a.AVhi = AVhi; a.AVlo = AVlo; a.set = set; a.grad_y = grad_y; a.inv = inv; a.gamma = gamma;
             a.inv_tm = 1.0f / p.c.tau_m; a.inv_ta = 1.0f / p.c.tau_a; a.inv_ts = 1.0f / p.c.tau_s;
             a.done = done; a.done_base = (unsigned int)MT * 4u * (unsigned int)(T - 2 - n);
-            a.ds = ds;
-            void* args[] = {&mWThi, &mWTlo, &mAVhi, &mAVlo, &dAhi[set], &dAlo[set], &dBhi, &dBlo, &a};
+            a.ds = ds; a.d16 = d16;
+            void* args[] = {&mWThi, &mWTlo, &mAVhi, &mAVlo, &dAhi[set], &dAlo[set], &dBhi, &dBlo,
+                            &dA16hi[set], &dA16lo[set], &dB16hi, &dB16lo, &a};
             const void* chain_fn = fuse_dw ? (const void*)k_tc_bwd_chain<true> : (const void*)k_tc_bwd_chain<false>;
             if (cudaLaunchCooperativeKernel(chain_fn, dim3(chain_grid), dim3(kThreads), args, chain_smem, s) != cudaSuccess)
                 return ODECOL_E_CUDA;
@@ -1004,6 +1222,7 @@
                 e.acurT = acurT; e.lamT = lamT; e.b4T = b4T; e.b3T = b3T; e.DRT = DRT[S - 1];
                 const size_t nxt = S == 1 ? (size_t)((set ^ 1) * 4 + 3) : (size_t)(set * 4 + S - 2);
                 e.AVhi_nxt = AVhi + nxt * astride; e.AVlo_nxt = AVlo + nxt * astride;
+                set_a16(e, d16, n, S, nxt, astride);
                 e.grad_y = grad_y; e.inv = inv; e.gamma = gamma;
                 e.inv_tm = 1.0f / p.c.tau_m; e.inv_ta = 1.0f / p.c.tau_a; e.inv_ts = 1.0f / p.c.tau_s;
                 e.dt = e.h8p = 0.f;
@@ -1015,7 +1234,13 @@
             { BwdEpiT<1> e; fill_b(e, 1); rc = launch_contract(mWThi, mWTlo, mAVhi, mAVlo, TileShape{MT, NT, L.TN, L.NPk / BK, r0 + 0 * L.Bp}, e, s); if (rc) return rc; }
         }
         if (!(use_chain && fuse_dw)) {
-            const int rcd = launch_dw(dAhi[set], dAlo[set], dBhi, dBlo, ds, s);
+            DwShape dsn = ds;
+            if (d16.fmt) {
+                k_dw16_check<<<296, 256, 0, s>>>(d16, n, AVhi, AVlo, set * 4 * astride, 4 * astride);
+                count_launch();
+                dsn.scl = d16.scl + n;
+            }
+            const int rcd = launch_dw(dAhi[set], dAlo[set], dBhi, dBlo, dA16hi[set], dA16lo[set], dB16hi, dB16lo, dsn, s);
             if (rcd) return rcd;
         }
     }
@@ -1032,16 +1257,17 @@
 
 int tc_rk4_bwd(const DevProblem& p, const float* t_dev, int T, const float* y_traj, const float* grad_y, const int* sel,
                int G, float* grad_y0, float* grad_W, void* ws, size_t ws_bytes, cudaStream_t s) {
-    return tc_rk4_bwd_impl(p, t_dev, T, y_traj, nullptr, nullptr, grad_y, sel, G, grad_y0, grad_W, ws, ws_bytes, s);
+    return tc_rk4_bwd_impl(p, t_dev, T, y_traj, nullptr, nullptr, nullptr, grad_y, sel, G, grad_y0, grad_W, ws, ws_bytes, s);
 }
 
 int tc_rk4_bwd_ckpt(const DevProblem& p, const float* t_dev, int T, const void* ckpt, size_t ckpt_bytes, const float* grad_y,
                     const int* sel, int G, float* grad_y0, float* grad_W, void* ws, size_t ws_bytes, cudaStream_t s) {
-    const tc::TcBwdLayout L = tc::tc_bwd_layout(p);
-    const size_t plane = (size_t)L.Np * L.Bp;
-    if (!ckpt || ckpt_bytes < 4 * plane * (2ull * T + 3ull * (T - 1))) return ODECOL_E_WORKSPACE;
+    const tc::TcBwdLayout L = tc::tc_bwd_layout(p, T);
+    const size_t plane = (size_t)L.Np * L.Bp, planes = plane * (2ull * T + 3ull * (T - 1));
+    if (!ckpt || ckpt_bytes < 4 * planes + sizeof(unsigned int)) return ODECOL_E_WORKSPACE;
     const float* VA = static_cast<const float*>(ckpt);
-    return tc_rk4_bwd_impl(p, t_dev, T, nullptr, VA, VA + 2 * plane * (size_t)T, grad_y, sel, G, grad_y0, grad_W, ws, ws_bytes, s);
-}
-
-}
+    return tc_rk4_bwd_impl(p, t_dev, T, nullptr, VA, VA + 2 * plane * (size_t)T, reinterpret_cast<const unsigned int*>(VA + planes),
+                           grad_y, sel, G, grad_y0, grad_W, ws, ws_bytes, s);
+}
+
+}
diff --git a/ode-column_b200/csrc/stage_tc_persist.cu b/ode-column_b200/csrc/stage_tc_persist.cu
--- a/ode-column_b200/csrc/stage_tc_persist.cu
+++ b/ode-column_b200/csrc/stage_tc_persist.cu
@@ -277,7 +277,7 @@
     a.ovf = ovf; a.run_if = nullptr;
     for (int i = 0; i < 3; ++i) a.KT[i] = KT[i];
     a.done = done;
-    if (ck) a.ck = *ck; else a.ck = CkptView{nullptr, nullptr, nullptr, nullptr, 0};
+    if (ck) a.ck = *ck; else a.ck = CkptView{nullptr, nullptr, nullptr, nullptr, 0, nullptr};
     a.inv_tm = 1.0f / p.c.tau_m; a.inv_ta = 1.0f / p.c.tau_a; a.inv_ts = 1.0f / p.c.tau_s;
     const size_t smem = (size_t)STAGES * (2 * BM * BK * 4 + 2 * (size_t)TN * BK * 4) + 1024;
     for (int v = 0; v < 2; ++v) {
@@ -302,6 +302,11 @@
     if (cudaLaunchCooperativeKernel((const void*)k_tc_rk4_fwd_persistent<false>, dim3(grid), dim3(kThreads), args, smem, s) != cudaSuccess)
         return ODECOL_E_CUDA;
     count_launch();
+    if (ck) {
+        const cudaError_t e = f16 ? cudaMemcpyAsync(ck->fmt, ovf, sizeof(unsigned int), cudaMemcpyDeviceToDevice, s)
+                                  : cudaMemsetAsync(ck->fmt, 0xFF, sizeof(unsigned int), s);
+        if (e != cudaSuccess) return ODECOL_E_CUDA;
+    }
     return cudaGetLastError() == cudaSuccess ? ODECOL_OK : ODECOL_E_CUDA;
 }
 
diff --git a/scratch/torch_launch_list.py b/scratch/torch_launch_list.py
--- /dev/null
+++ b/scratch/torch_launch_list.py
@@ -0,0 +1,32 @@
+import runpy
+import sys
+
+import torch
+from torch.profiler import ProfilerActivity, profile
+
+out = sys.argv[1]
+bench_args = sys.argv[sys.argv.index("--") + 1:]
+sys.argv = ["bench.py"] + bench_args
+with profile(activities=[ProfilerActivity.CUDA]) as prof:
+    try:
+        runpy.run_path("bench.py", run_name="__main__")
+    except SystemExit:
+        pass
+    torch.cuda.synchronize()
+rows = []
+for ka in prof.key_averages():
+    t = getattr(ka, "self_device_time_total", None)
+    if t is None:
+        t = ka.self_cuda_time_total
+    if ka.count and t > 0 and not ka.key.startswith("Memcpy") and not ka.key.startswith("Memset"):
+        rows.append((ka.key, ka.count, t))
+rows.sort(key=lambda r: -r[2])
+total = sum(r[2] for r in rows)
+name = torch.cuda.get_device_name()
+with open(out, "w") as f:
+    f.write(f"`python bench.py {' '.join(bench_args)}` under torch.profiler on {name}: {total / 1e3:.2f} ms of kernel time\n\n")
+    f.write("| kernel | launches | total us | mean us | share |\n|---|---:|---:|---:|---:|\n")
+    for k, n, t in rows:
+        k = k.split("(")[0].replace("odecol::tc::", "").replace("odecol::", "")
+        f.write(f"| `{k[:90]}` | {n} | {t:.0f} | {t / n:.1f} | {100 * t / total:.1f} % |\n")
+print(open(out).read())
```

After: 8.170 billion (median of 6 runs). 1.06x the previous value.
